# MihailMihov/simd-raytracer

Measured on AMD Instinct MI355X. Metric: Mrays/s (intersect invocations per second), hw09/scene5 dragon 1920x1080 1spp, higher is better.
Workload: dtype f32; 1 GPU; BASELINE configs[1]: scenes/hw09/scene5.crtscene 1920x1080 1spp max_ray_depth=5 (primary + shadow + reflection rays), kd_tree_simd_accel semantics; rays_per_frame=2726485, primary_rays=2073600, parallelism=bucket-tiles x1

## Files before the change

include/rtk.h:

```cpp
#ifndef RTK_H
#define RTK_H

#include <stddef.h>
#include <stdint.h>

#ifdef __cplusplus
extern "C" {
#endif

#define RTK_ABI_VERSION 4

enum {
    RTK_OK = 0,
    RTK_ERR_INVALID = 1,
    RTK_ERR_NO_DEVICE = 2,
    RTK_ERR_HIP = 3,
    RTK_ERR_IO = 4,
    RTK_ERR_PARSE = 5,
    RTK_ERR_UNSUPPORTED = 6
};

enum { RTK_MAT_DIFFUSE = 0, RTK_MAT_REFLECTIVE = 1, RTK_MAT_REFRACTIVE = 2, RTK_MAT_CONSTANT = 3, RTK_MAT_TEXTURE = 4 };

enum { RTK_TEX_ALBEDO = 0, RTK_TEX_EDGES = 1, RTK_TEX_CHECKER = 2, RTK_TEX_BITMAP = 3 };
// ... 28 lines not shown
    const int32_t *mat_texture;
    const float *uvs;
    const int32_t *mesh_has_uvs;
    int32_t n_textures;
    const int32_t *tex_kind;
    const float *tex_color_a;
    const float *tex_color_b;
    const float *tex_param;
    int32_t n_lights;
    const float *light_pos;
    const float *light_intensity;
    float cam_pos[3];
    float cam_mat[9];
    float background[3];
    int32_t width, height;
    int32_t bucket_size;
    const uint8_t *tex_pixels;
    const int32_t *tex_bitmap;
} rtk_scene_desc;

typedef struct {
    int32_t n_meshes, n_materials, n_lights;
    int32_t n_vertices, n_triangles;
    int32_t width, height, bucket_size;
    int32_t n_textures, n_uv_vertices;
    int32_t n_bitmap_bytes;
} rtk_scene_info;

typedef struct {
    int32_t max_depth;
    int32_t max_leaf_size;
    float eps;
    int32_t normalize_hit_normal;
    int32_t device;
    int32_t traversal;
} rtk_accel_params;

enum { RTK_TRAVERSAL_REFERENCE = 0, RTK_TRAVERSAL_FAST = 1 };

typedef struct {
    int32_t n_nodes, n_inner, n_leaves;
    int32_t n_leaf_refs;
    int32_t max_leaf_refs;
    int32_t n_triangles;
    int32_t tree_depth;
    int32_t reserved;
} rtk_tree_info;

typedef struct { float origin[3]; float direction[3]; } rtk_ray;

typedef struct {
    float t, u, v;
    uint32_t tri;
    uint32_t mesh;
    float normal[3];
} rtk_hit;

typedef struct {
    int32_t width, height;
    int32_t spp;
    int32_t max_ray_depth;
    int32_t diffuse_rays;
    uint32_t seed;
    double fov_degrees;
    float shadow_bias, reflection_bias, refraction_bias;
    int32_t trace_mode;
    int32_t rank, world_size;
    int32_t collect_stats;
    int32_t sample_begin, sample_count;
} rtk_render_params;

typedef struct {
    uint64_t rays;
    uint64_t primary;
    uint64_t hits;
    uint64_t nodes;
    uint64_t boxpass;
    uint64_t leaves;
    uint64_t tris;
    uint64_t packets16;
} rtk_counters;

int rtk_abi_version(void);
const char *rtk_last_error(void);
int rtk_device_count(int *count);

int rtk_scene_create(const rtk_scene_desc *desc, rtk_scene **out);
int rtk_scene_load_crtscene(const char *path, rtk_scene **out);
int rtk_scene_get_info(const rtk_scene *scene, rtk_scene_info *info);
int rtk_scene_get_arrays(const rtk_scene *scene, int32_t *mesh_material, int32_t *mesh_nverts, int32_t *mesh_ntris,
                         float *vertices, uint32_t *indices, int32_t *mat_kind, float *mat_albedo, float *mat_ior,
                         int32_t *mat_smooth, float *light_pos, float *light_intensity, float *cam_pos,
                         float *cam_mat, float *background);
int rtk_scene_get_textures(const rtk_scene *scene, int32_t *mat_texture, int32_t *mesh_has_uvs, float *uvs,
                           int32_t *tex_kind, float *tex_color_a, float *tex_color_b, float *tex_param);
int rtk_scene_get_bitmaps(const rtk_scene *scene, int32_t *tex_bitmap, uint8_t *tex_pixels);
int rtk_decode_jpeg(const uint8_t *data, size_t size, int32_t *width, int32_t *height, int32_t *channels,
                    uint8_t *pixels, size_t cap);
int rtk_scene_vertex_normals(const rtk_scene *scene, int32_t mesh, float *out);
void rtk_scene_destroy(rtk_scene *scene);

int rtk_accel_build(const rtk_scene *scene, const rtk_accel_params *params, rtk_accel **out);
int rtk_accel_tree_info(const rtk_accel *accel, rtk_tree_info *info);
int rtk_accel_tree_dump(const rtk_accel *accel, float *nodes_box, int32_t *nodes_link, int32_t *leaf_refs);
void rtk_accel_destroy(rtk_accel *accel);

int rtk_accel_intersect(rtk_accel *accel, const rtk_ray *rays, size_t n, int cull, int trace_mode,
                        rtk_hit *out);
int rtk_accel_intersect_device(rtk_accel *accel, const rtk_ray *d_rays, size_t n, int cull, int trace_mode,
                               rtk_hit *d_out, void *hip_stream);
int rtk_accel_intersect_stats(rtk_accel *accel, const rtk_ray *d_rays, size_t n, int cull, int trace_mode,
                              rtk_hit *d_out, rtk_counters *counters);

#define RTK_OCCLUDED_MAX_STEPS 1024
enum { RTK_OCC_CLEAR = 0, RTK_OCC_OCCLUDED = 1, RTK_OCC_STEP_LIMIT = 2 };

int rtk_accel_occluded(rtk_accel *accel, const rtk_ray *rays, const float *max_t, size_t n,
                       float shadow_bias, int trace_mode, uint8_t *out,
                       uint64_t *n_intersections );
int rtk_accel_occluded_device(rtk_accel *accel, const rtk_ray *d_rays, const float *d_max_t, size_t n,
                              float shadow_bias, int trace_mode, uint8_t *d_out,
                              void *hip_stream);

typedef struct {
    int32_t max_ray_depth;
    int32_t diffuse_rays;
    uint32_t seed;
    int32_t sample;
    float shadow_bias, reflection_bias, refraction_bias;
    int32_t cull;
    int32_t trace_mode;
} rtk_radiance_params;
int rtk_accel_radiance(rtk_accel *accel, const rtk_ray *rays, const uint32_t *ids , size_t n,
                       const rtk_radiance_params *p, float *rgb , rtk_counters *counters );
int rtk_accel_radiance_device(rtk_accel *accel, const rtk_ray *d_rays, const uint32_t *d_ids , size_t n,
                              const rtk_radiance_params *p, float *d_rgb , void *hip_stream);

int rtk_accel_update_vertices(rtk_accel *accel, const float *vertices );
int rtk_accel_update_vertices_device(rtk_accel *accel, const float *d_vertices , void *hip_stream);

int rtk_accel_update_geometry(rtk_accel *accel, const float *vertices ,
                              const uint32_t *indices ,
                              const int32_t *mesh_ntris );
int rtk_accel_update_geometry_device(rtk_accel *accel, const float *d_vertices, const uint32_t *d_indices,
                                     const int32_t *mesh_ntris , void *hip_stream);

int rtk_render_output_floats(const rtk_accel *accel, const rtk_render_params *p, size_t *n_floats);
int rtk_render_frame(rtk_accel *accel, const rtk_render_params *p, float *rgb ,
                     rtk_counters *counters );
int rtk_render_frame_device(rtk_accel *accel, const rtk_render_params *p, float *d_out, void *hip_stream);
int rtk_render_last_counters(rtk_accel *accel, rtk_counters *counters);
int rtk_render_last_critical_path(rtk_accel *accel, double *ms);
int rtk_debug_counter_fills(rtk_accel *accel, uint64_t *fills);
int rtk_tiles_assemble_device(const rtk_accel *accel, const rtk_render_params *p, const float *d_gathered,
                              float *d_rgb, void *hip_stream);

int rtk_camera_rays(rtk_accel *accel, const rtk_render_params *p, int32_t sample, rtk_ray *rays );
int rtk_camera_rays_device(rtk_accel *accel, const rtk_render_params *p, int32_t sample, rtk_ray *d_rays, void *hip_stream);

typedef struct { float position[3]; float matrix[9]; } rtk_view;

int rtk_accel_get_camera(const rtk_accel *accel, rtk_view *out);
int rtk_accel_set_camera(rtk_accel *accel, const rtk_view *view);

int rtk_render_views(rtk_accel *accel, const rtk_render_params *p, const rtk_view *views , int32_t n_views,
                     float *rgb , rtk_counters *counters );
int rtk_render_views_device(rtk_accel *accel, const rtk_render_params *p, const rtk_view *d_views ,
                            int32_t n_views, float *d_out , void *hip_stream);

typedef struct { int32_t x0, y0, x1, y1; } rtk_rect;
enum { RTK_REGIONS_IN_FRAME = 0, RTK_REGIONS_PACKED = 1 };

int rtk_render_regions(rtk_accel *accel, const rtk_render_params *p, const rtk_rect *rects , int32_t n_rects,
                       int layout, float *rgb , rtk_counters *counters );
int rtk_render_regions_device(rtk_accel *accel, const rtk_render_params *p, const rtk_rect *rects , int32_t n_rects,
                              int layout, float *d_out , void *hip_stream);

typedef struct {
    float    *depth;
    float    *position;
    float    *normal;
    float    *albedo;
    float    *bary;
    uint32_t *tri, *mesh, *material;
} rtk_gbuffer;

int rtk_render_gbuffer(rtk_accel *accel, const rtk_render_params *p, int32_t sample,
                       const rtk_view *views , int32_t n_views,
                       const rtk_gbuffer *out );
int rtk_render_gbuffer_device(rtk_accel *accel, const rtk_render_params *p, int32_t sample,
                              const rtk_view *d_views , int32_t n_views,
                              const rtk_gbuffer *out , void *hip_stream);

typedef struct {
    int32_t min_samples;
    int32_t step;
    float   threshold;
    float   floor;
} rtk_adaptive_params;

int rtk_render_adaptive(rtk_accel *accel, const rtk_render_params *p, const rtk_adaptive_params *ap,
                        float *rgb , uint32_t *samples ,
                        float *noise , rtk_counters *counters );
int rtk_render_adaptive_device(rtk_accel *accel, const rtk_render_params *p, const rtk_adaptive_params *ap,
                               float *d_rgb, uint32_t *d_samples, float *d_noise, void *hip_stream);

int rtk_render_frame_noise(rtk_accel *accel, const rtk_render_params *p, float *rgb ,
                           float *noise , rtk_counters *counters );
int rtk_render_frame_noise_device(rtk_accel *accel, const rtk_render_params *p, float *d_rgb, float *d_noise, void *hip_stream);
int rtk_debug_noise_fallbacks(rtk_accel *accel, uint64_t *count);

typedef struct {
    int32_t width, height;
    int32_t iterations;
    int32_t normal_power_log2;
    float   sigma_luminance;
    float   sigma_plane;
    float   albedo_floor;
    int32_t reserved;
} rtk_denoise_params;
typedef struct { const float *rgb, *noise, *albedo, *normal, *position, *depth; } rtk_denoise_inputs;

int rtk_denoise_workspace_bytes(const rtk_denoise_params *p, int32_t n_images, size_t *bytes);
int rtk_denoise_frame(const rtk_denoise_params *p, int32_t n_images, const rtk_denoise_inputs *in ,
                      float *rgb_out );
int rtk_denoise_frame_device(const rtk_denoise_params *p, int32_t n_images,
                             const rtk_denoise_inputs *in , float *d_rgb_out,
                             void *d_workspace, size_t workspace_bytes, void *hip_stream);

typedef struct { float position[3]; float intensity; } rtk_light;
typedef struct { int32_t kind, smooth; float albedo[3]; float ior; int32_t texture; int32_t reserved; } rtk_material;

int rtk_accel_get_lights(const rtk_accel *accel, rtk_light *out , int32_t cap, int32_t *n);
int rtk_accel_set_lights(rtk_accel *accel, const rtk_light *lights , int32_t n);
int rtk_accel_set_lights_device(rtk_accel *accel, const rtk_light *d_lights , int32_t n, void *hip_stream);

int rtk_accel_get_materials(const rtk_accel *accel, rtk_material *out );
int rtk_accel_set_materials(rtk_accel *accel, const rtk_material *materials , int32_t n);

int rtk_accel_get_background(const rtk_accel *accel, float rgb[3]);
int rtk_accel_set_background(rtk_accel *accel, const float rgb[3]);

typedef struct { int32_t kind; float color_a[3]; float color_b[3]; float param; int32_t width, height; } rtk_texture;

int rtk_accel_get_textures(const rtk_accel *accel, rtk_texture *out , int32_t cap, int32_t *n);
int rtk_accel_get_texture_pixels(const rtk_accel *accel, int32_t texture, uint8_t *out , size_t cap, size_t *n_bytes);
int rtk_accel_set_textures(rtk_accel *accel, const rtk_texture *textures, int32_t n,
                           const uint8_t *const *pixels );
int rtk_accel_set_texture_pixels(rtk_accel *accel, int32_t texture, int32_t width, int32_t height, const uint8_t *rgb );
int rtk_accel_set_texture_pixels_device(rtk_accel *accel, int32_t texture, int32_t width, int32_t height, const uint8_t *d_rgb, void *hip_stream);
int rtk_accel_set_texture_frame_device(rtk_accel *accel, int32_t texture, int32_t width, int32_t height,
                                       const float *d_rgb , void *hip_stream);
int rtk_accel_get_uvs(const rtk_accel *accel, float *uvs );
int rtk_accel_set_uvs(rtk_accel *accel, const float *uvs );
int rtk_accel_set_uvs_device(rtk_accel *accel, const float *d_uvs , void *hip_stream);

int rtk_frame_to_rgb8_device(const float *d_rgb, size_t n, uint8_t *d_out, void *hip_stream);
int rtk_format_ppm_rgb8(const uint8_t *rgb8, int32_t width, int32_t height, char *buf, size_t cap, size_t *n);
int rtk_write_ppm(const float *rgb, int32_t width, int32_t height, const char *path);
int rtk_format_ppm(const float *rgb, int32_t width, int32_t height, char *buf, size_t cap, size_t *n);

#ifdef __cplusplus
}
#endif
#endif
```

simd-raytracer_amd/__init__.py:

```python
from __future__ import annotations

import ctypes as C
import os
from dataclasses import dataclass

import numpy as np

_HERE = os.path.dirname(os.path.abspath(__file__))
_LIB_PATH = os.environ.get("RTK_LIB_OVERRIDE") or os.path.join(_HERE, "librtk_hip.so")

RTK_OK, RTK_ERR_INVALID, RTK_ERR_NO_DEVICE, RTK_ERR_HIP, RTK_ERR_IO, RTK_ERR_PARSE, RTK_ERR_UNSUPPORTED = range(7)
MAT_DIFFUSE, MAT_REFLECTIVE, MAT_REFRACTIVE, MAT_CONSTANT, MAT_TEXTURE = 0, 1, 2, 3, 4
TEX_ALBEDO, TEX_EDGES, TEX_CHECKER, TEX_BITMAP = 0, 1, 2, 3
TRACE_AUTO, TRACE_LANE, TRACE_WAVE, TRACE_GROUP4, TRACE_GROUP8, TRACE_GROUP16, TRACE_STREAM, TRACE_TWOPASS = 0, 1, 2, 3, 4, 5, 6, 7
TRAVERSAL_REFERENCE, TRAVERSAL_FAST = 0, 1
TRACE_REPACK = 8
OCC_CLEAR, OCC_OCCLUDED, OCC_STEP_LIMIT = 0, 1, 2
OCCLUDED_MAX_STEPS = 1024
REGIONS_IN_FRAME, REGIONS_PACKED = 0, 1
MAX_REGIONS = 65536

ABI_SYMBOLS = [
    "rtk_abi_version", "rtk_last_error", "rtk_device_count",
    "rtk_scene_create", "rtk_scene_load_crtscene", "rtk_scene_get_info", "rtk_scene_get_arrays", "rtk_scene_get_textures",
    "rtk_scene_get_bitmaps", "rtk_decode_jpeg",
    "rtk_scene_vertex_normals", "rtk_scene_destroy",
    "rtk_accel_build", "rtk_accel_tree_info", "rtk_accel_tree_dump", "rtk_accel_destroy",
    "rtk_accel_intersect", "rtk_accel_intersect_device", "rtk_accel_intersect_stats",
    "rtk_accel_occluded", "rtk_accel_occluded_device",
    "rtk_accel_radiance", "rtk_accel_radiance_device",
    "rtk_accel_update_vertices", "rtk_accel_update_vertices_device",
    "rtk_accel_update_geometry", "rtk_accel_update_geometry_device",
    "rtk_render_output_floats", "rtk_render_frame", "rtk_render_frame_device", "rtk_render_last_counters",
    "rtk_render_last_critical_path", "rtk_debug_counter_fills",
    "rtk_tiles_assemble_device", "rtk_camera_rays", "rtk_camera_rays_device",
    "rtk_accel_get_camera", "rtk_accel_set_camera", "rtk_render_views", "rtk_render_views_device",
    "rtk_render_regions", "rtk_render_regions_device",
    "rtk_render_gbuffer", "rtk_render_gbuffer_device",
    "rtk_render_adaptive", "rtk_render_adaptive_device",
    "rtk_render_frame_noise", "rtk_render_frame_noise_device", "rtk_debug_noise_fallbacks",
    "rtk_denoise_workspace_bytes", "rtk_denoise_frame", "rtk_denoise_frame_device",
    "rtk_accel_get_lights", "rtk_accel_set_lights", "rtk_accel_set_lights_device",
    "rtk_accel_get_materials", "rtk_accel_set_materials", "rtk_accel_get_background", "rtk_accel_set_background",
    "rtk_accel_get_textures", "rtk_accel_get_texture_pixels", "rtk_accel_set_textures", "rtk_accel_set_texture_pixels",
    "rtk_accel_set_texture_pixels_device", "rtk_accel_set_texture_frame_device",
    "rtk_accel_get_uvs", "rtk_accel_set_uvs", "rtk_accel_set_uvs_device",
    "rtk_frame_to_rgb8_device", "rtk_format_ppm_rgb8", "rtk_write_ppm", "rtk_format_ppm",
]


class RtkError(RuntimeError):
    def __init__(self, code: int, msg: str):
        super().__init__(f"rtk error {code}: {msg}")
        self.code = code


if not os.path.exists(_LIB_PATH):
    raise ImportError(
        f"{_LIB_PATH} is missing: build it with `python -c 'import __graft_entry__ as g; g.build()'` "
        "(hipcc --offload-arch=gfx950).  This package has no CPU fallback."
    )

try:
    import torch
except ImportError:
    torch = None

_L = C.CDLL(_LIB_PATH)


class SceneDesc(C.Structure):
    _fields_ = [
        ("n_meshes", C.c_int32), ("mesh_material", C.POINTER(C.c_int32)), ("mesh_nverts", C.POINTER(C.c_int32)),
        ("mesh_ntris", C.POINTER(C.c_int32)), ("vertices", C.POINTER(C.c_float)), ("indices", C.POINTER(C.c_uint32)),
        ("n_materials", C.c_int32), ("mat_kind", C.POINTER(C.c_int32)), ("mat_albedo", C.POINTER(C.c_float)),
        ("mat_ior", C.POINTER(C.c_float)), ("mat_smooth", C.POINTER(C.c_int32)),
        ("mat_texture", C.POINTER(C.c_int32)), ("uvs", C.POINTER(C.c_float)), ("mesh_has_uvs", C.POINTER(C.c_int32)),
        ("n_textures", C.c_int32), ("tex_kind", C.POINTER(C.c_int32)), ("tex_color_a", C.POINTER(C.c_float)),
        ("tex_color_b", C.POINTER(C.c_float)), ("tex_param", C.POINTER(C.c_float)),
        ("n_lights", C.c_int32), ("light_pos", C.POINTER(C.c_float)), ("light_intensity", C.POINTER(C.c_float)),
        ("cam_pos", C.c_float * 3), ("cam_mat", C.c_float * 9), ("background", C.c_float * 3),
        ("width", C.c_int32), ("height", C.c_int32), ("bucket_size", C.c_int32),
        ("tex_pixels", C.POINTER(C.c_uint8)), ("tex_bitmap", C.POINTER(C.c_int32)),
    ]


class SceneInfo(C.Structure):
    _fields_ = [(n, C.c_int32) for n in
                ("n_meshes", "n_materials", "n_lights", "n_vertices", "n_triangles", "width", "height", "bucket_size",
                 "n_textures", "n_uv_vertices", "n_bitmap_bytes")]


class AccelParams(C.Structure):
    _fields_ = [("max_depth", C.c_int32), ("max_leaf_size", C.c_int32), ("eps", C.c_float),
                ("normalize_hit_normal", C.c_int32), ("device", C.c_int32), ("traversal", C.c_int32)]


class TreeInfo(C.Structure):
    _fields_ = [(n, C.c_int32) for n in
                ("n_nodes", "n_inner", "n_leaves", "n_leaf_refs", "max_leaf_refs", "n_triangles", "tree_depth", "reserved")]


class RenderParams(C.Structure):
    _fields_ = [("width", C.c_int32), ("height", C.c_int32), ("spp", C.c_int32), ("max_ray_depth", C.c_int32),
                ("diffuse_rays", C.c_int32), ("seed", C.c_uint32), ("fov_degrees", C.c_double),
                ("shadow_bias", C.c_float), ("reflection_bias", C.c_float), ("refraction_bias", C.c_float),
                ("trace_mode", C.c_int32), ("rank", C.c_int32), ("world_size", C.c_int32), ("collect_stats", C.c_int32),
                ("sample_begin", C.c_int32), ("sample_count", C.c_int32)]


class RadianceParams(C.Structure):
    _fields_ = [("max_ray_depth", C.c_int32), ("diffuse_rays", C.c_int32), ("seed", C.c_uint32), ("sample", C.c_int32),
                ("shadow_bias", C.c_float), ("reflection_bias", C.c_float), ("refraction_bias", C.c_float),
                ("cull", C.c_int32), ("trace_mode", C.c_int32)]


class Counters(C.Structure):
    _fields_ = [(n, C.c_uint64) for n in ("rays", "primary", "hits", "nodes", "boxpass", "leaves", "tris", "packets16")]

    def as_dict(self):
        return {n: int(getattr(self, n)) for n, _ in self._fields_}


class GBuffer(C.Structure):
    _fields_ = [(n, C.c_void_p) for n in ("depth", "position", "normal", "albedo", "bary", "tri", "mesh", "material")]


class AdaptiveParams(C.Structure):
    _fields_ = [("min_samples", C.c_int32), ("step", C.c_int32), ("threshold", C.c_float), ("floor", C.c_float)]


class DenoiseParams(C.Structure):
    _fields_ = [("width", C.c_int32), ("height", C.c_int32), ("iterations", C.c_int32), ("normal_power_log2", C.c_int32),
                ("sigma_luminance", C.c_float), ("sigma_plane", C.c_float), ("albedo_floor", C.c_float), ("reserved", C.c_int32)]


class DenoiseInputs(C.Structure):
    _fields_ = [(n, C.c_void_p) for n in ("rgb", "noise", "albedo", "normal", "position", "depth")]


GBUFFER_PLANES = {"depth": ((), np.float32), "position": ((3,), np.float32), "normal": ((3,), np.float32),
                  "albedo": ((3,), np.float32), "bary": ((2,), np.float32), "tri": ((), np.uint32), "mesh": ((), np.uint32),
                  "material": ((), np.uint32)}

RAY_DTYPE = np.dtype([("origin", "<f4", (3,)), ("direction", "<f4", (3,))])
LIGHT_DTYPE = np.dtype([("position", "<f4", (3,)), ("intensity", "<f4")])
MATERIAL_DTYPE = np.dtype([("kind", "<i4"), ("smooth", "<i4"), ("albedo", "<f4", (3,)), ("ior", "<f4"), ("texture", "<i4"),
                           ("reserved", "<i4")])
TEXTURE_DTYPE = np.dtype([("kind", "<i4"), ("color_a", "<f4", (3,)), ("color_b", "<f4", (3,)), ("param", "<f4"), ("width", "<i4"),
                          ("height", "<i4")])
assert LIGHT_DTYPE.itemsize == 16 and MATERIAL_DTYPE.itemsize == 32 and TEXTURE_DTYPE.itemsize == 40
HIT_DTYPE = np.dtype([("t", "<f4"), ("u", "<f4"), ("v", "<f4"), ("tri", "<u4"), ("mesh", "<u4"), ("normal", "<f4", (3,))])
assert RAY_DTYPE.itemsize == 24 and HIT_DTYPE.itemsize == 32

_vp = C.c_void_p
_L.rtk_abi_version.restype = C.c_int
_L.rtk_last_error.restype = C.c_char_p
_L.rtk_device_count.argtypes = [C.POINTER(C.c_int)]
_L.rtk_scene_create.argtypes = [C.POINTER(SceneDesc), C.POINTER(_vp)]
_L.rtk_scene_load_crtscene.argtypes = [C.c_char_p, C.POINTER(_vp)]
_L.rtk_scene_get_info.argtypes = [_vp, C.POINTER(SceneInfo)]
_L.rtk_scene_get_arrays.argtypes = [_vp] * 15
_L.rtk_scene_get_textures.argtypes = [_vp] * 8
_L.rtk_scene_get_bitmaps.argtypes = [_vp] * 3
_L.rtk_decode_jpeg.argtypes = [_vp, C.c_size_t, C.POINTER(C.c_int32), C.POINTER(C.c_int32), C.POINTER(C.c_int32), _vp, C.c_size_t]
_L.rtk_scene_vertex_normals.argtypes = [_vp, C.c_int32, _vp]
_L.rtk_scene_destroy.argtypes = [_vp]
_L.rtk_scene_destroy.restype = None
_L.rtk_accel_build.argtypes = [_vp, C.POINTER(AccelParams), C.POINTER(_vp)]
_L.rtk_accel_tree_info.argtypes = [_vp, C.POINTER(TreeInfo)]
_L.rtk_accel_tree_dump.argtypes = [_vp, _vp, _vp, _vp]
_L.rtk_accel_destroy.argtypes = [_vp]
_L.rtk_accel_destroy.restype = None
_L.rtk_accel_intersect.argtypes = [_vp, _vp, C.c_size_t, C.c_int, C.c_int, _vp]
_L.rtk_accel_intersect_device.argtypes = [_vp, _vp, C.c_size_t, C.c_int, C.c_int, _vp, _vp]
_L.rtk_accel_intersect_stats.argtypes = [_vp, _vp, C.c_size_t, C.c_int, C.c_int, _vp, C.POINTER(Counters)]
_L.rtk_accel_occluded.argtypes = [_vp, _vp, _vp, C.c_size_t, C.c_float, C.c_int, _vp, C.POINTER(C.c_uint64)]
_L.rtk_accel_occluded_device.argtypes = [_vp, _vp, _vp, C.c_size_t, C.c_float, C.c_int, _vp, _vp]
_L.rtk_accel_radiance.argtypes = [_vp, _vp, _vp, C.c_size_t, C.POINTER(RadianceParams), _vp, C.POINTER(Counters)]
_L.rtk_accel_radiance_device.argtypes = [_vp, _vp, _vp, C.c_size_t, C.POINTER(RadianceParams), _vp, _vp]
_L.rtk_accel_update_vertices.argtypes = [_vp, _vp]
_L.rtk_accel_update_vertices_device.argtypes = [_vp, _vp, _vp]
_L.rtk_accel_update_geometry.argtypes = [_vp, _vp, _vp, _vp]
_L.rtk_accel_update_geometry_device.argtypes = [_vp, _vp, _vp, _vp, _vp]
_L.rtk_render_output_floats.argtypes = [_vp, C.POINTER(RenderParams), C.POINTER(C.c_size_t)]
_L.rtk_render_frame.argtypes = [_vp, C.POINTER(RenderParams), _vp, C.POINTER(Counters)]
_L.rtk_render_frame_device.argtypes = [_vp, C.POINTER(RenderParams), _vp, _vp]
_L.rtk_render_last_counters.argtypes = [_vp, C.POINTER(Counters)]
_L.rtk_render_last_critical_path.argtypes = [_vp, C.POINTER(C.c_double)]
if hasattr(_L, "rtk_debug_counter_fills"):
    _L.rtk_debug_counter_fills.argtypes = [_vp, C.POINTER(C.c_uint64)]
_L.rtk_tiles_assemble_device.argtypes = [_vp, C.POINTER(RenderParams), _vp, _vp, _vp]
_L.rtk_camera_rays.argtypes = [_vp, C.POINTER(RenderParams), C.c_int32, _vp]
_L.rtk_camera_rays_device.argtypes = [_vp, C.POINTER(RenderParams), C.c_int32, _vp, _vp]
_L.rtk_accel_get_camera.argtypes = [_vp, _vp]
_L.rtk_accel_set_camera.argtypes = [_vp, _vp]
_L.rtk_render_views.argtypes = [_vp, C.POINTER(RenderParams), _vp, C.c_int32, _vp, C.POINTER(Counters)]
_L.rtk_render_views_device.argtypes = [_vp, C.POINTER(RenderParams), _vp, C.c_int32, _vp, _vp]
_L.rtk_render_regions.argtypes = [_vp, C.POINTER(RenderParams), _vp, C.c_int32, C.c_int, _vp, C.POINTER(Counters)]
_L.rtk_render_regions_device.argtypes = [_vp, C.POINTER(RenderParams), _vp, C.c_int32, C.c_int, _vp, _vp]
_L.rtk_render_gbuffer.argtypes = [_vp, C.POINTER(RenderParams), C.c_int32, _vp, C.c_int32, C.POINTER(GBuffer)]
_L.rtk_render_gbuffer_device.argtypes = [_vp, C.POINTER(RenderParams), C.c_int32, _vp, C.c_int32, C.POINTER(GBuffer), _vp]
_L.rtk_render_adaptive.argtypes = [_vp, C.POINTER(RenderParams), C.POINTER(AdaptiveParams), _vp, _vp, _vp, C.POINTER(Counters)]
_L.rtk_render_adaptive_device.argtypes = [_vp, C.POINTER(RenderParams), C.POINTER(AdaptiveParams), _vp, _vp, _vp, _vp]
if hasattr(_L, "rtk_render_frame_noise"):
    _L.rtk_render_frame_noise.argtypes = [_vp, C.POINTER(RenderParams), _vp, _vp, C.POINTER(Counters)]
    _L.rtk_render_frame_noise_device.argtypes = [_vp, C.POINTER(RenderParams), _vp, _vp, _vp]
    _L.rtk_debug_noise_fallbacks.argtypes = [_vp, C.POINTER(C.c_uint64)]
_L.rtk_denoise_workspace_bytes.argtypes =[C.POINTER(DenoiseParams), C.c_int32, C.POINTER(C.c_size_t)]
_L.rtk_denoise_frame.argtypes = [C.POINTER(DenoiseParams), C.c_int32, C.POINTER(DenoiseInputs), _vp]
_L.rtk_denoise_frame_device.argtypes = [C.POINTER(DenoiseParams), C.c_int32, C.POINTER(DenoiseInputs), _vp, _vp, C.c_size_t, _vp]
_L.rtk_accel_get_lights.argtypes =[_vp, _vp, C.c_int32, C.POINTER(C.c_int32)]
_L.rtk_accel_set_lights.argtypes = [_vp, _vp, C.c_int32]
_L.rtk_accel_set_lights_device.argtypes = [_vp, _vp, C.c_int32, _vp]
_L.rtk_accel_get_materials.argtypes = [_vp, _vp]
_L.rtk_accel_set_materials.argtypes = [_vp, _vp, C.c_int32]
_L.rtk_accel_get_background.argtypes = [_vp, _vp]
_L.rtk_accel_set_background.argtypes = [_vp, _vp]
_L.rtk_accel_get_textures.argtypes = [_vp, _vp, C.c_int32, C.POINTER(C.c_int32)]
_L.rtk_accel_get_texture_pixels.argtypes = [_vp, C.c_int32, _vp, C.c_size_t, C.POINTER(C.c_size_t)]
_L.rtk_accel_set_textures.argtypes = [_vp, _vp, C.c_int32, _vp]
_L.rtk_accel_set_texture_pixels.argtypes = [_vp, C.c_int32, C.c_int32, C.c_int32, _vp]
_L.rtk_accel_set_texture_pixels_device.argtypes = [_vp, C.c_int32, C.c_int32, C.c_int32, _vp, _vp]
_L.rtk_accel_set_texture_frame_device.argtypes = [_vp, C.c_int32, C.c_int32, C.c_int32, _vp, _vp]
_L.rtk_accel_get_uvs.argtypes = [_vp, _vp]
_L.rtk_accel_set_uvs.argtypes = [_vp, _vp]
_L.rtk_accel_set_uvs_device.argtypes = [_vp, _vp, _vp]
_L.rtk_frame_to_rgb8_device.argtypes = [_vp, C.c_size_t, _vp, _vp]
_L.rtk_format_ppm_rgb8.argtypes = [_vp, C.c_int32, C.c_int32, _vp, C.c_size_t, C.POINTER(C.c_size_t)]
_L.rtk_write_ppm.argtypes = [_vp, C.c_int32, C.c_int32, C.c_char_p]
_L.rtk_format_ppm.argtypes = [_vp, C.c_int32, C.c_int32, _vp, C.c_size_t, C.POINTER(C.c_size_t)]


def _check(rc: int) -> None:
    if rc != RTK_OK:
        raise RtkError(rc, (_L.rtk_last_error() or b"").decode("utf-8", "replace"))


def lib() -> C.CDLL:
    return _L


def lib_path() -> str:
    return _LIB_PATH


def abi_version() -> int:
    return _L.rtk_abi_version()


def device_count() -> int:
    n = C.c_int(0)
    _check(_L.rtk_device_count(C.byref(n)))
    return n.value


def _fp(a, ty):
    return a.ctypes.data_as(C.POINTER(ty))


class Scene:

    def __init__(self, handle):
        self._h = handle
        info = SceneInfo()
        _check(_L.rtk_scene_get_info(self._h, C.byref(info)))
        self.info = info

    @classmethod
    def from_arrays(cls, mesh_material, mesh_nverts, mesh_ntris, vertices, indices, mat_kind, mat_albedo, mat_ior,
                    mat_smooth, light_pos, light_intensity, cam_pos, cam_mat, background, width, height, bucket_size=64,
                    mat_texture=None, uvs=None, mesh_has_uvs=None, tex_kind=None, tex_color_a=None, tex_color_b=None,
                    tex_param=None, tex_pixels=None, tex_bitmap=None):
        n_tex = 0 if tex_kind is None else len(tex_kind)
        keep = dict(
            mt=np.ascontiguousarray(mat_texture if mat_texture is not None else np.full(len(mat_kind), -1), np.int32),
            uv=np.ascontiguousarray(uvs if uvs is not None else np.zeros((0, 2)), np.float32),
            hu=np.ascontiguousarray(mesh_has_uvs if mesh_has_uvs is not None else np.zeros(len(mesh_material)), np.int32),
            tk=np.ascontiguousarray(tex_kind if tex_kind is not None else np.zeros(0), np.int32),
            ta=np.ascontiguousarray(tex_color_a if tex_color_a is not None else np.zeros((n_tex, 3)), np.float32),
            tb=np.ascontiguousarray(tex_color_b if tex_color_b is not None else np.zeros((n_tex, 3)), np.float32),
            tp=np.ascontiguousarray(tex_param if tex_param is not None else np.zeros(n_tex), np.float32),
            px=np.ascontiguousarray(tex_pixels if tex_pixels is not None else np.zeros(0), np.uint8),
            bm=np.ascontiguousarray(tex_bitmap if tex_bitmap is not None else np.zeros((n_tex, 3)), np.int32),
            mm=np.ascontiguousarray(mesh_material, np.int32), nv=np.ascontiguousarray(mesh_nverts, np.int32),
            nt=np.ascontiguousarray(mesh_ntris, np.int32), v=np.ascontiguousarray(vertices, np.float32),
            ix=np.ascontiguousarray(indices, np.uint32), mk=np.ascontiguousarray(mat_kind, np.int32),
            ma=np.ascontiguousarray(mat_albedo, np.float32), mi=np.ascontiguousarray(mat_ior, np.float32),
            ms=np.ascontiguousarray(mat_smooth, np.int32), lp=np.ascontiguousarray(light_pos, np.float32),
            li=np.ascontiguousarray(light_intensity, np.float32),
        )
        d = SceneDesc()
        d.n_meshes = len(keep["mm"])
        d.mesh_material, d.mesh_nverts, d.mesh_ntris = _fp(keep["mm"], C.c_int32), _fp(keep["nv"], C.c_int32), _fp(keep["nt"], C.c_int32)
        d.vertices, d.indices = _fp(keep["v"], C.c_float), _fp(keep["ix"], C.c_uint32)
        d.n_materials = len(keep["mk"])
        d.mat_kind, d.mat_albedo = _fp(keep["mk"], C.c_int32), _fp(keep["ma"], C.c_float)
        d.mat_ior, d.mat_smooth = _fp(keep["mi"], C.c_float), _fp(keep["ms"], C.c_int32)
        d.mat_texture, d.uvs, d.mesh_has_uvs = _fp(keep["mt"], C.c_int32), _fp(keep["uv"], C.c_float), _fp(keep["hu"], C.c_int32)
        d.n_textures = n_tex
        d.tex_kind, d.tex_color_a = _fp(keep["tk"], C.c_int32), _fp(keep["ta"], C.c_float)
        d.tex_color_b, d.tex_param = _fp(keep["tb"], C.c_float), _fp(keep["tp"], C.c_float)
        d.tex_pixels, d.tex_bitmap = _fp(keep["px"], C.c_uint8), _fp(keep["bm"], C.c_int32)
        d.n_lights = len(keep["li"])
        d.light_pos, d.light_intensity = _fp(keep["lp"], C.c_float), _fp(keep["li"], C.c_float)
        d.cam_pos[:] = [float(x) for x in np.asarray(cam_pos, np.float32)]
        d.cam_mat[:] = [float(x) for x in np.asarray(cam_mat, np.float32)]
        d.background[:] = [float(x) for x in np.asarray(background, np.float32)]
        d.width, d.height, d.bucket_size = int(width), int(height), int(bucket_size)
        h = _vp()
        _check(_L.rtk_scene_create(C.byref(d), C.byref(h)))
        return cls(h)

    def arrays(self) -> dict:
        i = self.info
        out = dict(
            mesh_material=np.zeros(i.n_meshes, np.int32), mesh_nverts=np.zeros(i.n_meshes, np.int32),
            mesh_ntris=np.zeros(i.n_meshes, np.int32), vertices=np.zeros((i.n_vertices, 3), np.float32),
            indices=np.zeros((i.n_triangles, 3), np.uint32), mat_kind=np.zeros(i.n_materials, np.int32),
            mat_albedo=np.zeros((i.n_materials, 3), np.float32), mat_ior=np.zeros(i.n_materials, np.float32),
            mat_smooth=np.zeros(i.n_materials, np.int32), light_pos=np.zeros((i.n_lights, 3), np.float32),
            light_intensity=np.zeros(i.n_lights, np.float32), cam_pos=np.zeros(3, np.float32),
            cam_mat=np.zeros(9, np.float32), background=np.zeros(3, np.float32),
        )
        _check(_L.rtk_scene_get_arrays(self._h, *[a.ctypes.data for a in out.values()]))
        tex = dict(
            mat_texture=np.zeros(i.n_materials, np.int32), mesh_has_uvs=np.zeros(i.n_meshes, np.int32),
            uvs=np.zeros((i.n_uv_vertices, 2), np.float32), tex_kind=np.zeros(i.n_textures, np.int32),
            tex_color_a=np.zeros((i.n_textures, 3), np.float32), tex_color_b=np.zeros((i.n_textures, 3), np.float32),
            tex_param=np.zeros(i.n_textures, np.float32),
        )
        _check(_L.rtk_scene_get_textures(self._h, *[a.ctypes.data for a in tex.values()]))
        out.update(tex)
        bmp = dict(tex_bitmap=np.zeros((i.n_textures, 3), np.int32), tex_pixels=np.zeros(i.n_bitmap_bytes, np.uint8))
        _check(_L.rtk_scene_get_bitmaps(self._h, bmp["tex_bitmap"].ctypes.data, bmp["tex_pixels"].ctypes.data))
        out.update(bmp)
        out.update(width=i.width, height=i.height, bucket_size=i.bucket_size)
        return out

    def vertex_normals(self, mesh: int) -> np.ndarray:
        nv = int(self.arrays()["mesh_nverts"][mesh])
        out = np.zeros((nv, 3), np.float32)
        _check(_L.rtk_scene_vertex_normals(self._h, mesh, out.ctypes.data))
        return out
# ... 395 lines not shown
        _check(_L.rtk_render_adaptive_device(self._h, C.byref(p), C.byref(ap), d_rgb_ptr or None, d_samples_ptr or None,
                                             d_noise_ptr or None, stream))

    def render_frame_noise(self, cfg: RenderConfig):
        w = cfg.width or self.scene.info.width
        h = cfg.height or self.scene.info.height
        rgb = np.zeros((h, w, 3), np.float32)
        noise = np.zeros((h, w), np.float32)
        p = cfg.to_c()
        c = Counters()
        _check(_L.rtk_render_frame_noise(self._h, C.byref(p), rgb.ctypes.data, noise.ctypes.data, C.byref(c)))
        return rgb, noise, c.as_dict()

    def render_frame_noise_device(self, cfg: RenderConfig, d_rgb_ptr: int, d_noise_ptr: int, stream: int = 0) -> None:
        p = cfg.to_c()
        _check(_L.rtk_render_frame_noise_device(self._h, C.byref(p), d_rgb_ptr or None, d_noise_ptr or None, stream))

    def noise_fallbacks(self) -> int:
        n = C.c_uint64(0)
        _check(_L.rtk_debug_noise_fallbacks(self._h, C.byref(n)))
        return n.value

    def lights(self):
        n = C.c_int32(0)
        _check(_L.rtk_accel_get_lights(self._h, None, 0, C.byref(n)))
        tab = np.zeros(n.value, LIGHT_DTYPE)
        _check(_L.rtk_accel_get_lights(self._h, tab.ctypes.data if n.value else None, n.value, C.byref(n)))
        return tab["position"].copy(), tab["intensity"].copy()

    def set_lights(self, positions, intensities) -> None:
        pos, inten = np.asarray(positions, np.float32), np.asarray(intensities, np.float32)
        if inten.ndim != 1 or pos.shape != (inten.shape[0], 3):
            raise ValueError("positions must have shape (n, 3) and intensities (n,)")
        tab = np.zeros(inten.shape[0], LIGHT_DTYPE)
        tab["position"], tab["intensity"] = pos, inten
        _check(_L.rtk_accel_set_lights(self._h, tab.ctypes.data if tab.size else None, tab.shape[0]))

    def set_lights_device(self, d_lights_ptr: int, n: int, stream: int = 0) -> None:
        _check(_L.rtk_accel_set_lights_device(self._h, d_lights_ptr or None, n, stream))

    def materials(self) -> dict:
        tab = np.zeros(self.scene.info.n_materials, MATERIAL_DTYPE)
        _check(_L.rtk_accel_get_materials(self._h, tab.ctypes.data))
        return {k: tab[k].copy() for k in ("kind", "albedo", "ior", "smooth", "texture")}

    def set_materials(self, kind, albedo, ior, smooth, texture=None) -> None:
        m = self.scene.info.n_materials
        kind, smooth = np.asarray(kind), np.asarray(smooth)
        albedo, ior = np.asarray(albedo, np.float32), np.asarray(ior, np.float32)
        texture = np.full(m, -1, np.int32) if texture is None else np.asarray(texture)
        for a in (kind, smooth, texture):
            if a.shape != (m,) or a.dtype.kind not in "iub":
                raise ValueError(f"kind, smooth and texture must be {m} integers, one per material")
        if albedo.shape != (m, 3) or ior.shape != (m,):
            raise ValueError(f"albedo must have shape ({m}, 3) and ior ({m},)")
        tab = np.zeros(m, MATERIAL_DTYPE)
        tab["kind"], tab["smooth"], tab["albedo"], tab["ior"], tab["texture"] = kind, smooth, albedo, ior, texture
        _check(_L.rtk_accel_set_materials(self._h, tab.ctypes.data, m))

    def background(self) -> np.ndarray:
        rgb = np.zeros(3, np.float32)
        _check(_L.rtk_accel_get_background(self._h, rgb.ctypes.data))
        return rgb

    def set_background(self, rgb) -> None:
        rgb = np.asarray(rgb, np.float32)
        if rgb.shape != (3,):
            raise ValueError("the background has 3 floats")
        rgb = np.ascontiguousarray(rgb)
        _check(_L.rtk_accel_set_background(self._h, rgb.ctypes.data))

    def textures(self) -> dict:
        n = C.c_int32(0)
        _check(_L.rtk_accel_get_textures(self._h, None, 0, C.byref(n)))
        tab = np.zeros(n.value, TEXTURE_DTYPE)
        _check(_L.rtk_accel_get_textures(self._h, tab.ctypes.data if n.value else None, n.value, C.byref(n)))
        return {k: tab[k].copy() for k in TEXTURE_DTYPE.names}

    def set_textures(self, kind, color_a=None, color_b=None, param=None, pixels=None) -> None:
        kind = np.asarray(kind)
        if kind.ndim != 1 or (kind.size and kind.dtype.kind not in "iub"):
            raise ValueError("kind must be a list of integers, one per texture")
        t = kind.shape[0]
        color_a = np.zeros((t, 3), np.float32) if color_a is None else np.asarray(color_a, np.float32)
        color_b = np.zeros((t, 3), np.float32) if color_b is None else np.asarray(color_b, np.float32)
        param = np.zeros(t, np.float32) if param is None else np.asarray(param, np.float32)
        if color_a.shape != (t, 3) or color_b.shape != (t, 3) or param.shape != (t,):
            raise ValueError(f"color_a and color_b must have shape ({t}, 3) and param ({t},)")
        pixels = [None] * t if pixels is None else list(pixels)
        if len(pixels) != t:
            raise ValueError("pixels must have one entry per texture")
        tab = np.zeros(t, TEXTURE_DTYPE)
        tab["kind"], tab["color_a"], tab["color_b"], tab["param"] = kind, color_a, color_b, param
        keep, ptrs = [], (_vp * max(1, t))()
        for i in range(t):
            if pixels[i] is None or kind[i] != TEX_BITMAP:
                continue
            px = np.ascontiguousarray(pixels[i], np.uint8)
            if px.ndim != 3 or px.shape[2] != 3:
                raise ValueError("the texels of a bitmap are uint8 [height, width, 3]")
            tab["height"][i], tab["width"][i] = px.shape[0], px.shape[1]
            keep.append(px)
            ptrs[i] = px.ctypes.data
        _check(_L.rtk_accel_set_textures(self._h, tab.ctypes.data if t else None, t, ptrs))

    def texture_pixels(self, texture: int) -> np.ndarray:
        n = C.c_size_t(0)
        _check(_L.rtk_accel_get_texture_pixels(self._h, texture, None, 0, C.byref(n)))
        tex = self.textures()
        out = np.zeros((int(tex["height"][texture]), int(tex["width"][texture]), 3), np.uint8)
        assert out.size == n.value
        if out.size:
            _check(_L.rtk_accel_get_texture_pixels(self._h, texture, out.ctypes.data, out.size, C.byref(n)))
        return out

    def set_texture_pixels(self, texture: int, rgb) -> None:
        px = np.asarray(rgb)
        if px.dtype != np.uint8 or px.ndim != 3 or px.shape[2] != 3:
            raise ValueError("the texels of a bitmap are uint8 [height, width, 3]")
        px = np.ascontiguousarray(px)
        _check(_L.rtk_accel_set_texture_pixels(self._h, texture, px.shape[1], px.shape[0], px.ctypes.data if px.size else None))

    def set_texture_pixels_device(self, texture: int, width: int, height: int, d_rgb_ptr: int, stream: int = 0) -> None:
        _check(_L.rtk_accel_set_texture_pixels_device(self._h, texture, width, height, d_rgb_ptr or None, stream))

    def set_texture_frame_device(self, texture: int, width: int, height: int, d_rgb_ptr: int, stream: int = 0) -> None:
        _check(_L.rtk_accel_set_texture_frame_device(self._h, texture, width, height, d_rgb_ptr or None, stream))

    def uvs(self) -> np.ndarray:
        out = np.zeros((self.scene.info.n_vertices, 2), np.float32)
        _check(_L.rtk_accel_get_uvs(self._h, out.ctypes.data))
        return out

    def set_uvs(self, uv) -> None:
        uv = np.asarray(uv, np.float32)
        if uv.shape != (self.scene.info.n_vertices, 2):
            raise ValueError(f"uvs must have shape ({self.scene.info.n_vertices}, 2)")
        uv = np.ascontiguousarray(uv)
        _check(_L.rtk_accel_set_uvs(self._h, uv.ctypes.data))

    def set_uvs_device(self, d_uvs_ptr: int, stream: int = 0) -> None:
        _check(_L.rtk_accel_set_uvs_device(self._h, d_uvs_ptr or None, stream))

    def last_critical_path_ms(self) -> float:
        ms = C.c_double(0.0)
        _check(_L.rtk_render_last_critical_path(self._h, C.byref(ms)))
        return ms.value

    def counter_fills(self) -> int:
        n = C.c_uint64(0)
        _check(_L.rtk_debug_counter_fills(self._h, C.byref(n)))
        return int(n.value)

    def assemble_device(self, cfg: RenderConfig, d_gathered_ptr: int, d_rgb_ptr: int, stream: int = 0) -> None:
        p = cfg.to_c()
        _check(_L.rtk_tiles_assemble_device(self._h, C.byref(p), d_gathered_ptr, d_rgb_ptr, stream))

    def __del__(self, _destroy=_L.rtk_accel_destroy):
        if getattr(self, "_h", None):
            _destroy(self._h)
            self._h = None


def render_frame(accel: KdTreeSimdAccel, cfg: RenderConfig | None = None):
    return accel.render_frame(cfg or RenderConfig())


def format_ppm(rgb: np.ndarray) -> bytes:
    rgb = np.ascontiguousarray(rgb, np.float32)
    h, w, _ = rgb.shape
    n = C.c_size_t(0)
    _check(_L.rtk_format_ppm(rgb.ctypes.data, w, h, None, 0, C.byref(n)))
    buf = C.create_string_buffer(n.value)
    _check(_L.rtk_format_ppm(rgb.ctypes.data, w, h, buf, n.value, C.byref(n)))
    return buf.raw[: n.value]


def frame_to_rgb8_device(d_rgb_ptr: int, n_floats: int, d_out_ptr: int, stream: int = 0) -> None:
    _check(_L.rtk_frame_to_rgb8_device(d_rgb_ptr, n_floats, d_out_ptr, stream))


def denoise_workspace_bytes(width: int, height: int, n_images: int = 1, cfg: DenoiseConfig | None = None) -> int:
    p = (cfg or DenoiseConfig()).to_c(width, height)
    n = C.c_size_t(0)
    _check(_L.rtk_denoise_workspace_bytes(C.byref(p), n_images, C.byref(n)))
    return n.value


def denoise(rgb: np.ndarray, normal: np.ndarray, position: np.ndarray, depth: np.ndarray, noise: np.ndarray | None = None,
            albedo: np.ndarray | None = None, cfg: DenoiseConfig | None = None) -> np.ndarray:
    rgb = np.ascontiguousarray(rgb, np.float32)
    if rgb.ndim not in (3, 4) or rgb.shape[-1] != 3:
        raise ValueError("rgb must be [h, w, 3] or [K, h, w, 3]")
    lead = rgb.shape[:-1]
    k = 1 if rgb.ndim == 3 else lead[0]
    h, w = lead[-2], lead[-1]

    def plane(a, shape, name):
        if a is None:
            return None
        a = np.ascontiguousarray(a, np.float32)
        if a.shape != shape:
            raise ValueError(f"{name} must have shape {shape}, not {a.shape}")
        return a

    normal, position = plane(normal, rgb.shape, "normal"), plane(position, rgb.shape, "position")
    albedo = plane(albedo, rgb.shape, "albedo")
    depth, noise = plane(depth, lead, "depth"), plane(noise, lead, "noise")
    if normal is None or position is None or depth is None:
        raise ValueError("normal, position and depth are required")
    out = np.zeros_like(rgb)
    if rgb.size == 0:
        return out
    ptr = lambda a: None if a is None else a.ctypes.data
    inputs = DenoiseInputs(ptr(rgb), ptr(noise), ptr(albedo), ptr(normal), ptr(position), ptr(depth))
    p = (cfg or DenoiseConfig()).to_c(w, h)
    _check(_L.rtk_denoise_frame(C.byref(p), k, C.byref(inputs), out.ctypes.data))
    return out


def denoise_device(width: int, height: int, d_rgb_ptr: int, d_normal_ptr: int, d_position_ptr: int, d_depth_ptr: int, d_out_ptr: int,
                   d_workspace_ptr: int, workspace_bytes: int, d_noise_ptr: int = 0, d_albedo_ptr: int = 0, n_images: int = 1,
                   cfg: DenoiseConfig | None = None, stream: int = 0) -> None:
    inputs = DenoiseInputs(d_rgb_ptr or None, d_noise_ptr or None, d_albedo_ptr or None, d_normal_ptr or None, d_position_ptr or None,
                           d_depth_ptr or None)
    p = (cfg or DenoiseConfig()).to_c(width, height)
    _check(_L.rtk_denoise_frame_device(C.byref(p), n_images, C.byref(inputs), d_out_ptr or None, d_workspace_ptr or None,
                                       workspace_bytes, stream or None))


def format_ppm_rgb8(rgb8: np.ndarray) -> bytes:
    rgb8 = np.ascontiguousarray(rgb8, np.uint8)
    h, w, _ = rgb8.shape
    n = C.c_size_t(0)
    _check(_L.rtk_format_ppm_rgb8(rgb8.ctypes.data, w, h, None, 0, C.byref(n)))
    buf = C.create_string_buffer(n.value)
    _check(_L.rtk_format_ppm_rgb8(rgb8.ctypes.data, w, h, buf, n.value, C.byref(n)))
    return buf.raw[: n.value]


def write_ppm(rgb: np.ndarray, path: str) -> None:
    rgb = np.ascontiguousarray(rgb, np.float32)
    h, w, _ = rgb.shape
    _check(_L.rtk_write_ppm(rgb.ctypes.data, w, h, os.fsencode(path)))
```

simd-raytracer_amd/csrc/accel.hpp:

```cpp
#pragma once

#include <hip/hip_runtime.h>

#include <cstdlib>
#include <mutex>
#include <string>
#include <vector>

#include "abi_guard.hpp"
#include "kernels.hpp"
#include "stream.hpp"
#include "build.hpp"
#include "dev_mem.hpp"
#include "frame_plan.hpp"
#include "update_plan.hpp"

struct rtk_knobs {
    uint32_t slice_min_tris = rtk::kSliceMinTrisDefault;
    bool shadow_exit = true;
    bool skip_unlit_shadow = true;
    bool bundle_cull = true;
    bool auto_trials = true;
    bool cost_feedback = true;
    unsigned resort_every = 16;
    uint32_t light_cycles = 140000u;
    uint32_t order_floor_cycles = 20000u;
    bool batch_scalar_surv = false;
    bool stream_scalar_surv = true;
    bool repack = true;
    bool raster_tiles = true;
    int repack_skip_bits = 6;
    bool repack_full_bounds = false;
    int repack_skip_bits2 = 14;
    bool repack_dirs3 = false;
    int repack_trace = -1;
    size_t group8_below = 9000;
    int stream_node_factor = 0;
    int stream_deep_level = 99, stream_deep_mode = RTK_TRACE_AUTO;
    uint32_t auto_min_lanes = 12;
    int stream_sort_from = -1;
    bool stream_debug = false;
    bool stream_side = true;
    int stream_lanes = 4;
    int stream_slices = 0;
    int stream_batch = 0;
    int stream_mem_gb = 96;
    int stream_side_below = 2;
    bool first_frame_prior = true;
    bool fast_occluders = true;
    bool camera_keeps_order = false;
    size_t views_launch_units = 131072;
    bool traversal_fast = false;
    size_t adaptive_chunk_pixels = size_t(1) << 20;

    static rtk_knobs from_env() {
        rtk_knobs k;
        auto geti = [](const char *name, long &out) { const char *e = std::getenv(name); if (!e || !*e) return false; out = std::atol(e); return true; };
        long v;
        if (geti("RTK_SLICE_MIN_TRIS", v) && v > 0) k.slice_min_tris = uint32_t(v);
        if (geti("RTK_SHADOW_EARLY_EXIT", v)) k.shadow_exit = v != 0;
        if (geti("RTK_SKIP_UNLIT_SHADOW", v)) k.skip_unlit_shadow = v != 0;
        if (geti("RTK_BUNDLE_CULL", v)) k.bundle_cull = v != 0;
        if (geti("RTK_AUTO_TRIALS", v)) k.auto_trials = v != 0;
        if (geti("RTK_COST_FEEDBACK", v)) k.cost_feedback = v != 0;
        if (geti("RTK_COST_RESORT_EVERY", v) && v > 0) k.resort_every = unsigned(v);
        if (geti("RTK_LIGHT_BELOW_CYCLES", v) && v >= 0) k.light_cycles = uint32_t(v);
        if (geti("RTK_ORDER_FLOOR_CYCLES", v) && v >= 0) k.order_floor_cycles = uint32_t(v);
        if (geti("RTK_REPACK", v)) k.repack = v != 0;
        if (geti("RTK_RASTER_TILES", v)) k.raster_tiles = v != 0;
        if (geti("RTK_REPACK_FULL_BOUNDS", v)) k.repack_full_bounds = v != 0;
        if (geti("RTK_REPACK_SKIP_BITS2", v) && v >= 0 && v <= 22) k.repack_skip_bits2 = int(v);
        if (geti("RTK_REPACK_DIRS3", v)) k.repack_dirs3 = v != 0;
        if (geti("RTK_REPACK_SKIP_BITS", v) && v >= 0 && v <= 14) k.repack_skip_bits = int(v);
        if (geti("RTK_STREAM_SCALAR_SURV", v)) k.stream_scalar_surv = v != 0;
        if (geti("RTK_BATCH_SCALAR_SURV", v)) k.batch_scalar_surv = v != 0;
        if (geti("RTK_REPACK_TRACE", v) && (v == RTK_TRACE_AUTO || v == RTK_TRACE_WAVE || v == RTK_TRACE_LANE)) k.repack_trace = int(v);
        if (geti("RTK_GROUP8_BELOW_BLOCKS", v) && v >= 0) k.group8_below = size_t(v);
        if (geti("RTK_STREAM_NODE_FACTOR", v) && v >= 1) k.stream_node_factor = int(v);
        if (geti("RTK_STREAM_DEEP_LEVEL", v)) k.stream_deep_level = int(v);
        if (geti("RTK_STREAM_DEEP_MODE", v)) k.stream_deep_mode = int(v);
        if (geti("RTK_AUTO_MIN_LANES", v) && v > 0 && v <= 64) k.auto_min_lanes = uint32_t(v);
        if (geti("RTK_STREAM_SORT_FROM", v)) k.stream_sort_from = int(v);
        if (geti("RTK_STREAM_DEBUG", v)) k.stream_debug = v != 0;
        if (geti("RTK_STREAM_SIDE", v)) k.stream_side = v != 0;
        if (geti("RTK_TRAVERSAL_FAST", v)) k.traversal_fast = v != 0;
        if (geti("RTK_FIRST_FRAME_PRIOR", v)) k.first_frame_prior = v != 0;
        if (geti("RTK_STREAM_SLICES", v) && (v == 0 || v == 1 || v == 2 || v == 4)) k.stream_slices = int(v);
        if (geti("RTK_STREAM_BATCH", v) && v >= 0 && v <= 4096) k.stream_batch = int(v);
        if (geti("RTK_STREAM_MEM_GB", v) && v >= 1 && v <= 256) k.stream_mem_gb = int(v);
        if (geti("RTK_FAST_OCCLUDERS", v)) k.fast_occluders = v != 0;
        if (geti("RTK_STREAM_SIDE_BELOW", v) && v >= 0) k.stream_side_below = int(v);
        if (geti("RTK_VIEWS_LAUNCH_UNITS", v) && v >= 1 && v <= (1l << 30)) k.views_launch_units = size_t(v);
        if (geti("RTK_CAMERA_KEEPS_ORDER", v)) k.camera_keeps_order = v != 0;
        if (geti("RTK_STREAM_LANES", v) && v >= 1 && v <= rtk::dev::kStreamLanes) k.stream_lanes = int(v);
        if (geti("RTK_ADAPTIVE_CHUNK_PIXELS", v) && v >= 1 && v <= (1l << 30)) k.adaptive_chunk_pixels = size_t(v);
        return k;
    }
};

namespace rtk {
struct DeviceMem {
    static int alloc(void **p, size_t bytes) { return int(hipMalloc(p, bytes)); }
    static void free(void *p) { (void)hipFree(p); }
};
struct PinnedMem {
    static int alloc(void **p, size_t bytes) { return int(hipHostMalloc(p, bytes, hipHostMallocDefault)); }
    static void free(void *p) { (void)hipHostFree(p); }
};
template <unsigned Flags> struct EventSrc {
    using handle = hipEvent_t;
    static int create(handle *h) { return int(Flags == hipEventDefault ? hipEventCreate(h) : hipEventCreateWithFlags(h, Flags)); }
    static void destroy(handle h) { (void)hipEventDestroy(h); }
};
template <typename T> using DevBuf = Buf<T, DeviceMem>;
template <typename T> using PinBuf = Buf<T, PinnedMem>;
using DevEvent = Event<EventSrc<hipEventDisableTiming>>;
using TimedEvent = Event<EventSrc<hipEventDefault>>;

struct LastUse {
    DevEvent done;
    bool in_use = false;
    hipError_t wait_previous(hipStream_t s) {
        const hipError_t e = static_cast<hipError_t>(done.ensure());
        return e == hipSuccess && in_use ? hipStreamWaitEvent(s, done.get(), 0) : e;
    }
    hipError_t record(hipStream_t s) {
        hipError_t e = static_cast<hipError_t>(done.ensure());
        if (e == hipSuccess) e = hipEventRecord(done.get(), s);
        if (e == hipSuccess) in_use = true;
        return e;
    }
};

class GeomFence {
    DevEvent ready_;
    bool pending_ = false;
public:
    hipError_t quiesce() {
        hipError_t e = static_cast<hipError_t>(ready_.ensure());
        if (e == hipSuccess) e = hipDeviceSynchronize();
        if (e == hipSuccess) pending_ = false;
        return e;
    }
    hipError_t publish(hipStream_t s) {
        const hipError_t e = hipEventRecord(ready_.get(), s);
        if (e == hipSuccess) pending_ = true;
        return e;
    }
    hipError_t wait(hipStream_t s) {
        if (!pending_) return hipSuccess;
        if (hipEventQuery(ready_.get()) == hipSuccess) { pending_ = false; return hipSuccess; }
        (void)hipGetLastError();
        return hipStreamWaitEvent(s, ready_.get(), 0);
    }
    hipError_t sync_host() const { return ready_.get() ? hipEventSynchronize(ready_.get()) : hipSuccess; }
};

struct GeomBufs {
    DevBuf<DevNode> nodes, leaves;
    DevBuf<DevNode> leaves_fast;
    DevBuf<DevTri> tris;
    DevBuf<uint32_t> tri_ids;
    DevBuf<DevShade> shade;
    DevBuf<int32_t> leaf_refs;
    DevBuf<DevNode> occl_nodes, occl_leaves;
    DevBuf<DevTri> occl_tris;
    DevBuf<uint32_t> occl_ids;
    void swap_occl(GeomBufs &o) { occl_nodes.swap(o.occl_nodes); occl_leaves.swap(o.occl_leaves); occl_tris.swap(o.occl_tris); occl_ids.swap(o.occl_ids); }
    void swap(GeomBufs &o, bool fast, bool occl) {
        nodes.swap(o.nodes); leaves.swap(o.leaves); tris.swap(o.tris); tri_ids.swap(o.tri_ids); shade.swap(o.shade); leaf_refs.swap(o.leaf_refs);
        if (fast) leaves_fast.swap(o.leaves_fast);
        if (occl) swap_occl(o);
    }
};
struct TopoBufs {
    DevBuf<uint32_t> index, inc_off, inc;
    DevBuf<uint8_t> opaque;
    DevBuf<DevTriUv> tri_uv;
    void swap(TopoBufs &o, bool uv) { index.swap(o.index); inc_off.swap(o.inc_off); inc.swap(o.inc); opaque.swap(o.opaque); if (uv) tri_uv.swap(o.tri_uv); }
};
struct StreamBufs {
    DevBuf<dev::RayRec> rays;
    DevBuf<dev::NodeRes> nodes;
    DevBuf<dev::HitRec> hits;
    DevBuf<float2> contrib;
    DevBuf<uint32_t> ctrl, node_bins, hit_bins, node_order, hit_order;
    void reset() { rays.reset(); nodes.reset(); hits.reset(); contrib.reset(); ctrl.reset(); node_bins.reset(); hit_bins.reset(); node_order.reset(); hit_order.reset(); }
};
}

struct rtk_cost_feedback {
    rtk::DevBuf<uint32_t> cost, order;
    rtk::DevBuf<uint8_t> bins;
    rtk::OrderState state;
    rtk::PinBuf<uint32_t> nwgs_host;
    rtk::DevEvent nwgs_ev;

    void forget() { state.forget(); }
};

struct rtk_accel {
    rtk_knobs knobs;
    bool coords_small = false;
    rtk_scene scene;
    rtk::HostTree tree;
    rtk_accel_params params;
    bool has_refractive = false;
    bool fast_traversal = false;
    int stream_slices_auto = 4;
    std::mutex mu;
    bool on_device = false;
    int device = -1;
    ~rtk_accel() { if (device >= 0) (void)hipSetDevice(device); }
    rtk::GeomBufs geom, geom_spare;
    rtk::DevBuf<rtk::DevMaterial> d_materials;
    rtk::DevBuf<rtk::DevLight> d_lights;
    rtk::DevBuf<rtk::DevTexture> d_textures;
    rtk::DevBuf<uint8_t> d_tex_pixels;
    rtk::DevBuf<unsigned long long> d_counters;
    rtk::CounterState cnt;
    uint64_t counter_fills = 0;
    uint32_t occl_n_leaves = 0;
    bool occl_on = false;
    rtk::StreamBufs ws_bufs[rtk::dev::kStreamLanes];
    rtk::DevBuf<float> ws_sumbuf;
    rtk::dev::StreamWs ws = {};
    rtk::dev::StreamWs ws_lane[rtk::dev::kStreamLanes] = {};
    rtk::StreamWsShape ws_shape;
    hipStream_t lane_stream[rtk::dev::kStreamLanes] = {};
    rtk::DevEvent lane_done[rtk::dev::kStreamLanes];
    rtk::DevEvent lane_fork;
    struct SideEvents { rtk::DevEvent ready[2], done[2]; } lane_side_ev[rtk::dev::kStreamLanes];
    rtk::StreamSide lane_side[rtk::dev::kStreamLanes] = {};
    rtk::LastUse ws_last;
    rtk_cost_feedback fb;
    std::vector<rtk_cost_feedback> fb_views;
    rtk::DevBuf<rtk_view> views_tab;
    rtk::DevBuf<float> views_out;
    rtk::DevBuf<unsigned long long> d_views_counters;
    std::vector<rtk_cost_feedback> fb_regions;
    std::vector<rtk_rect> rg_rects;
    rtk::RegionsPlan rg_plan;
    int rg_layout = -1;
    uint32_t rg_width = 0;
    size_t rg_limit = 0;
    rtk::DevBuf<rtk::RegionEntry> rg_table;
    bool rg_table_valid = false;
    rtk::LastUse rg_last;
    rtk::DevBuf<rtk_ray> rg_rays;
    rtk::DevBuf<uint32_t> rg_ids;
    rtk::DevBuf<float> rg_rgb;
    rtk::DevBuf<float> rg_out;
    rtk::DevBuf<rtk_view> gb_views;
    rtk::DevBuf<uint32_t> gb_out;
    rtk::DevBuf<double> ad_s1, ad_s2;
    rtk::DevBuf<uint32_t> ad_list;
    rtk::DevBuf<uint32_t> ad_blocks;
    rtk::DevBuf<unsigned long long> ad_count;
    rtk::PinBuf<unsigned long long> ad_count_host;
    rtk::DevBuf<rtk_ray> ad_rays;
    rtk::DevBuf<float> ad_rgb;
    rtk::DevBuf<uint32_t> ad_out;
    rtk::LastUse ad_last;
    rtk::PinBuf<uint32_t> fn_overflow_host;
    rtk::DevBuf<float> fn_out;
    uint64_t noise_fallbacks = 0;
    rtk::TimedEvent trial_ev[4];
    rtk::EngineTrial trial;
    rtk::DevBuf<uint32_t> rp_bounds, rp_keys, rp_idx;
    rtk::DevBuf<uint8_t> rp_temp;
    size_t rp_temp_bytes = 0;
    rtk::PinBuf<uint32_t> rp_host;
    rtk::DevEvent rp_probe_ev;
    rtk::LastUse rp_last;
    rtk::DevBuf<rtk_ray> oc_rays;
    rtk::DevBuf<float> oc_max_t;
    rtk::DevBuf<uint8_t> oc_out;
    rtk::DevBuf<unsigned long long> d_rad_counters;
    rtk::DevBuf<rtk_ray> rad_rays;
    rtk::DevBuf<uint32_t> rad_ids;
    rtk::DevBuf<float> rad_rgb;
    bool refs_on_device = false;
    int32_t n_leaf_refs_dev = 0;
    bool up_static = false;
    rtk::TopoBufs topo, topo_spare;
    rtk::DevBuf<float> up_verts;
    rtk::DevBuf<rtk::DevTri> up_tris;
    rtk::DevBuf<float> up_tbox;
    std::vector<int32_t> mesh_nverts, mesh_ntris;
    rtk::DevBuf<rtk::dev::TopoMesh> topo_meshes;
    rtk::DevBuf<float> topo_vert_uv;
    rtk::DevBuf<uint32_t> topo_keys;
    rtk::DevBuf<uint8_t> topo_temp;
    rtk::DevBuf<uint32_t> up_idx_stage;
    rtk::DevBuf<uint32_t> up_ref_id, up_ref_node;
    rtk::DevBuf<uint8_t> up_table;
    rtk::PinBuf<uint8_t> up_table_host;
    rtk::DevBuf<rtk::dev::GatherLeaf> up_gather;
    rtk::PinBuf<uint8_t> up_stage;
    rtk::GeomFence geom_fence;
    bool lights_on_device = false;
    rtk::DevBuf<rtk::DevMaterial> st_materials;
    rtk::DevBuf<rtk::dev::OcclLeaf> st_leaves;
    rtk::DevBuf<uint32_t> st_counts;
    struct TexSlot {
        int32_t off = 0;
        size_t cap = 0;
        bool on_device = false;
    };
    std::vector<TexSlot> tx_slots;
    size_t tx_used = 0;
    rtk::DevBuf<rtk::DevTexture> tx_textures;
    rtk::DevBuf<uint8_t> tx_pixels;
    std::vector<float> vert_uv;
    bool vert_uv_made = false;
    bool uvs_on_device = false;
    bool vert_uv_dev = false;
    hipStream_t last_stream = nullptr;
    uint64_t last_primary = 0;
    bool last_stats = false;
};

namespace rtk {

inline int fail(int code, const std::string &msg) { set_error(msg); return code; }

inline int hip_fail(hipError_t e, const char *what) {
    set_error(std::string(what) + ": " + hipGetErrorString(e));
    return RTK_ERR_HIP;
}

#define RTK_HIP_AS(call, what)                               \
    do {                                                     \
        const hipError_t e_ = (call);                        \
        if (e_ != hipSuccess) return hip_fail(e_, what);     \
    } while (0)
#define RTK_HIP(call) RTK_HIP_AS(call, #call)
#define RTK_TRY(call) do { const int rc_ = (call); if (rc_ != RTK_OK) return rc_; } while (0)

#define RTK_MEM(call) RTK_HIP_AS(static_cast<hipError_t>(call), #call)

template <typename T>
int upload(const std::vector<T> &src, DevBuf<T> &dst) {
    RTK_MEM(dst.reserve(src.empty() ? 1 : src.size()));
    if (src.empty()) return RTK_OK;
    const hipError_t e = hipMemcpy(dst.get(), src.data(), src.size() * sizeof(T), hipMemcpyHostToDevice);
    if (e != hipSuccess) { dst.reset(); return hip_fail(e, "upload"); }
    return RTK_OK;
}

inline bool valid_mode(int m) { return m == RTK_TRACE_AUTO || m == RTK_TRACE_LANE || m == RTK_TRACE_WAVE; }
inline bool valid_batch_mode(int m) { return valid_mode(m) || m == RTK_TRACE_REPACK; }
inline bool valid_frame_mode(int m) { return valid_mode(m) || m == RTK_TRACE_GROUP4 || m == RTK_TRACE_GROUP8 || m == RTK_TRACE_GROUP16 ||
           m == RTK_TRACE_STREAM || m == RTK_TRACE_TWOPASS; }

inline int stream_slices_for(const HostTree &t) {
    double refs = 0.0, sq = 0.0;
    for (const DevNode &l : t.dev_leaves) { refs += double(l.b); sq += double(l.b) * double(l.b); }
    return (refs > 0.0 && sq / refs < 150.0) ? 1 : 4;
}

inline bool scene_forks(const rtk_accel *a, int diffuse_rays) { return a->has_refractive || diffuse_rays > 0; }
inline bool scene_general(const rtk_accel *a, int diffuse_rays) { return scene_forks(a, diffuse_rays) || !a->scene.textures.empty(); }

inline unsigned long long *counters_now(const rtk_accel *a) { return a->d_counters.get() + size_t(a->cnt.current) * kCounterAllocWords; }
inline unsigned long long *counters_other(const rtk_accel *a) { return a->d_counters.get() + size_t(a->cnt.current ^ 1) * kCounterAllocWords; }

int ensure_device(rtk_accel *a, hipStream_t s = nullptr);
dev::TreeView tree_view(const rtk_accel *a);
enum : unsigned { kKeepViewOrders = 1u, kKeepTrial = 2u };
inline void forget_orders(rtk_accel *a, unsigned keep = 0u) {
    a->fb.forget();
    a->cnt.forget();
    if (!(keep & kKeepViewOrders)) for (rtk_cost_feedback &f : a->fb_views) f.forget();
    for (rtk_cost_feedback &f : a->fb_regions) f.forget();
    if (!(keep & kKeepTrial)) a->trial.abandon();
}

int remake_occluders(rtk_accel *a, const std::vector<DevMaterial> &materials, const DevMaterial *d_materials, hipStream_t s);
int ensure_update_static(rtk_accel *a);
void dense_texture_slots(rtk_accel *a);
const std::vector<float> &host_vert_uv(rtk_accel *a);
int ensure_vert_uv_dev(rtk_accel *a);
int frame_geom(const rtk_accel *a, const rtk_render_params *p, FrameGeom &g);
rtk_view accel_camera(const rtk_accel *a);
void camera_args(const rtk_view &cam, const rtk_render_params *p, const FrameGeom &g, dev::RenderArgs &A);
int ensure_stream_ws(rtk_accel *a, size_t pixels, size_t nodes, size_t lights, bool need_sum, int lanes);
hipError_t zero_counters(rtk_accel *a, hipStream_t s);
void record_last(rtk_accel *a, hipStream_t s, bool stats, uint64_t primary);
int radiance_device_impl(rtk_accel *a, const rtk_ray *d_rays, const uint32_t *d_ids, size_t n, const rtk_radiance_params *p,
                         float *d_rgb, hipStream_t s, uint32_t *n_chunks_out);
void free_stream_ws(rtk_accel *a);
struct StreamSetup {
    dev::StreamArgs S;
    int deep_level, deep_mode, sort_from, slices;
    size_t factor, node_bytes, budget;
};
StreamSetup stream_args(const rtk_accel *a, const dev::RenderArgs &A, int diffuse_rays, bool forks);
int claim_stream_ws(rtk_accel *a, hipStream_t s);
int release_stream_ws(rtk_accel *a, hipStream_t s);
int fork_lanes(rtk_accel *a, int lanes, hipStream_t s);
int join_lanes(rtk_accel *a, int lanes, hipStream_t s);
dev::RenderArgs frame_args(const rtk_accel *a, const rtk_render_params *p, const FrameGeom &g, const rtk_view &cam, float *d_out);
int adaptive_device_impl(rtk_accel *a, const rtk_render_params *p, const rtk_adaptive_params *ap, const FrameGeom &g, float *d_rgb,
                         uint32_t *d_samples, float *d_noise, hipStream_t s);

}
```

simd-raytracer_amd/csrc/api_frame.hip:

```cpp
#include <cmath>
#include <cstdio>
#include <cstring>
#include <mutex>

#include "accel.hpp"
#include "stream_plan.hpp"

namespace rtk {

int frame_geom(const rtk_accel *a, const rtk_render_params *p, FrameGeom &g) {
    if (!a || !p) return fail(RTK_ERR_INVALID, "null accel or params");
    const int64_t w = p->width > 0 ? p->width : a->scene.width;
    const int64_t h = p->height > 0 ? p->height : a->scene.height;
    if (w <= 0 || h <= 0 || w > 65536 || h > 65536) return fail(RTK_ERR_INVALID, "image size must be in [1, 65536]");
    if (p->spp < 1) return fail(RTK_ERR_INVALID, "spp must be >= 1");
    if (p->max_ray_depth < 0 || p->max_ray_depth > kMaxRayDepth)
        return fail(RTK_ERR_INVALID, "max_ray_depth must be in [0, 16]");
    if (p->diffuse_rays < 0 || p->diffuse_rays > 32767) return fail(RTK_ERR_INVALID, "diffuse_rays must be in [0, 32767]");
    if (!valid_frame_mode(p->trace_mode)) return fail(RTK_ERR_INVALID, "unknown trace_mode");
    if (p->sample_begin < 0 || p->sample_count < 0 || p->sample_begin >= p->spp ||
        int64_t(p->sample_begin) + p->sample_count > p->spp)
        return fail(RTK_ERR_INVALID, "sample_begin / sample_count must select samples inside [0, spp)");
    if (p->sample_count == 0 && p->sample_begin != 0) return fail(RTK_ERR_INVALID, "sample_count == 0 means all samples: sample_begin must be 0");
    g.sample_begin = p->sample_begin;
// ... 125 lines not shown
        A.occl.nodes = a->geom.occl_nodes.get(); A.occl.leaves = a->geom.occl_leaves.get(); A.occl.leaves_fast = nullptr; A.occl.n_leaves = a->occl_n_leaves;
        A.occl.tris = a->geom.occl_tris.get(); A.occl.tri_ids = a->geom.occl_ids.get();
    }
    return A;
}

hipError_t fill_counters(rtk_accel *a, hipStream_t s) {
    a->counter_fills += 1;
    return hipMemsetAsync(counters_now(a), 0, kCounterAllocWords * sizeof(unsigned long long), s);
}

}

hipError_t zero_counters(rtk_accel *a, hipStream_t s) {
    a->cnt.forget();
    return fill_counters(a, s);
}

void record_last(rtk_accel *a, hipStream_t s, bool stats, uint64_t primary) {
    a->last_stream = s;
    a->last_stats = stats;
    a->last_primary = primary;
}

rtk_view accel_camera(const rtk_accel *a) {
    rtk_view v;
    std::memcpy(v.position, a->scene.cam_pos, sizeof(v.position));
    std::memcpy(v.matrix, a->scene.cam_mat, sizeof(v.matrix));
    return v;
}

void camera_args(const rtk_view &cam, const rtk_render_params *p, const FrameGeom &g, dev::RenderArgs &A) {
    std::memcpy(A.cam_pos, cam.position, sizeof(A.cam_pos));
    std::memcpy(A.cam_mat, cam.matrix, sizeof(A.cam_mat));
    A.width = g.width; A.height = g.height;
    A.aspect = static_cast<float>(g.width) / static_cast<float>(g.height);
    const float fov_radians = static_cast<float>(p->fov_degrees * (3.14159265358979323846 / 180.0));
    A.tan_half_fov = std::tan(fov_radians / 2.0f);
    A.spp = p->spp; A.seed = p->seed;
    A.width_f = static_cast<float>(g.width); A.height_f = static_cast<float>(g.height); A.spp_f = static_cast<float>(p->spp);
}


StreamSetup stream_args(const rtk_accel *a, const dev::RenderArgs &A, int diffuse_rays, bool forks) {
    StreamSetup u = {};
    u.S.r = A; u.S.r.tree.scalar_surv = a->knobs.stream_scalar_surv ? 1 : 0;
    u.S.key_dirs = diffuse_rays > 0 ? 1u : 0u; u.S.n_batch = 1; u.S.auto_min_lanes = a->knobs.auto_min_lanes;
    const DevNode &root = a->tree.dev_nodes[0];
    for (int k = 0; k < 3; ++k) {
        const float ext = root.hi[k] - root.lo[k];
        u.S.grid_lo[k] = root.lo[k];
        u.S.grid_scale[k] = (ext > 0.f && ext < 3.0e38f) ? 16.0f / ext : 0.f;
    }
    u.deep_level = a->knobs.stream_deep_level; u.deep_mode = a->knobs.stream_deep_mode;
    u.sort_from = a->knobs.stream_sort_from >= 0 ? a->knobs.stream_sort_from : (forks ? 1 : 99);
    u.slices = a->knobs.stream_slices > 0 ? a->knobs.stream_slices : a->stream_slices_auto;
    u.factor = a->knobs.stream_node_factor > 0 ? size_t(a->knobs.stream_node_factor) : (forks ? 8 : 3);
    u.node_bytes = stream_bytes_per_node(sizeof(dev::RayRec), sizeof(dev::NodeRes), sizeof(dev::HitRec), sizeof(float2), a->scene.lights.size());
    u.budget = size_t(a->knobs.stream_mem_gb) << 30;
    return u;
}

int claim_stream_ws(rtk_accel *a, hipStream_t s) { RTK_HIP(a->ws_last.wait_previous(s)); return RTK_OK; }
int release_stream_ws(rtk_accel *a, hipStream_t s) { RTK_HIP(a->ws_last.record(s)); return RTK_OK; }

int fork_lanes(rtk_accel *a, int lanes, hipStream_t s) {
    if (lanes > 1) RTK_HIP(hipEventRecord(a->lane_fork.get(), s));
    for (int j = 1; j < lanes; ++j) RTK_HIP(hipStreamWaitEvent(a->lane_stream[j], a->lane_fork.get(), 0));
    return RTK_OK;
}
int join_lanes(rtk_accel *a, int lanes, hipStream_t s) {
    for (int j = 1; j < lanes; ++j) RTK_HIP(hipStreamWaitEvent(s, a->lane_done[j].get(), 0));
    return RTK_OK;
}

namespace {

void trial_abandon(rtk_accel *a, hipEvent_t trial[2]) { trial[0] = trial[1] = nullptr; a->trial.abandon(); }

int choose_engine(rtk_accel *a, const rtk_render_params *p, const FrameGeom &g, bool forks, bool &stream, hipEvent_t trial[2]) {
    stream = p->trace_mode == RTK_TRACE_STREAM || (p->trace_mode == RTK_TRACE_AUTO && forks);
    if (!EngineTrial::applies(p->trace_mode, forks, p->collect_stats != 0)) return RTK_OK;
    uint64_t tsig[3];
    shape_sig(g, p->spp, p->max_ray_depth, p->diffuse_rays, tsig);
    if (a->knobs.auto_trials) {
        for (TimedEvent &e : a->trial_ev) RTK_MEM(e.ensure());
        if (a->trial.waiting(tsig)) {
            float t_stream = 0.f, t_mega = 0.f;
            if (hipEventQuery(a->trial_ev[1].get()) == hipSuccess && hipEventQuery(a->trial_ev[3].get()) == hipSuccess &&
                hipEventElapsedTime(&t_stream, a->trial_ev[0].get(), a->trial_ev[1].get()) == hipSuccess &&
                hipEventElapsedTime(&t_mega, a->trial_ev[2].get(), a->trial_ev[3].get()) == hipSuccess)
                a->trial.verdict(t_stream, t_mega);
            else (void)hipGetLastError();
        }
    }
    const EngineTrial::Step step = a->trial.next(tsig, a->knobs.auto_trials);
    stream = step.stream;
    if (step.record != EngineTrial::kNoRecord) { trial[0] = a->trial_ev[step.record].get(); trial[1] = a->trial_ev[step.record + 1].get(); }
    return RTK_OK;
}

int render_stream(rtk_accel *a, const rtk_render_params *p, const FrameGeom &g, const dev::RenderArgs &A, bool forks, bool general,
                  hipEvent_t trial[2], hipStream_t s) {
    StreamSetup u = stream_args(a, A, p->diffuse_rays, forks);
    const size_t n_root = g.blocks() * 64;
    const size_t nodes_per_sample = n_root * u.factor + 4096;
    const FramePlan plan = plan_frame_batches(g.sample_end - g.sample_begin, nodes_per_sample, u.node_bytes, u.budget,
                                              a->knobs.stream_lanes, a->knobs.stream_batch);
    const int batch = plan.batch, lanes = plan.lanes;
    const StreamWsShape ws_before = a->ws_shape;
    RTK_TRY(ensure_stream_ws(a, out_pixels(g), nodes_per_sample * size_t(batch), a->scene.lights.size(), p->spp > 1, lanes));
    if (trial[0] && (a->ws_shape.nodes != ws_before.nodes || a->ws_shape.lanes != ws_before.lanes)) trial_abandon(a, trial);
    if (trial[0]) RTK_HIP(hipEventRecord(trial[0], s));
    dev::StreamArgs &S = u.S;
    S.ws = a->ws; S.n_root = uint32_t(n_root); S.n_level0 = uint32_t(n_root);
    S.n_lanes = uint32_t(lanes);
    for (int j = 0; j < dev::kStreamLanes; ++j) S.lane_overflow[j] = a->ws_lane[j < lanes ? j : 0].ctrl + dev::kCtrlOverflow;
    RTK_TRY(claim_stream_ws(a, s));
    for (int j = 0; j < lanes; ++j) RTK_HIP(hipMemsetAsync(a->ws_lane[j].ctrl, 0, dev::kCtrlWords * sizeof(uint32_t), s));
    RTK_TRY(fork_lanes(a, lanes, s));
    const bool side = a->knobs.stream_side && lanes <= 2 && batch * lanes <= a->knobs.stream_side_below;
    for (int i = 0; i < plan.n_launch; ++i) {
        const int j = i % lanes;
        S.sample = g.sample_begin + i * batch;
        S.n_batch = uint32_t(g.sample_end - S.sample < batch ? g.sample_end - S.sample : batch);
        S.n_level0 = uint32_t(n_root) * S.n_batch;
        S.ws = a->ws_lane[j];
        const hipStream_t ls = j == 0 ? s : a->lane_stream[j];
        const hipEvent_t wait = (lanes > 1 && i > 0) ? a->lane_done[(i - 1) % lanes].get() : nullptr;
        const hipEvent_t done = lanes > 1 ? a->lane_done[j].get() : nullptr;
        RTK_HIP_AS(launch_stream_sample(S, p->collect_stats != 0, u.deep_level, u.deep_mode, u.sort_from, ls, wait, done,
                                        side ? &a->lane_side[j] : nullptr, u.slices), "launch streaming pipeline");
    }
    RTK_TRY(join_lanes(a, lanes, s));
    S.ws = a->ws;
    RTK_HIP_AS(launch_stream_overflow_reset(S, s), "launch overflow reset");
    dev::RenderArgs F = A;
    F.only_if = a->ws.ctrl + dev::kCtrlOverflow;
    RTK_HIP_AS(launch_render(F, RTK_TRACE_GROUP4, p->collect_stats != 0, general, s), "launch fallback k_render");
    RTK_TRY(release_stream_ws(a, s));
    if (a->knobs.stream_debug) {
        uint32_t h[dev::kCtrlWords];
        (void)hipStreamSynchronize(s);
        (void)hipMemcpy(h, a->ws.ctrl, sizeof(h), hipMemcpyDeviceToHost);
        std::fprintf(stderr, "[rtk stream] node_cap %u hit_cap %u overflow %u; nodes per level:", a->ws.node_cap, a->ws.hit_cap, h[dev::kCtrlOverflow]);
        for (int l = 0; l <= p->max_ray_depth + 1; ++l) std::fprintf(stderr, " %u", l == 0 ? unsigned(n_root) : h[dev::kCtrlNodeCount + l]);
        std::fprintf(stderr, "; hits:");
        for (int l = 0; l <= p->max_ray_depth; ++l) std::fprintf(stderr, " %u", h[dev::kCtrlHitCount + l]);
        std::fprintf(stderr, "\n");
    }
    return RTK_OK;
}

int ensure_feedback_ws(rtk_accel *a, rtk_cost_feedback &fb, const FrameGeom &g, size_t units) {
    if (fb.state.units >= units) return RTK_OK;
    const uint32_t bk = g.bucket;
    const uint64_t tx = (uint64_t(a->scene.width > 0 ? a->scene.width : 0) + bk - 1) / bk, ty = (uint64_t(a->scene.height > 0 ? a->scene.height : 0) + bk - 1) / bk;
    const size_t cap = fb.state.capacity(units, &fb == &a->fb, g.blocks_of(tx * ty));
    RTK_MEM(fb.cost.reserve(cap));
    RTK_MEM(fb.order.reserve(2 * (2 * cap + 4) + 8));
    RTK_MEM(fb.bins.reserve(cap));
    fb.state.units = cap;
    return RTK_OK;
}

struct ListSet { uint32_t *order, *hdr, *wg_list; };
ListSet list_set(rtk_cost_feedback &fb, int k, size_t units) {
    uint32_t *const order = fb.order.get() + size_t(k) * (2 * fb.state.units + 4);
    return {order, order + units, order + units + 4};
}

int launch_sort(rtk_accel *a, rtk_cost_feedback &fb, int k, int frame_mode, size_t units, hipStream_t s) {
    const ListSet L = list_set(fb, k, units);
    RTK_HIP_AS(launch_order_by_cost(fb.cost.get(), fb.bins.get(), L.order, L.wg_list, L.hdr, uint32_t(units),
                                    frame_mode == RTK_TRACE_GROUP4 ? a->knobs.light_cycles >> 4 : 0u, a->knobs.order_floor_cycles >> 4, 4u, s),
               "launch k_order_by_cost");
    RTK_MEM(fb.nwgs_host.reserve(1));
    RTK_MEM(fb.nwgs_ev.ensure());
    RTK_HIP(hipMemcpyAsync(fb.nwgs_host.get(), L.hdr, sizeof(uint32_t), hipMemcpyDeviceToHost, s));
    RTK_HIP(hipEventRecord(fb.nwgs_ev.get(), s));
    return RTK_OK;
}

int order_launch(rtk_accel *a, rtk_cost_feedback &fb, const rtk_render_params *p, const FrameGeom &g, dev::RenderArgs &A, int frame_mode,
                 size_t units, hipStream_t s, OrderState::Step &step) {
    uint64_t sig[5];
    shape_sig(g, p->spp, p->max_ray_depth, p->diffuse_rays, sig);
    sig[3] = (uint64_t(uint32_t(g.bucket)) << 32) | (uint64_t(uint32_t(g.sample_end - g.sample_begin) & 0xFFFFu) << 16) | uint32_t(p->trace_mode);
    sig[4] = A.regions ? ((1ull << 63) | (uint64_t(A.n_regions) << 32) | uint64_t(A.n_units))
                       : (A.views ? uint64_t(A.n_views) : 0ull);
    RTK_TRY(ensure_feedback_ws(a, fb, g, units));
    step = fb.state.step(sig, frame_mode, p->collect_stats != 0, A.regions != nullptr, {a->knobs.first_frame_prior, a->knobs.resort_every});
    const ListSet L = list_set(fb, step.read_set, units);
    if (step.prior)
        RTK_HIP_AS(launch_block_prior(A, fb.bins.get(), L.order, L.wg_list, L.hdr,
                                      reinterpret_cast<uint32_t *>(A.counters + kPriorScratchWord), 4u, s), "launch k_block_prior");
    if (step.sort_front) RTK_TRY(launch_sort(a, fb, step.read_set, frame_mode, units, s));
    if (step.use_order) { A.order_in = L.order; A.order_hdr = L.hdr; A.wg_list = L.wg_list; }
    if (&fb == &a->fb) a->cnt.after_order(step);
    A.cost_out = fb.cost.get();
    return RTK_OK;
}

int render_megakernel(rtk_accel *a, rtk_cost_feedback &fb, const rtk_render_params *p, const FrameGeom &g, dev::RenderArgs &A, bool general,
                      hipStream_t s) {
    const size_t units = A.regions ? size_t(A.n_units) : (A.views ? g.blocks() * A.n_views : g.blocks());
    A.n_units = uint32_t(units);
    const int frame_mode = OrderState::frame_mode(p->trace_mode, units, a->knobs.group8_below);
    OrderState::Step step = {};
    if (a->knobs.cost_feedback && units > 0 && units <= 0x7FFFFFFFull) {
        const int rc = order_launch(a, fb, p, g, A, frame_mode, units, s, step);
        if (rc != RTK_OK) { fb.forget(); return rc; }
    }
    unsigned n_wgs = 0;
    if (A.wg_list != nullptr) {
        bool ready = false;
        if (fb.state.awaits_count() && !(ready = hipEventQuery(fb.nwgs_ev.get()) == hipSuccess)) (void)hipGetLastError();
        n_wgs = fb.state.workgroups(ready, fb.nwgs_host.get());
    }
    int rc = RTK_OK;
    const hipError_t e = launch_render(A, frame_mode, p->collect_stats != 0, general, s, n_wgs);
    if (e != hipSuccess) rc = hip_fail(e, "launch k_render");
    if (rc == RTK_OK && step.sort_behind) rc = launch_sort(a, fb, step.write_set, frame_mode, units, s);
    if (rc != RTK_OK) fb.forget();
    return rc;
}

}

dev::RenderArgs frame_args(const rtk_accel *a, const rtk_render_params *p, const FrameGeom &g, const rtk_view &cam, float *d_out) {
    dev::RenderArgs A = scene_args(a, p->collect_stats);
    camera_args(cam, p, g, A);
    A.max_depth = p->max_ray_depth; A.diffuse_rays = p->diffuse_rays;
    A.gi_div_f = static_cast<float>(p->diffuse_rays + 1);
    A.sample_begin = g.sample_begin; A.sample_end = g.sample_end;
    A.shadow_bias = p->shadow_bias; A.reflection_bias = p->reflection_bias; A.refraction_bias = p->refraction_bias;
    A.bucket = g.bucket; A.tiles_x = g.tiles_x; A.tiles_y = g.tiles_y; A.n_buckets = g.n_buckets;
    A.blocks_per_bucket_side = g.blocks_side; A.buckets_per_rank = g.buckets_per_rank;
    A.rank = g.rank; A.world = g.world; A.compact = g.world > 1 ? 1 : 0; A.skew_q = g.skew_q;
    A.out = d_out; A.counters = counters_now(a);
    return A;
}

namespace {

int render_frame_body(rtk_accel *a, const rtk_render_params *p, const FrameGeom &g, const rtk_view &cam, float *d_out, hipStream_t s, bool steady) {
    const bool forks = scene_forks(a, p->diffuse_rays), general = scene_general(a, p->diffuse_rays);
    bool stream = false;
    hipEvent_t trial[2] = {nullptr, nullptr};
    RTK_TRY(choose_engine(a, p, g, forks, stream, trial));
    const CounterState::Step cs = a->cnt.frame(s, steady && !stream && p->collect_stats == 0);
    if (cs.fill) RTK_HIP(fill_counters(a, s));
    dev::RenderArgs A = frame_args(a, p, g, cam, d_out);
    if (cs.carry) A.zero_next = counters_other(a);
    if (g.world > 1 && g.sample_begin == 0) RTK_HIP(hipMemsetAsync(d_out, 0, out_pixels(g) * 3 * sizeof(float), s));
    if (trial[0] && !stream) RTK_HIP(hipEventRecord(trial[0], s));
    if (p->trace_mode == RTK_TRACE_TWOPASS && p->spp != 1) return fail(RTK_ERR_UNSUPPORTED, "RTK_TRACE_TWOPASS needs spp == 1");
    if (stream) RTK_TRY(render_stream(a, p, g, A, forks, general, trial, s));
    else RTK_TRY(render_megakernel(a, a->fb, p, g, A, general, s));
    if (trial[1]) RTK_HIP(hipEventRecord(trial[1], s));
    record_last(a, s, p->collect_stats != 0, primary_rays_of_rank(g));
    return RTK_OK;
}

int render_frame_impl(rtk_accel *a, const rtk_render_params *p, const FrameGeom &g, const rtk_view &cam, float *d_out, hipStream_t s, bool steady) {
    const int rc = render_frame_body(a, p, g, cam, d_out, s, steady);
    if (rc != RTK_OK) a->cnt.forget();
    return rc;
}

int render_device_impl(rtk_accel *a, const rtk_render_params *p, float *d_out, hipStream_t s) {
    FrameGeom g;
    RTK_TRY(frame_geom(a, p, g));
    if (!d_out) return fail(RTK_ERR_INVALID, "null output buffer");
    return render_frame_impl(a, p, g, accel_camera(a), d_out, s, true);
}



bool views_one_launch(const rtk_accel *a, const rtk_render_params *p) {
    if (p->collect_stats != 0) return false;
    if (p->trace_mode == RTK_TRACE_GROUP4 || p->trace_mode == RTK_TRACE_GROUP8 || p->trace_mode == RTK_TRACE_GROUP16) return true;
    return p->trace_mode == RTK_TRACE_AUTO && !scene_forks(a, p->diffuse_rays);
}

int views_check(const rtk_accel *a, const rtk_render_params *p, const void *views, int32_t n_views, const void *out, FrameGeom &g) {
    RTK_TRY(frame_geom(a, p, g));
    if (n_views < 0) return fail(RTK_ERR_INVALID, "n_views must be >= 0");
    if (p->world_size > 1) return fail(RTK_ERR_INVALID, "views are not sharded: deal whole views to the ranks");
    if (n_views > 0 && (!views || !out)) return fail(RTK_ERR_INVALID, "null views or output buffer");
    return RTK_OK;
}

struct CallCounters {
    rtk_accel *a;
    bool many;
    hipStream_t s;
    int begin() {
        if (!many) return RTK_OK;
        RTK_MEM(a->d_views_counters.reserve(kCounterWords));
        RTK_HIP(hipMemsetAsync(a->d_views_counters.get(), 0, kCounterWords * sizeof(unsigned long long), s));
        return RTK_OK;
    }
    int zero_part() { RTK_HIP(zero_counters(a, s)); return RTK_OK; }
    int after_part() { if (many) RTK_HIP_AS(launch_counters_fold(counters_now(a), a->d_views_counters.get(), s), "launch k_counters_fold"); return RTK_OK; }
    int end() {
        if (many) RTK_HIP(hipMemcpyAsync(counters_now(a), a->d_views_counters.get(), kCounterWords * sizeof(unsigned long long), hipMemcpyDeviceToDevice, s));
        return RTK_OK;
    }
};

template <typename PartArgs>
int render_parts(rtk_accel *a, std::vector<rtk_cost_feedback> &tables, size_t n_parts, const rtk_render_params *p, const FrameGeom &g,
                 hipStream_t s, PartArgs part_args) {
    if (tables.size() < n_parts) tables.resize(n_parts);
    const bool general = scene_general(a, p->diffuse_rays);
    CallCounters cc{a, n_parts > 1, s};
    RTK_TRY(cc.begin());
    for (size_t c = 0; c < n_parts; ++c) {
        dev::RenderArgs A = part_args(c);
        RTK_TRY(cc.zero_part());
        RTK_TRY(render_megakernel(a, tables[c], p, g, A, general, s));
        RTK_TRY(cc.after_part());
    }
    return cc.end();
}

int render_views_impl(rtk_accel *a, const rtk_render_params *p, const FrameGeom &g, const rtk_view *h_views, const rtk_view *d_views,
                      int32_t n_views, float *d_out, hipStream_t s) {
    const size_t stride = size_t(g.width) * g.height * 3;
    const size_t n = size_t(n_views);
    if (views_one_launch(a, p)) {
        const size_t per_view = g.blocks();
        const ViewsLaunches cut = views_launches(n, per_view, a->knobs.views_launch_units);
        const size_t per_launch = cut.per_launch;
        RTK_TRY(render_parts(a, a->fb_views, cut.n_parts, p, g, s, [&](size_t c) {
            const size_t first = c * per_launch, cnt = n - first < per_launch ? n - first : per_launch;
            dev::RenderArgs A = frame_args(a, p, g, accel_camera(a), d_out + first * stride);
            A.views = reinterpret_cast<const float *>(d_views + first);
            A.n_views = uint32_t(cnt); A.units_per_view = uint32_t(per_view); A.view_stride = stride;
            return A;
        }));
    } else {
        std::vector<rtk_view> back;
        if (!h_views) {
            back.resize(n);
            RTK_HIP(hipMemcpyAsync(back.data(), d_views, n * sizeof(rtk_view), hipMemcpyDeviceToHost, s));
            RTK_HIP(hipStreamSynchronize(s));
            h_views = back.data();
        }
        CallCounters cc{a, n > 1, s};
        RTK_TRY(cc.begin());
        for (size_t v = 0; v < n; ++v) {
            RTK_TRY(render_frame_impl(a, p, g, h_views[v], d_out + v * stride, s, false));
            RTK_TRY(cc.after_part());
        }
        RTK_TRY(cc.end());
    }
    record_last(a, s, p->collect_stats != 0, primary_rays_of_rank(g) * uint64_t(n));
    return RTK_OK;
}

int radiance_check(const rtk_accel *a, const void *rays, const void *ids, size_t n, const rtk_radiance_params *p, const void *rgb) {
    if (!a || !p) return fail(RTK_ERR_INVALID, "null accel or params");
    if (p->trace_mode != RTK_TRACE_AUTO && p->trace_mode != RTK_TRACE_STREAM)
        return fail(RTK_ERR_INVALID, "trace_mode of a radiance batch must be RTK_TRACE_AUTO or RTK_TRACE_STREAM");
    if (p->max_ray_depth < 0 || p->max_ray_depth > kMaxRayDepth) return fail(RTK_ERR_INVALID, "max_ray_depth must be in [0, 16]");
    if (p->diffuse_rays < 0 || p->diffuse_rays > 32767) return fail(RTK_ERR_INVALID, "diffuse_rays must be in [0, 32767]");
    if (p->sample < 0) return fail(RTK_ERR_INVALID, "sample must be >= 0");
    if (!std::isfinite(p->shadow_bias) || !std::isfinite(p->reflection_bias) || !std::isfinite(p->refraction_bias))
        return fail(RTK_ERR_INVALID, "shadow_bias, reflection_bias and refraction_bias must be finite");
    if (n > (size_t(1) << 38)) return fail(RTK_ERR_INVALID, "too many rays for one call");
    if (n > 0 && (!rays || !rgb)) return fail(RTK_ERR_INVALID, "null ray or colour buffer");
    if (!ids && n > (size_t(1) << 32)) return fail(RTK_ERR_INVALID, "more than 2^32 rays need explicit ids");
    return RTK_OK;
}
// ... 61 lines not shown
    if (p->world_size > 1) return fail(RTK_ERR_INVALID, "regions are not sharded: deal rectangles to the ranks");
    if (n_rects < 0 || n_rects > kMaxRegions) return fail(RTK_ERR_INVALID, "n_rects must be in [0, 65536]");
    if (layout != RTK_REGIONS_IN_FRAME && layout != RTK_REGIONS_PACKED) return fail(RTK_ERR_INVALID, "unknown layout");
    if (n_rects > 0 && (!rects || !out)) return fail(RTK_ERR_INVALID, "null rectangles or output buffer");
    for (int32_t i = 0; i < n_rects; ++i)
        if (!region_valid(rects[i], g.width, g.height)) return fail(RTK_ERR_INVALID, "rectangle " + std::to_string(i) + " is not inside the frame");
    if (layout == RTK_REGIONS_IN_FRAME && regions_overlap(rects, size_t(n_rects)))
        return fail(RTK_ERR_INVALID, "rectangles overlap: RTK_REGIONS_IN_FRAME needs them pairwise disjoint");
    return RTK_OK;
}

uint64_t regions_pixels(const rtk_rect *rects, int32_t n_rects) {
    uint64_t px = 0;
    for (int32_t i = 0; i < n_rects; ++i) px += region_area(rects[i]);
    return px;
}

int regions_table(rtk_accel *a, const FrameGeom &g, const rtk_rect *rects, size_t n, int layout, hipStream_t s) {
    const size_t limit = a->knobs.views_launch_units;
    if (a->rg_table_valid && a->rg_layout == layout && a->rg_width == g.width && a->rg_limit == limit && a->rg_rects.size() == n &&
        std::memcmp(a->rg_rects.data(), rects, n * sizeof(rtk_rect)) == 0) return RTK_OK;
    a->rg_table_valid = false;
    for (rtk_cost_feedback &f : a->fb_regions) f.forget();
    a->rg_plan = plan_regions(rects, n, layout, g.width, limit);
    const size_t n_entries = a->rg_plan.entries.size();
    if (a->rg_table.capacity() < n_entries) {
        RTK_HIP(hipDeviceSynchronize());
        RTK_MEM(a->rg_table.reserve(n_entries, grow_table()));
    } else {
        RTK_HIP(a->rg_last.wait_previous(s));
    }
    RTK_HIP(hipMemcpyAsync(a->rg_table.get(), a->rg_plan.entries.data(), n_entries * sizeof(RegionEntry), hipMemcpyHostToDevice, s));
    a->rg_rects.assign(rects, rects + n);
    a->rg_layout = layout; a->rg_width = g.width; a->rg_limit = limit;
    a->rg_table_valid = true;
    return RTK_OK;
}

int render_regions_impl(rtk_accel *a, const rtk_render_params *p, const FrameGeom &g, const rtk_rect *rects, int32_t n_rects, int layout,
                        float *d_out, hipStream_t s) {
    RTK_TRY(regions_table(a, g, rects, size_t(n_rects), layout, s));
    const RegionsPlan &P = a->rg_plan;
    const bool forks = scene_forks(a, p->diffuse_rays);
    const bool stream = p->trace_mode == RTK_TRACE_STREAM || (p->trace_mode == RTK_TRACE_AUTO && forks);
    dev::RenderArgs A = frame_args(a, p, g, accel_camera(a), d_out);
    if (!stream) {
        RTK_TRY(render_parts(a, a->fb_regions, P.launches.size(), p, g, s, [&](size_t c) {
            const RegionLaunch &L = P.launches[c];
            dev::RenderArgs R = A;
            R.regions = a->rg_table.get() + L.first_entry; R.n_regions = L.n_entries; R.n_units = L.n_units;
            return R;
        }));
    } else {
        uint64_t largest = 0;
        for (const RegionLaunch &L : P.launches) largest = L.n_pixels > largest ? L.n_pixels : largest;
        const size_t chunk = size_t(largest < kRegionChunkPixels ? largest : kRegionChunkPixels);
        if (a->rg_rays.capacity() < chunk || a->rg_ids.capacity() < chunk || a->rg_rgb.capacity() < chunk * 3) {
            const grow_capped rule{size_t(kRegionChunkPixels)};
            RTK_HIP(hipDeviceSynchronize());
            RTK_MEM(a->rg_rays.reserve(chunk, rule));
            RTK_MEM(a->rg_ids.reserve(chunk, rule));
            RTK_MEM(a->rg_rgb.reserve(rule(chunk, 0) * 3));
        }
        rtk_radiance_params rp;
        rp.max_ray_depth = p->max_ray_depth; rp.diffuse_rays = p->diffuse_rays; rp.seed = p->seed; rp.sample = 0;
        rp.shadow_bias = p->shadow_bias; rp.reflection_bias = p->reflection_bias; rp.refraction_bias = p->refraction_bias;
        rp.cull = 1; rp.trace_mode = RTK_TRACE_STREAM;
        RTK_HIP(zero_counters(a, s));
        for (const RegionLaunch &L : P.launches) {
            A.regions = a->rg_table.get() + L.first_entry; A.n_regions = L.n_entries; A.n_units = L.n_units;
            for (uint64_t first = 0; first < L.n_pixels; first += chunk) {
                const uint32_t cn = uint32_t(L.n_pixels - first < chunk ? L.n_pixels - first : chunk);
                for (int smp = g.sample_begin; smp < g.sample_end; ++smp) {
                    RTK_HIP_AS(launch_region_rays(A, smp, first, cn, a->rg_rays.get(), a->rg_ids.get(), s), "launch k_region_rays");
                    rp.sample = smp;
                    RTK_TRY(radiance_device_impl(a, a->rg_rays.get(), a->rg_ids.get(), cn, &rp, a->rg_rgb.get(), s, nullptr));
                    RTK_HIP_AS(launch_add_word(counters_now(a), a->d_rad_counters.get() + radiance_total_word(dev::kStreamLanes) + kRadianceRays, s), "launch k_add_word");
                    RTK_HIP_AS(launch_region_accumulate(A, first, cn, a->rg_rgb.get(), smp == 0, p->spp != 1 && smp + 1 == p->spp, s), "launch k_region_accumulate");
                }
            }
        }
    }
    RTK_HIP(a->rg_last.record(s));
    record_last(a, s, false, P.total_pixels * uint64_t(g.sample_end - g.sample_begin));
    return RTK_OK;
}

}
}

using namespace rtk;

extern "C" {

int rtk_render_output_floats(const rtk_accel *a, const rtk_render_params *p, size_t *n_floats) {
    return abi_guard([&]() -> int {
        if (!n_floats) return fail(RTK_ERR_INVALID, "null n_floats");
        FrameGeom g;
        RTK_TRY(frame_geom(a, p, g));
        *n_floats = out_pixels(g) * 3;
        return RTK_OK;
    });
}

int rtk_render_frame_device(rtk_accel *a, const rtk_render_params *p, float *d_out, void *stream) {
    return abi_guard([&]() -> int {
        if (!a || !p) return fail(RTK_ERR_INVALID, "null accel or params");
        std::lock_guard<std::mutex> lock(a->mu);
        RTK_TRY(ensure_device(a, static_cast<hipStream_t>(stream)));
        return render_device_impl(a, p, d_out, static_cast<hipStream_t>(stream));
    });
}

int rtk_render_last_counters(rtk_accel *a, rtk_counters *c) {
    return abi_guard([&]() -> int {
        if (!a || !c) return fail(RTK_ERR_INVALID, "null accel or counters");
        std::lock_guard<std::mutex> lock(a->mu);
        if (!a->on_device) return fail(RTK_ERR_INVALID, "no frame has been rendered on this accel");
        RTK_HIP(hipSetDevice(a->device));
        RTK_HIP(hipStreamSynchronize(a->last_stream));
        unsigned long long h[kCounterWords];
        RTK_HIP(hipMemcpy(h, counters_now(a), sizeof(h), hipMemcpyDeviceToHost));
        counters_from_block(h, a->last_stats, c);
        for (int i = 0; i < kRayCounterShards; ++i) c->rays += h[kRayShardWord + i];
        c->primary = a->last_primary;
        return RTK_OK;
    });
}

int rtk_render_last_critical_path(rtk_accel *a, double *ms) {
    return abi_guard([&]() -> int {
        if (!a || !ms) return fail(RTK_ERR_INVALID, "null accel or ms");
        std::lock_guard<std::mutex> lock(a->mu);
        if (!a->on_device) return fail(RTK_ERR_INVALID, "no frame has been rendered on this accel");
        RTK_HIP(hipSetDevice(a->device));
        RTK_HIP(hipStreamSynchronize(a->last_stream));
        unsigned long long shard[kRayCounterShards], ticks = 0;
        RTK_HIP(hipMemcpy(shard, counters_now(a) + kCriticalWord, sizeof(shard), hipMemcpyDeviceToHost));
        for (unsigned long long t : shard) ticks = t > ticks ? t : ticks;
        *ms = double(ticks) * 1.0e-5;
        return RTK_OK;
    });
}

int rtk_debug_counter_fills(rtk_accel *a, uint64_t *fills) {
    return abi_guard([&]() -> int {
        if (!a || !fills) return fail(RTK_ERR_INVALID, "null accel or fills");
        std::lock_guard<std::mutex> lock(a->mu);
        *fills = a->counter_fills;
        return RTK_OK;
    });
}

int rtk_render_frame(rtk_accel *a, const rtk_render_params *p, float *rgb, rtk_counters *counters) {
    return abi_guard([&]() -> int {
        if (!a || !p || !rgb) return fail(RTK_ERR_INVALID, "null accel, params or rgb");
        if (p->world_size > 1) return fail(RTK_ERR_INVALID, "rtk_render_frame renders whole frames; use rtk_render_frame_device for sharded output");
        size_t nf = 0;
        RTK_TRY(rtk_render_output_floats(a, p, &nf));
        {
            std::lock_guard<std::mutex> lock(a->mu);
            RTK_TRY(ensure_device(a));
            DevBuf<float> d_out;
            RTK_MEM(d_out.reserve(nf));
            if (p->sample_begin > 0) RTK_HIP_AS(hipMemcpy(d_out.get(), rgb, nf * sizeof(float), hipMemcpyHostToDevice), "upload of the running sums");
            RTK_TRY(render_device_impl(a, p, d_out.get(), nullptr));
            RTK_HIP_AS(hipMemcpy(rgb, d_out.get(), nf * sizeof(float), hipMemcpyDeviceToHost), "frame copy");
        }
        if (counters) return rtk_render_last_counters(a, counters);
        return RTK_OK;
    });
}

int rtk_tiles_assemble_device(const rtk_accel *a, const rtk_render_params *p, const float *d_gathered, float *d_rgb, void *stream) {
    return abi_guard([&]() -> int {
        FrameGeom g;
        RTK_TRY(frame_geom(a, p, g));
        if (!d_gathered || !d_rgb) return fail(RTK_ERR_INVALID, "null buffer");
        dev::AssembleArgs A;
        A.gathered = d_gathered; A.rgb = d_rgb; A.width = g.width; A.height = g.height; A.bucket = g.bucket;
        A.tiles_x = g.tiles_x; A.world = uint32_t(g.world); A.buckets_per_rank = g.buckets_per_rank; A.skew_q = g.skew_q;
        RTK_HIP_AS(launch_assemble(A, static_cast<hipStream_t>(stream)), "launch k_assemble");
        return RTK_OK;
    });
}


int rtk_accel_radiance_device(rtk_accel *a, const rtk_ray *d_rays, const uint32_t *d_ids, size_t n, const rtk_radiance_params *p,
                              float *d_rgb, void *stream) {
    return abi_guard([&]() -> int {
        RTK_TRY(radiance_check(a, d_rays, d_ids, n, p, d_rgb));
        if (n == 0) return RTK_OK;
        std::lock_guard<std::mutex> lock(a->mu);
        RTK_TRY(ensure_device(a, static_cast<hipStream_t>(stream)));
        return radiance_device_impl(a, d_rays, d_ids, n, p, d_rgb, static_cast<hipStream_t>(stream), nullptr);
    });
}

int rtk_accel_radiance(rtk_accel *a, const rtk_ray *rays, const uint32_t *ids, size_t n, const rtk_radiance_params *p, float *rgb,
                       rtk_counters *counters) {
    return abi_guard([&]() -> int {
        RTK_TRY(radiance_check(a, rays, ids, n, p, rgb));
        if (n == 0) {
            if (counters) std::memset(counters, 0, sizeof(*counters));
            return RTK_OK;
        }
        std::lock_guard<std::mutex> lock(a->mu);
        RTK_TRY(ensure_device(a));
        RTK_MEM(a->rad_rays.reserve(n));
        RTK_MEM(a->rad_ids.reserve(n));
        RTK_MEM(a->rad_rgb.reserve(n * 3));
        RTK_HIP(hipMemcpy(a->rad_rays.get(), rays, n * sizeof(rtk_ray), hipMemcpyHostToDevice));
        if (ids) RTK_HIP(hipMemcpy(a->rad_ids.get(), ids, n * sizeof(uint32_t), hipMemcpyHostToDevice));
        uint32_t n_chunks = 0;
        RTK_TRY(radiance_device_impl(a, a->rad_rays.get(), ids ? a->rad_ids.get() : nullptr, n, p, a->rad_rgb.get(), nullptr, &n_chunks));
        RTK_HIP(hipMemcpy(rgb, a->rad_rgb.get(), n * 3 * sizeof(float), hipMemcpyDeviceToHost));
        unsigned long long h[kRadianceTotalWords] = {};
        RTK_HIP(hipMemcpy(h, a->d_rad_counters.get() + radiance_total_word(dev::kStreamLanes), sizeof(h), hipMemcpyDeviceToHost));
        if (counters) {
            std::memset(counters, 0, sizeof(*counters));
            counters->rays = h[kRadianceRays]; counters->primary = n;
        }
        if (a->knobs.stream_debug)
            std::fprintf(stderr, "[rtk radiance] rays %zu chunks %u redone %llu node_cap %u\n", n, n_chunks, h[kRadianceRedone], a->ws.node_cap);
        return RTK_OK;
    });
}


int rtk_accel_get_camera(const rtk_accel *a, rtk_view *out) {
    return abi_guard([&]() -> int {
        if (!a || !out) return fail(RTK_ERR_INVALID, "null accel or view");
        std::lock_guard<std::mutex> lock(const_cast<rtk_accel *>(a)->mu);
        *out = accel_camera(a);
        return RTK_OK;
    });
}

int rtk_accel_set_camera(rtk_accel *a, const rtk_view *view) {
    return abi_guard([&]() -> int {
        if (!a || !view) return fail(RTK_ERR_INVALID, "null accel or view");
        std::lock_guard<std::mutex> lock(a->mu);
        std::memcpy(a->scene.cam_pos, view->position, sizeof(a->scene.cam_pos));
        std::memcpy(a->scene.cam_mat, view->matrix, sizeof(a->scene.cam_mat));
        if (!a->knobs.camera_keeps_order) forget_orders(a, kKeepViewOrders | kKeepTrial);
        return RTK_OK;
    });
}

int rtk_render_views_device(rtk_accel *a, const rtk_render_params *p, const rtk_view *d_views, int32_t n_views, float *d_out, void *stream) {
    return abi_guard([&]() -> int {
        if (!a || !p) return fail(RTK_ERR_INVALID, "null accel or params");
        FrameGeom g;
        RTK_TRY(views_check(a, p, d_views, n_views, d_out, g));
        if (n_views == 0) return RTK_OK;
        std::lock_guard<std::mutex> lock(a->mu);
        RTK_TRY(ensure_device(a, static_cast<hipStream_t>(stream)));
        return render_views_impl(a, p, g, nullptr, d_views, n_views, d_out, static_cast<hipStream_t>(stream));
    });
}

int rtk_render_views(rtk_accel *a, const rtk_render_params *p, const rtk_view *views, int32_t n_views, float *rgb, rtk_counters *counters) {
    return abi_guard([&]() -> int {
        if (!a || !p) return fail(RTK_ERR_INVALID, "null accel or params");
        FrameGeom g;
        RTK_TRY(views_check(a, p, views, n_views, rgb, g));
        if (n_views == 0) return RTK_OK;
        {
            std::lock_guard<std::mutex> lock(a->mu);
            RTK_TRY(ensure_device(a));
            const size_t n = size_t(n_views), nf = n * g.width * g.height * 3;
            RTK_MEM(a->views_tab.reserve(n));
            RTK_MEM(a->views_out.reserve(nf));
            RTK_HIP(hipMemcpy(a->views_tab.get(), views, n * sizeof(rtk_view), hipMemcpyHostToDevice));
            if (p->sample_begin > 0) RTK_HIP(hipMemcpy(a->views_out.get(), rgb, nf * sizeof(float), hipMemcpyHostToDevice));
            RTK_TRY(render_views_impl(a, p, g, views, a->views_tab.get(), n_views, a->views_out.get(), nullptr));
            RTK_HIP(hipMemcpy(rgb, a->views_out.get(), nf * sizeof(float), hipMemcpyDeviceToHost));
        }
        if (counters) return rtk_render_last_counters(a, counters);
        return RTK_OK;
    });
}


int rtk_render_regions_device(rtk_accel *a, const rtk_render_params *p, const rtk_rect *rects, int32_t n_rects, int layout, float *d_out,
                              void *stream) {
    return abi_guard([&]() -> int {
        if (!a || !p) return fail(RTK_ERR_INVALID, "null accel or params");
        FrameGeom g;
        RTK_TRY(regions_check(a, p, rects, n_rects, layout, d_out, g));
        if (n_rects == 0 || regions_pixels(rects, n_rects) == 0) return RTK_OK;
        std::lock_guard<std::mutex> lock(a->mu);
        RTK_TRY(ensure_device(a, static_cast<hipStream_t>(stream)));
        return render_regions_impl(a, p, g, rects, n_rects, layout, d_out, static_cast<hipStream_t>(stream));
    });
}

int rtk_render_regions(rtk_accel *a, const rtk_render_params *p, const rtk_rect *rects, int32_t n_rects, int layout, float *rgb,
                       rtk_counters *counters) {
    return abi_guard([&]() -> int {
        if (!a || !p) return fail(RTK_ERR_INVALID, "null accel or params");
        FrameGeom g;
        RTK_TRY(regions_check(a, p, rects, n_rects, layout, rgb, g));
        const uint64_t pixels = n_rects > 0 ? regions_pixels(rects, n_rects) : 0;
        if (pixels == 0) return RTK_OK;
        {
// ... 51 lines not shown
```

simd-raytracer_amd/csrc/api_state.hip:

```cpp
#include <algorithm>
#include <cstring>
#include <mutex>

#include "accel.hpp"

using namespace rtk;

namespace {

int reserve_lights(rtk_accel *a, size_t n) {
    if (n <= a->d_lights.capacity()) return RTK_OK;
    DevBuf<DevLight> larger;
    RTK_MEM(larger.reserve(n, grow_lights()));
    a->d_lights.swap(larger);
    return RTK_OK;
}

void lights_changed(rtk_accel *a, size_t n_before) {
    if (a->scene.lights.size() == n_before) return;
    forget_orders(a, kKeepTrial);
}


constexpr size_t kTexelLimit = 0x7FFFFFFFull;
constexpr size_t kSlotAlign = 16;

inline size_t slot_round(size_t bytes) { return (bytes + kSlotAlign - 1) & ~(kSlotAlign - 1); }
inline bool is_bitmap(const DevTexture &t) { return t.kind == RTK_TEX_BITMAP; }
inline size_t texel_bytes(const DevTexture &t) { return is_bitmap(t) ? size_t(t.bmp[0]) * size_t(t.bmp[1]) * 3 : 0; }

inline bool bitmap_size_ok(int32_t w, int32_t h) { return w >= 1 && h >= 1 && int64_t(w) * int64_t(h) <= (int64_t{1} << 28); }

void host_tri_uv(const rtk_accel *a, const std::vector<float> &vert_uv, std::vector<DevTriUv> &out) {
    std::vector<size_t> first(a->mesh_nverts.size() + 1, 0);
    for (size_t mi = 0; mi < a->mesh_nverts.size(); ++mi) first[mi + 1] = first[mi] + size_t(a->mesh_nverts[mi]);
    out.resize(a->tree.triangles.size());
    for (size_t i = 0; i < out.size(); ++i) {
        const HostTriangle &tr = a->tree.triangles[i];
        for (int k = 0; k < 3; ++k) {
            const size_t g = first[tr.mesh] + tr.vi[k];
            out[i].uv[k * 2] = vert_uv[g * 2]; out[i].uv[k * 2 + 1] = vert_uv[g * 2 + 1];
        }
    }
}

int make_tri_uv(rtk_accel *a, hipStream_t s) {
    RTK_TRY(ensure_update_static(a));
    const size_t nt = size_t(a->scene.n_triangles);
    RTK_MEM(a->topo_spare.tri_uv.reserve(std::max<size_t>(1, nt), grow_bytes()));
    RTK_HIP_AS(launch_tri_uv(a->topo.index.get(), a->topo_vert_uv.get(), uint32_t(nt), uint32_t(a->scene.n_vertices), a->topo_spare.tri_uv.get(), s),
               "launch k_tri_uv");
    return RTK_OK;
}

DevTexture device_row(const DevTexture &host, const rtk_accel::TexSlot &slot) {
    DevTexture t = host;
    if (is_bitmap(t)) t.bmp[2] = slot.off;
    return t;
}

int send_rows(rtk_accel *a, const std::vector<DevTexture> &rows, DevTexture *table, size_t first, size_t n, hipStream_t s) {
    if (n == 0) return RTK_OK;
    RTK_MEM(a->up_stage.reserve(n * sizeof(DevTexture), grow_bytes()));
    std::memcpy(a->up_stage.get(), rows.data() + first, n * sizeof(DevTexture));
    RTK_HIP(hipMemcpyAsync(table + first, a->up_stage.get(), n * sizeof(DevTexture), hipMemcpyHostToDevice, s));
    return RTK_OK;
}

struct TexelPlan {
    uint8_t *dst = nullptr;
    std::vector<rtk_accel::TexSlot> slots;
    size_t used = 0;
    bool moved = false;
};

int place_texels(rtk_accel *a, size_t texture, const DevTexture &row, size_t need, hipStream_t s, TexelPlan &P) {
    const std::vector<DevTexture> &tex = a->scene.textures;
    P.slots = a->tx_slots; P.used = a->tx_used;
    rtk_accel::TexSlot &mine = P.slots[texture];
    const bool same_shape = tex[texture].bmp[0] == row.bmp[0] && tex[texture].bmp[1] == row.bmp[1];
    if (need <= mine.cap) {
        P.dst = a->d_tex_pixels.get() + mine.off;
        if (same_shape) return RTK_OK;
    } else {
        size_t room = slot_round(need + need / 2);
        size_t off = slot_round(P.used);
        if (off + room > kTexelLimit) room = slot_round(need);
        if (off + room <= a->d_tex_pixels.capacity() && off + room <= kTexelLimit && a->d_tex_pixels.get()) {
            mine.off = int32_t(off); mine.cap = room; P.used = off + room;
            P.dst = a->d_tex_pixels.get() + off;
        } else {
            size_t at = 0;
            std::vector<rtk_accel::TexSlot> packed = P.slots;
            for (size_t i = 0; i < tex.size(); ++i) {
                if (!is_bitmap(tex[i])) continue;
                const size_t live = i == texture ? need : texel_bytes(tex[i]);
                packed[i].off = int32_t(at); packed[i].cap = slot_round(i == texture ? need + need / 2 : live);
                if (at + packed[i].cap > kTexelLimit) packed[i].cap = slot_round(live);
                at += packed[i].cap;
                if (at > kTexelLimit) return fail(RTK_ERR_INVALID, "the texel bytes of all bitmaps must fit an int32 offset");
            }
            RTK_MEM(a->tx_pixels.reserve(at, grow_bytes()));
            for (size_t i = 0; i < tex.size(); ++i)
                if (is_bitmap(tex[i]) && i != texture)
                    RTK_HIP(hipMemcpyAsync(a->tx_pixels.get() + packed[i].off, a->d_tex_pixels.get() + P.slots[i].off, texel_bytes(tex[i]),
                                           hipMemcpyDeviceToDevice, s));
            P.slots.swap(packed); P.used = at; P.moved = true;
            P.dst = a->tx_pixels.get() + P.slots[texture].off;
            std::vector<DevTexture> rows(tex.size());
            for (size_t i = 0; i < tex.size(); ++i) rows[i] = device_row(i == texture ? row : tex[i], P.slots[i]);
            RTK_MEM(a->tx_textures.reserve(rows.size()));
            return send_rows(a, rows, a->tx_textures.get(), 0, rows.size(), s);
        }
    }
    std::vector<DevTexture> rows(tex.size());
    rows[texture] = device_row(row, P.slots[texture]);
    return send_rows(a, rows, a->d_textures.get(), texture, 1, s);
}

struct HostTexels {
    bool same = false;
    std::vector<DevTexture> table;
    std::vector<uint8_t> pixels;
};
int host_texels(const rtk_accel *a, size_t texture, int32_t w, int32_t h, const uint8_t *rgb, HostTexels &H) {
    const std::vector<DevTexture> &tex = a->scene.textures;
    const size_t was = texel_bytes(tex[texture]), need = size_t(w) * size_t(h) * 3, at = size_t(tex[texture].bmp[2]);
    const std::vector<uint8_t> &old = a->scene.tex_pixels;
    if (old.size() - was + need > kTexelLimit) return fail(RTK_ERR_INVALID, "the texel bytes of all bitmaps must fit an int32 offset");
    H.same = tex[texture].bmp[0] == w && tex[texture].bmp[1] == h;
    if (H.same) return RTK_OK;
    H.table = tex;
    H.table[texture].bmp[0] = w; H.table[texture].bmp[1] = h;
    for (size_t i = 0; i < tex.size(); ++i)
        if (is_bitmap(tex[i]) && size_t(tex[i].bmp[2]) > at) H.table[i].bmp[2] = int32_t(size_t(tex[i].bmp[2]) - was + need);
    H.pixels.resize(old.size() - was + need);
    std::memcpy(H.pixels.data(), old.data(), at);
    if (rgb) std::memcpy(H.pixels.data() + at, rgb, need);
    std::memcpy(H.pixels.data() + at + need, old.data() + at + was, old.size() - at - was);
    return RTK_OK;
}

int check_texel_call(const rtk_accel *a, int32_t texture, int32_t w, int32_t h) {
    if (texture < 0 || size_t(texture) >= a->scene.textures.size()) return fail(RTK_ERR_INVALID, "texture index out of range");
    if (!bitmap_size_ok(w, h)) return fail(RTK_ERR_INVALID, "bad bitmap texture size");
    if (!is_bitmap(a->scene.textures[size_t(texture)])) return fail(RTK_ERR_INVALID, "the texture is not a bitmap");
    return RTK_OK;
}

void adopt_texels(rtk_accel *a, size_t texture, HostTexels &H, const uint8_t *rgb, TexelPlan *P, bool on_device) {
    if (H.same) { if (rgb) std::memcpy(a->scene.tex_pixels.data() + a->scene.textures[texture].bmp[2], rgb, texel_bytes(a->scene.textures[texture])); }
    else { a->scene.textures.swap(H.table); a->scene.tex_pixels.swap(H.pixels); }
    if (!P) return;
    if (P->moved) { a->d_tex_pixels.swap(a->tx_pixels); a->d_textures.swap(a->tx_textures); }
    a->tx_slots.swap(P->slots); a->tx_used = P->used;
    a->tx_slots[texture].on_device = on_device;
}

template <typename Write>
int set_texels_device(rtk_accel *a, int32_t texture, int32_t w, int32_t h, const void *d_src, hipStream_t s, Write write) {
    if (!a || !d_src) return fail(RTK_ERR_INVALID, "null accel or texels");
    std::lock_guard<std::mutex> lock(a->mu);
    RTK_TRY(check_texel_call(a, texture, w, h));
    HostTexels H;
    RTK_TRY(host_texels(a, size_t(texture), w, h, nullptr, H));
    RTK_TRY(ensure_device(a));
    RTK_HIP(a->geom_fence.quiesce());
    DevTexture row = a->scene.textures[size_t(texture)];
    row.bmp[0] = w; row.bmp[1] = h;
    TexelPlan P;
    RTK_TRY(place_texels(a, size_t(texture), row, size_t(w) * size_t(h) * 3, s, P));
    RTK_TRY(write(P.dst, s));
// ... 369 lines not shown
```

simd-raytracer_amd/csrc/frame_plan.hpp:

```cpp
#pragma once

#include <cstddef>
#include <cstdint>
#include <cstring>

#include "../../include/rtk.h"

namespace rtk {

struct FrameGeom {
    uint32_t width, height, bucket, tiles_x, tiles_y, n_buckets, blocks_side, buckets_per_rank;
    uint32_t skew_q;
    int rank, world;
    int sample_begin, sample_end;
    uint64_t blocks_of(uint64_t buckets) const { return buckets * blocks_side * blocks_side; }
    size_t blocks() const { return size_t(blocks_of(buckets_per_rank)); }
};

inline void shape_sig(const FrameGeom &g, int spp, int max_ray_depth, int diffuse_rays, uint64_t out[3]) {
    out[0] = (uint64_t(uint32_t(g.width)) << 32) | uint32_t(g.height);
    out[1] = (uint64_t(uint32_t(g.rank)) << 32) | uint32_t(g.world);
    out[2] = (uint64_t(uint32_t(spp)) << 32) | (uint64_t(uint32_t(max_ray_depth)) << 16) | uint32_t(diffuse_rays);
}

struct EngineTrial {
    enum { kNoRecord = -1, kPipelinePair = 0, kMegakernelPair = 2 };
    struct Step { bool stream; int record; };
    uint64_t sig[3] = {0, 0, 0};
    int state = 0;

    static bool applies(int trace_mode, bool forks, bool stats) { return trace_mode == RTK_TRACE_AUTO && forks && !stats; }
    bool same(const uint64_t s[3]) const { return std::memcmp(s, sig, sizeof(sig)) == 0; }
    bool waiting(const uint64_t s[3]) const { return state == 3 && same(s); }
    void verdict(float t_stream, float t_mega) { state = t_mega < t_stream ? 5 : 4; }
    void abandon() { state = 0; }
    Step next(const uint64_t s[3], bool trials_on) {
        if (!same(s)) { std::memcpy(sig, s, sizeof(sig)); state = 0; }
        if (!trials_on) return {true, kNoRecord};
        switch (state) {
            case 0: state = 1; return {true, kPipelinePair};
            case 1: state = 2; return {false, kNoRecord};
            case 2: state = 3; return {false, kMegakernelPair};
            case 5: return {false, kNoRecord};
            default: return {true, kNoRecord};
        }
    }
};

struct OrderState {
    struct Knobs { bool first_frame_prior; unsigned resort_every; };
    struct Step { bool prior, resort, use_order, sort_front, sort_behind; int read_set, write_set; };
    size_t units = 0;
    uint64_t sig[5] = {0, 0, 0, 0, 0};
    bool valid = false;
    bool order_valid = false;
    unsigned age = 0;
    bool nwgs_pending = false, nwgs_known = false;
    int set = 0;
    bool presorted = false;

    void forget() { valid = false; order_valid = false; age = 0; nwgs_pending = false; nwgs_known = false; set = 0; presorted = false; }

    static int frame_mode(int trace_mode, size_t n_units, size_t group8_below) {
        if (trace_mode == RTK_TRACE_TWOPASS) return RTK_TRACE_GROUP4;
        return trace_mode != RTK_TRACE_AUTO ? trace_mode : (n_units < group8_below ? RTK_TRACE_GROUP8 : RTK_TRACE_GROUP4);
    }

    size_t capacity(size_t n_units, bool is_frame_table, uint64_t native) {
        if (units >= n_units) return units;
        size_t cap = n_units;
        if (is_frame_table && units == 0 && native > cap && native <= (1ull << 24)) cap = size_t(native);
        units = 0; valid = false; order_valid = false;
        return cap;
    }

    Step step(const uint64_t s[5], int mode, bool stats, bool regions, const Knobs &k) {
        const bool same_shape = valid && std::memcmp(s, sig, sizeof(sig)) == 0;
        if (!same_shape) { order_valid = false; set = 0; presorted = false; }
        Step r = {!same_shape && k.first_frame_prior && mode == RTK_TRACE_GROUP4 && !stats && !regions, false, false, false, false, 0, 0};
        if (same_shape) {
            r.resort = !order_valid || age >= k.resort_every;
            if (r.resort) {
                r.sort_front = !presorted;
                if (presorted) set ^= 1;
                presorted = false;
                order_valid = true; age = 0; nwgs_known = false; nwgs_pending = true;
            }
            age += 1;
            r.sort_behind = age >= k.resort_every;
            presorted = r.sort_behind;
        }
        r.use_order = r.prior || same_shape;
        r.read_set = set; r.write_set = set ^ 1;
        std::memcpy(sig, s, sizeof(sig));
        valid = true;
        return r;
    }

    bool awaits_count() const { return order_valid && nwgs_pending; }
    unsigned workgroups(bool ready, const uint32_t *host_word) {
        if (!order_valid) return 0;
        if (nwgs_pending && ready) { nwgs_pending = false; nwgs_known = true; }
        return nwgs_known && !nwgs_pending ? *host_word : 0;
    }
};

struct CounterState {
    struct Step { int current; bool fill, carry; };
    int current = 0;
    bool other_zero = false;
    const void *stream = nullptr;

    void forget() { other_zero = false; }
    void after_order(const OrderState::Step &st) { if (st.prior || !st.use_order) forget(); }
    Step frame(const void *s, bool carries) {
        const bool flip = carries && other_zero && stream == s;
        if (flip) current ^= 1;
        other_zero = carries; stream = s;
        return {current, !flip, carries};
    }
};

struct ViewsLaunches { size_t per_launch, n_parts; };
inline ViewsLaunches views_launches(size_t n, size_t per_view, size_t limit) {
    const size_t per_launch = per_view >= limit ? 1 : limit / per_view;
    return {per_launch, (n + per_launch - 1) / per_launch};
}

struct StreamWsShape {
    size_t pixels = 0, nodes = 0, lights = 0;
    int lanes = 0;
    bool sum = false;
    StreamWsShape asked() const { StreamWsShape r = *this; if (r.lights == 0) r.lights = 1; if (r.lanes < 1) r.lanes = 1; return r; }
    bool covers(const StreamWsShape &request) const {
        const StreamWsShape r = request.asked();
        return r.pixels <= pixels && r.nodes <= nodes && r.lights <= lights && (!r.sum || sum) && r.lanes <= lanes;
    }
    StreamWsShape grown(const StreamWsShape &request) const {
        const StreamWsShape r = request.asked();
        StreamWsShape n;
        n.pixels = r.pixels > pixels ? r.pixels : pixels; n.nodes = r.nodes > nodes ? r.nodes : nodes;
        n.lights = r.lights > lights ? r.lights : lights; n.lanes = r.lanes > lanes ? r.lanes : lanes;
        n.sum = r.sum || sum;
        return n;
    }
    bool refused() const { return nodes > 0xFFFFFFF0ull; }
    static size_t hit_cap(size_t nodes) { return nodes / 2 + 64; }
};

}
```

simd-raytracer_amd/csrc/kernels.hip:

```cpp
#include <hip/hip_runtime.h>

#include "kernels.hpp"
#include "trace.hip.hpp"
#include "shade.hip.hpp"

namespace rtk {
namespace dev {

template <int MODE, bool STATS, bool LDS_NODES>
__global__ __launch_bounds__(256) void k_intersect(IntersectArgs A) {
    extern __shared__ __attribute__((aligned(16))) unsigned char smem[];
    DevNode *lds_nodes = reinterpret_cast<DevNode *>(smem);
    if (LDS_NODES) stage_nodes(A.tree.nodes, A.tree.n_nodes, lds_nodes);

    const size_t slot = (size_t)blockIdx.x * blockDim.x + threadIdx.x;
    const bool active = slot < A.n;
    size_t i = (active && A.perm != nullptr) ? (size_t)A.perm[slot] : slot;
    uint32_t raster_w = A.raster_w;
    if (A.verdict != nullptr) {
        if (A.verdict[16] != 0u) return;
        raster_w = A.verdict[15];
        if (raster_w < 64u || (raster_w & 7u) != 0u || (size_t)raster_w * 16u > A.n) raster_w = 0u;
    }
    if (raster_w != 0u) {
        const size_t band = (size_t)raster_w * 8u;
        const size_t tiled = (A.n / band) * band;
        if (slot < tiled) {
            const size_t b = slot / band;
            const uint32_t within = (uint32_t)(slot % band), tile = within >> 6, l = within & 63u;
            i = (b * 8u + (l >> 3)) * (size_t)raster_w + (size_t)tile * 8u + (l & 7u);
        }
    }
    Ray r;
    if (active) {
        const float *p = reinterpret_cast<const float *>(A.rays + i);
        r = make_ray(mk(p[0], p[1], p[2]), mk(p[3], p[4], p[5]));
    } else {
        r = make_ray(mk(0.f, 0.f, 0.f), mk(1.f, 1.f, 1.f));
    }
    Stats st = {0, 0, 0, 0, 0, 0};
    __shared__ __attribute__((aligned(16))) float wave_bundles[4][kMaxBundles * kBundleFloats];
    SliceCtx sx = {nullptr, 0u, 0u, true, 0u, wave_bundles[(threadIdx.x >> 6) & 3u]};
    const Cand c = trace<MODE, STATS, LDS_NODES>(A.tree, lds_nodes, r, A.cull != 0, active, st, sx);
    if (active) {
        float4 o0, o1;
        if (c.k != kMiss) {
            const Surface s = reconstruct(A.tree, c);
            o0 = make_float4(c.t, c.u, c.v, __uint_as_float(s.tri));
            o1 = make_float4(__uint_as_float(s.mesh), s.hit_normal.x, s.hit_normal.y, s.hit_normal.z);
        } else {
            o0 = make_float4(-1.0f, 0.0f, 0.0f, __uint_as_float(kMiss));
            o1 = make_float4(__uint_as_float(kMiss), 0.0f, 0.0f, 0.0f);
        }
        float4 *out = reinterpret_cast<float4 *>(A.out + i);
        out[0] = o0;
        out[1] = o1;
    }
    if (STATS) flush_stats(st, active ? 1u : 0u, A.counters);
}


__device__ __forceinline__ bool upper_half(const V3 d, const bool sel) {
    Ray q;
    q.o = d; q.d = d; q.inv = d;
    const DirSpread S = dir_spread(q, sel);
    const float dv = S.axis == 0u ? d.x : (S.axis == 1u ? d.y : d.z);
    return sel & !(dv <= S.mid);
}
__device__ __forceinline__ uint32_t burst_part(const V3 d, const bool in, const uint32_t plog) {
    uint32_t part = 0u;
    if (plog == 0u) return part;
    if (upper_half(d, in)) part = 1u;
    if (plog >= 2u) {
#pragma unroll
        for (uint32_t h = 0u; h < 2u; ++h)
            if (upper_half(d, in & (part == h))) part |= 2u;
    }
    return part;
}

template <int SLICES>
struct ShadowBurstService {
    const RenderArgs &A;
    float4 *res;
    __device__ __forceinline__ void operator()(GroupShared *sh, const uint32_t slice) const {
        const uint32_t lane = __lane_id();
        const uint32_t hdr = (uint32_t)__builtin_amdgcn_readfirstlane((int)sh->count);
        const uint32_t plog = hdr & 0xFFu, n_jobs = hdr >> 8;
        const uint32_t first = (uint32_t)__builtin_amdgcn_readfirstlane((int)sh->first);
        const unsigned long long mask = sh->pass_mask;
        const float4 a = sh->ray_o[lane], b = sh->ray_d[lane];
        const V3 P = mk(a.x, a.y, a.z), ncos = mk(a.w, b.x, b.y);
        const bool in_burst = ((mask >> lane) & 1ull) != 0ull;
        for (;;) {
            uint32_t job = 0u;
            if (lane == 0u) job = atomicAdd(&sh->pad[0], 1u);
            job = (uint32_t)__builtin_amdgcn_readfirstlane((int)job);
            if (job >= n_jobs) break;
            const uint32_t k = first + (job >> plog);
            const uint32_t part = job & ((1u << plog) - 1u);
            const DevLight *L = A.lights + k;
            const V3 lp = mk(L->pos[0], L->pos[1], L->pos[2]);
            const LightTerm lt = light_term(L, P, ncos);
            const V3 ld = lt.dir;
            const float radius = lt.radius, contrib = lt.contrib;
            const bool mine = in_burst & (burst_part(ld, in_burst, plog) == part);
            const bool asked = mine & (0.0f < radius);
            const bool q = asked & !(A.skip_unlit != 0 && unlit_query(contrib, b.z));
            const Ray ray = make_ray(P + (A.shadow_bias * ld), ld);
            Stats st = {0, 0, 0, 0, 0, 0};
            SliceCtx sx = {nullptr, 0xFFFFFFFFu, 0u, true, 0u, group_private_bundles<SLICES>(sh, slice)};
            const float exit_t = A.shadow_exit ? radius : -1.0f;
            const Cand c = trace<RTK_TRACE_WAVE, false, false, 1>(A.tree, nullptr, ray, false, q, st, sx, kAutoMinLanes, exit_t,
                                                                  kClsHasApex | (0x100u + k), lp);
            bool clear = true;
            uint32_t fl = mine ? 2u : 0u;
            if (asked) fl |= 1u;
            if (q) clear = (c.k == kMiss) | (radius < c.t);
            res[job * 64u + lane] = make_float4(contrib, clear ? 1.0f : 0.0f, __uint_as_float(fl), 0.0f);
        }
    }
};

__device__ __forceinline__ uint32_t fresh_lane() {
    uint32_t l;
    asm volatile("v_mbcnt_lo_u32_b32 %0, -1, 0\n\tv_mbcnt_hi_u32_b32 %0, -1, %0" : "=v"(l));
    return l;
}

__device__ __forceinline__ Ray spawn_ray(const V3 o, const V3 d) {
    Ray r;
    r.o = o; r.d = d; r.inv = d;
    return r;
}

typedef const RegionEntry __attribute__((address_space(4))) *cptr_region;
__device__ __forceinline__ cptr_region region_entry(const RegionEntry *table, const uint32_t r) {
    return (cptr_region)(const void __attribute__((address_space(4))) *)(table + r);
}

enum : int { ST_NEW_SAMPLE = 0, ST_TRACE, ST_SHADE, ST_LIGHT, ST_RETURN, ST_DONE };
enum : int { PEND_CHILD_BG = 0, PEND_CHILD_BLACK = 1, PEND_SHADOW = 2 };
enum : uint32_t { FR_REFR_A = 0, FR_REFR_B = 1, FR_DIFFUSE = 2 };

struct Frame {
    float a[12];
    uint32_t meta;
    uint32_t tri;
    uint32_t key;
};

template <int MODE, bool STATS, bool FORKS, bool LDS_NODES, int SLICES, bool VIEWS = false, bool REGIONS = false>
__global__ __launch_bounds__(SLICES > 1 ? 64 * SLICES : 256, SLICES == 16 ? 1 : SLICES == 8 ? 2 : (SLICES == 4 && !STATS ? RTK_G4_WAVES : 4)) void k_render(RenderArgs A) {
    FrameProbe phases = FrameProbe::enter();
    if (A.only_if != nullptr && *A.only_if == 0u) return;
// ... 600 lines not shown
    if constexpr (VIEWS || REGIONS) return hipErrorInvalidValue;
    else {
        const unsigned packed = (units + 3u) / 4u;
        switch (mode) {
            case RTK_TRACE_LANE: return launch_render_mode<RTK_TRACE_LANE, 1, false, false>(A, packed, stats, forks, lds, lds_bytes, s);
            case RTK_TRACE_WAVE: return launch_render_mode<RTK_TRACE_WAVE, 1, false, false>(A, packed, stats, forks, lds, lds_bytes, s);
            default: return launch_render_mode<RTK_TRACE_AUTO, 1, false, false>(A, packed, stats, forks, lds, lds_bytes, s);
        }
    }
}

}

hipError_t launch_intersect(const dev::IntersectArgs &A, int mode, bool stats, hipStream_t s) {
    const size_t lds_bytes = (size_t)A.tree.n_nodes * sizeof(DevNode);
    const bool lds = lds_bytes <= kMaxNodeLdsBytes;
    switch (mode) {
        case RTK_TRACE_LANE:
            return stats ? launch_intersect_m<RTK_TRACE_LANE, true>(A, lds, lds_bytes, s)
                         : launch_intersect_m<RTK_TRACE_LANE, false>(A, lds, lds_bytes, s);
        case RTK_TRACE_WAVE:
            return stats ? launch_intersect_m<RTK_TRACE_WAVE, true>(A, lds, lds_bytes, s)
                         : launch_intersect_m<RTK_TRACE_WAVE, false>(A, lds, lds_bytes, s);
        default:
            return stats ? launch_intersect_m<RTK_TRACE_AUTO, true>(A, lds, lds_bytes, s)
                         : launch_intersect_m<RTK_TRACE_AUTO, false>(A, lds, lds_bytes, s);
    }
}

hipError_t launch_render(const dev::RenderArgs &A, int mode, bool stats, bool forks, hipStream_t s, unsigned n_workgroups) {
#ifdef RTK_ONLY_LEAN_G4
    hipLaunchKernelGGL((dev::k_render<RTK_TRACE_WAVE, false, false, false, 4>), dim3(A.n_units), dim3(256), 0, s, A);
    return hipGetLastError();
#else
    if (A.regions != nullptr) {
        if (stats || A.views != nullptr || A.n_regions == 0u || A.n_units == 0u || A.n_units > 0x7FFFFFFFu || A.world > 1) return hipErrorInvalidValue;
        const unsigned listed = (n_workgroups != 0u && n_workgroups < A.n_units) ? n_workgroups : A.n_units;
        return launch_render_units<false, true>(A, mode, A.n_units, listed, false, forks, s);
    }
    const uint32_t bpb = A.blocks_per_bucket_side * A.blocks_per_bucket_side;
    const uint64_t waves = (uint64_t)A.buckets_per_rank * bpb * (A.views != nullptr ? A.n_views : 1u);
    if (waves == 0) return hipSuccess;
    if (waves > 0x7FFFFFFFull) return hipErrorInvalidValue;
    const unsigned listed = (n_workgroups != 0u && n_workgroups < waves) ? n_workgroups : (unsigned)waves;
    if (A.views != nullptr) {
        if (stats || (uint64_t)A.units_per_view * A.n_views != waves || A.n_units != waves) return hipErrorInvalidValue;
        return launch_render_units<true, false>(A, mode, (unsigned)waves, listed, false, forks, s);
    }
    return launch_render_units<false, false>(A, mode, (unsigned)waves, listed, stats, forks, s);
#endif
}

namespace dev {
template <bool VIEWS>
__global__ __launch_bounds__(256) void k_block_prior(RenderArgs A, uint8_t *cls, uint32_t *count ) {
    const uint32_t unit = blockIdx.x * blockDim.x + threadIdx.x;
    const bool have = unit < A.n_units;
    const uint32_t view = (VIEWS && have) ? unit / A.units_per_view : 0u;
    const BlockMap blk = block_map(A, have ? unit - view * (VIEWS ? A.units_per_view : 0u) : 0u);
    const uint32_t x0 = blk.bx + blk.sub_x0, y0 = blk.by + blk.sub_y0;
    const bool in_frame = have && blk.bucket < A.n_buckets && x0 < A.width && y0 < A.height;
    const uint32_t x1 = x0 + 7u < A.width ? x0 + 7u : A.width - 1u, y1 = y0 + 7u < A.height ? y0 + 7u : A.height - 1u;
    RenderArgs P = A;
    P.spp = 1;
    if constexpr (VIEWS) {
        const float *cam = A.views + (size_t)(view < A.n_views ? view : 0u) * 12u;
        for (int i = 0; i < 3; ++i) P.cam_pos[i] = cam[i];
        for (int i = 0; i < 9; ++i) P.cam_mat[i] = cam[3 + i];
    }
    const float4 *root = reinterpret_cast<const float4 *>(A.tree.nodes);
    const float4 r0 = root[0], r1 = root[1];
    float t_min;
    const Ray centre = camera_ray(P, in_frame ? (x0 + x1) >> 1 : 0u, in_frame ? (y0 + y1) >> 1 : 0u, 0u);
    const bool centre_in = in_frame && slab(r0.x, r0.y, r0.z, r0.w, r1.x, r1.y, centre, t_min);
    bool enters = centre_in;
    if (in_frame) {
        const uint32_t px[4] = {x0, x1, x0, x1}, py[4] = {y0, y0, y1, y1};
#pragma unroll
        for (int i = 0; i < 4; ++i) {
            const Ray r = camera_ray(P, px[i], py[i], 0u);
            enters = enters | slab(r0.x, r0.y, r0.z, r0.w, r1.x, r1.y, r, t_min);
        }
    }
    const uint32_t c = enters ? 1u : 0u;
    if (have) cls[unit] = (uint8_t)c;
#pragma unroll
    for (uint32_t q = 0; q < 3u; ++q) {
        const unsigned long long m = __builtin_amdgcn_ballot_w64(have && c == q);
        if (m != 0ull && (int)__lane_id() == __builtin_ctzll(m)) atomicAdd(count + q, (uint32_t)__popcll(m));
    }
}

__global__ __launch_bounds__(256) void k_prior_layout(const uint8_t *cls, const uint32_t *count, uint32_t *cursor ,
                                                      uint32_t *order, uint32_t *wg_list, uint32_t *hdr, uint32_t n, uint32_t pack) {
    const uint32_t unit = blockIdx.x * blockDim.x + threadIdx.x;
    const bool have = unit < n;
    const uint32_t c = have ? (uint32_t)cls[unit] : 3u;
    const uint32_t n2 = count[2], n1 = count[1], n0 = count[0];
    uint32_t pos = 0u;
#pragma unroll
    for (uint32_t q = 0; q < 3u; ++q) {
        const unsigned long long m = __builtin_amdgcn_ballot_w64(have && c == q);
        if (m == 0ull) continue;
        const int leader = __builtin_ctzll(m);
        uint32_t first = 0u;
        if ((int)__lane_id() == leader) first = atomicAdd(cursor + q, (uint32_t)__popcll(m));
        first = (uint32_t)__builtin_amdgcn_readlane((int)first, leader);
        if (c == q) pos = first + (uint32_t)__popcll(m & ((1ull << __lane_id()) - 1ull));
    }
    if (have) {
        const uint32_t at = c == 2u ? pos : (c == 1u ? n2 + pos : n2 + n1 + pos);
        order[at] = unit;
        if (c != 0u) wg_list[at] = unit;
        else if (pos % pack == 0u) wg_list[n2 + n1 + pos / pack] = 0x80000000u | at;
    }
    if (unit == 0u) { hdr[0] = n2 + n1 + (n0 + pack - 1u) / pack; hdr[1] = n; }
}
}

hipError_t launch_block_prior(const dev::RenderArgs &A, uint8_t *cls, uint32_t *order, uint32_t *wg_list, uint32_t *hdr,
                              uint32_t *scratch , uint32_t pack, hipStream_t s) {
    if (A.n_units == 0u) return hipSuccess;
    const unsigned blocks = (A.n_units + 255u) / 256u;
    if (A.views != nullptr) hipLaunchKernelGGL(dev::k_block_prior<true>, dim3(blocks), dim3(256), 0, s, A, cls, scratch);
    else hipLaunchKernelGGL(dev::k_block_prior<false>, dim3(blocks), dim3(256), 0, s, A, cls, scratch);
    hipLaunchKernelGGL(dev::k_prior_layout, dim3(blocks), dim3(256), 0, s, cls, scratch, scratch + 3, order, wg_list, hdr, A.n_units, pack);
    return hipGetLastError();
}

namespace dev {
__global__ __launch_bounds__(256) void k_counters_fold(const unsigned long long *cur, unsigned long long *acc) {
    const uint32_t i = threadIdx.x;
    if (i >= (uint32_t)kCounterWords) return;
    const bool longest = i >= (uint32_t)kCriticalWord;
    const unsigned long long a = acc[i], c = cur[i];
    acc[i] = longest ? (a < c ? c : a) : a + c;
}
}

hipError_t launch_counters_fold(const unsigned long long *cur, unsigned long long *acc, hipStream_t s) {
    hipLaunchKernelGGL(dev::k_counters_fold, dim3(1), dim3(256), 0, s, cur, acc);
    return hipGetLastError();
}

namespace dev {
__device__ __forceinline__ uint32_t cost_bin(uint32_t c) {
    c |= 1u;
    const uint32_t e = 31u - (uint32_t)__clz((int)c);
    const uint32_t m = e >= 3u ? (c >> (e - 3u)) & 7u : (c << (3u - e)) & 7u;
    return e * 8u + m;
}
__global__ __launch_bounds__(1024) void k_order_by_cost(const uint32_t *cost, uint8_t *bins, uint32_t *order, uint32_t *wg_list,
                                                        uint32_t *hdr, uint32_t n, uint32_t light_below, uint32_t floor_below,
                                                        uint32_t pack) {
    __shared__ uint32_t hist[256];
    __shared__ uint32_t start[256];
    __shared__ uint32_t wg_hist[2][256], wg_base[2][256];
    __shared__ uint32_t n_single_sh;
    const uint32_t light_bin = light_below > 0u ? cost_bin(light_below) : 0u;
    const uint32_t floor_raw = floor_below > 0u ? cost_bin(floor_below) : 0u;
    const uint32_t floor_bin = floor_raw < light_bin ? floor_raw : light_bin;
    constexpr uint32_t kBatch = 8;
    for (uint32_t i = threadIdx.x; i < 256u; i += blockDim.x) { hist[i] = 0u; wg_hist[0][i] = 0u; wg_hist[1][i] = 0u; }
    __syncthreads();
    for (uint32_t base = 0; base < n; base += blockDim.x * kBatch) {
        uint32_t c[kBatch];
#pragma unroll
        for (uint32_t k = 0; k < kBatch; ++k) {
            const uint32_t i = base + k * blockDim.x + threadIdx.x;
            c[k] = i < n ? cost[i] : 0u;
        }
#pragma unroll
        for (uint32_t k = 0; k < kBatch; ++k) {
            const uint32_t i = base + k * blockDim.x + threadIdx.x;
            uint32_t b = i < n ? cost_bin(c[k]) : 0u;
            if (b < floor_bin) b = 0u;
            if (i < n) bins[i] = (uint8_t)b;
            const unsigned long long cheap = __builtin_amdgcn_ballot_w64(i < n && b == 0u);
            if (i < n && b != 0u) atomicAdd(&hist[b], 1u);
            if (cheap != 0ull && (int)__lane_id() == __builtin_ctzll(cheap)) atomicAdd(&hist[0], (uint32_t)__popcll(cheap));
        }
    }
    __syncthreads();
    if (threadIdx.x == 0u) {
        uint32_t acc = 0u;
        uint32_t singles = 0u;
        for (int b = 255; b >= 0; --b) {
            start[b] = acc; acc += hist[b];
            if (light_bin == 0u || (uint32_t)b >= light_bin) singles = acc;
        }
        n_single_sh = light_bin > 0u ? singles : n;
        hdr[1] = n;
    }
    __syncthreads();
    for (uint32_t base = 0; base < n; base += blockDim.x * kBatch) {
        uint32_t b[kBatch], pos[kBatch];
#pragma unroll
        for (uint32_t k = 0; k < kBatch; ++k) {
            const uint32_t i = base + k * blockDim.x + threadIdx.x;
            b[k] = i < n ? (uint32_t)bins[i] : 0u;
        }
#pragma unroll
        for (uint32_t k = 0; k < kBatch; ++k) {
            const uint32_t i = base + k * blockDim.x + threadIdx.x;
            const unsigned long long cheap = __builtin_amdgcn_ballot_w64(i < n && b[k] == 0u);
            pos[k] = 0u;
            if (i < n && b[k] != 0u) pos[k] = atomicAdd(&start[b[k]], 1u);
            if (cheap != 0ull) {
                const int leader = __builtin_ctzll(cheap);
                uint32_t first = 0u;
                if ((int)__lane_id() == leader) first = atomicAdd(&start[0], (uint32_t)__popcll(cheap));
                first = (uint32_t)__builtin_amdgcn_readlane((int)first, leader);
                if (i < n && b[k] == 0u) pos[k] = first + (uint32_t)__popcll(cheap & ((1ull << __lane_id()) - 1ull));
            }
        }
#pragma unroll
        for (uint32_t k = 0; k < kBatch; ++k) {
            const uint32_t i = base + k * blockDim.x + threadIdx.x;
            if (i < n) order[pos[k]] = i;
        }
    }
    __threadfence_block();
    __syncthreads();
    const uint32_t n_single = n_single_sh;
    const uint32_t n_packed = (n - n_single + pack - 1u) / pack;
    const uint32_t n_wgs = n_single + n_packed;
    for (uint32_t w = threadIdx.x; w < n_wgs; w += blockDim.x) {
        const bool packed = w >= n_single;
        const uint32_t at = packed ? n_single + (w - n_single) * pack : w;
        uint32_t key = (uint32_t)bins[order[at]];
        if (packed && key != 0u) key = key + 8u < 255u ? key + 8u : 255u;
        atomicAdd(&wg_hist[packed ? 1 : 0][key], 1u);
    }
    __syncthreads();
    if (threadIdx.x == 0u) {
        uint32_t acc = 0u;
        for (int b = 255; b >= 0; --b) {
            wg_base[0][b] = acc; acc += wg_hist[0][b];
            wg_base[1][b] = acc; acc += wg_hist[1][b];
        }
        hdr[0] = n_wgs;
    }
    __syncthreads();
    for (uint32_t w = threadIdx.x; w < n_wgs; w += blockDim.x) {
        const bool packed = w >= n_single;
        const uint32_t at = packed ? n_single + (w - n_single) * pack : w;
        const uint32_t blk = order[at];
        uint32_t key = (uint32_t)bins[blk];
        if (packed && key != 0u) key = key + 8u < 255u ? key + 8u : 255u;
        const uint32_t pos = atomicAdd(&wg_base[packed ? 1 : 0][key], 1u);
        wg_list[pos] = packed ? (0x80000000u | at) : blk;
    }
}
}

hipError_t launch_order_by_cost(const uint32_t *cost, uint8_t *bins, uint32_t *order, uint32_t *wg_list, uint32_t *hdr, uint32_t n,
                                uint32_t light_below, uint32_t floor_below, uint32_t pack, hipStream_t s) {
    if (n == 0u) return hipSuccess;
    if (pack == 0u) return hipErrorInvalidValue;
    hipLaunchKernelGGL(dev::k_order_by_cost, dim3(1), dim3(1024), 0, s, cost, bins, order, wg_list, hdr, n, light_below, floor_below, pack);
    return hipGetLastError();
}

hipError_t launch_camera_rays(const dev::RenderArgs &A, int sample, rtk_ray *d_rays, hipStream_t s) {
    const size_t n = (size_t)A.width * A.height;
    if (n == 0) return hipSuccess;
    hipLaunchKernelGGL(dev::k_camera_rays, dim3((unsigned)((n + 255) / 256)), dim3(256), 0, s, A, sample, d_rays);
    return hipGetLastError();
}

hipError_t launch_region_rays(const dev::RenderArgs &A, int sample, uint64_t first, uint32_t n, rtk_ray *d_rays, uint32_t *d_ids, hipStream_t s) {
    if (n == 0u) return hipSuccess;
    if (A.regions == nullptr || A.n_regions == 0u) return hipErrorInvalidValue;
    hipLaunchKernelGGL(dev::k_region_rays, dim3((n + 255u) / 256u), dim3(256), 0, s, A, sample, first, n, d_rays, d_ids);
    return hipGetLastError();
}

hipError_t launch_region_accumulate(const dev::RenderArgs &A, uint64_t first, uint32_t n, const float *d_rgb, bool start, bool divide, hipStream_t s) {
    if (n == 0u) return hipSuccess;
    if (A.regions == nullptr || A.n_regions == 0u) return hipErrorInvalidValue;
    hipLaunchKernelGGL(dev::k_region_accumulate, dim3((n + 255u) / 256u), dim3(256), 0, s, A, first, n, d_rgb, start ? 1 : 0, divide ? 1 : 0);
    return hipGetLastError();
}

hipError_t launch_add_word(unsigned long long *dst, const unsigned long long *src, hipStream_t s) {
    hipLaunchKernelGGL(dev::k_add_word, dim3(1), dim3(64), 0, s, dst, src);
    return hipGetLastError();
}

hipError_t launch_frame_to_texels(const float *d_rgb, size_t n, uint8_t *d_out, hipStream_t s) {
    if (n == 0) return hipSuccess;
    const size_t threads = n / 12u + 1u;
    hipLaunchKernelGGL(dev::k_frame_to_texels, dim3((unsigned)((threads + 255) / 256)), dim3(256), 0, s, d_rgb, n, d_out);
    return hipGetLastError();
}

hipError_t launch_to_rgb8(const float *d_rgb, size_t n, uint8_t *d_out, hipStream_t s) {
    if (n == 0) return hipSuccess;
    hipLaunchKernelGGL(dev::k_to_rgb8, dim3((unsigned)((n + 255) / 256)), dim3(256), 0, s, d_rgb, n, d_out);
    return hipGetLastError();
}

hipError_t launch_assemble(const dev::AssembleArgs &A, hipStream_t s) {
    const size_t n = (size_t)A.width * A.height;
    const unsigned blocks = (unsigned)((n + 255) / 256);
    if (blocks == 0) return hipSuccess;
    hipLaunchKernelGGL(dev::k_assemble, dim3(blocks), dim3(256), 0, s, A);
    return hipGetLastError();
}

}
```

simd-raytracer_amd/csrc/kernels.hpp:

```cpp
#pragma once

#include <hip/hip_runtime.h>

#include "rtk_internal.hpp"
#include "counters.hpp"

namespace rtk {

constexpr int kMaxRayDepth = 16;
constexpr unsigned long long kCriticalMinTicks = 1000;
constexpr uint32_t kSliceMinTrisDefault = 33;
constexpr size_t kMaxNodeLdsBytes = 48 * 1024;

}

#include "trace.hip.hpp"
#include "regions_plan.hpp"

namespace rtk {
namespace dev {

__host__ __device__ inline uint32_t rank_bucket(uint32_t rank, uint32_t local, uint32_t world, uint32_t skew_q) {
    if (skew_q == 0u) return rank + local * world;
    const uint32_t by = local / skew_q, m = local % skew_q;
    const uint32_t c0 = (rank + world - by % world) % world;
    return by * (skew_q * world) + c0 + m * world;
}
__host__ __device__ inline void bucket_owner(uint32_t bucket, uint32_t tiles_x, uint32_t world, uint32_t skew_q, uint32_t &rank, uint32_t &local) {
    if (skew_q == 0u) { rank = bucket % world; local = bucket / world; return; }
    const uint32_t bx = bucket % tiles_x, by = bucket / tiles_x;
    rank = (bx + by) % world; local = by * skew_q + bx / world;
}

struct IntersectArgs {
    TreeView tree;
    const rtk_ray *rays;
    rtk_hit *out;
    size_t n;
    const uint32_t *perm;
    uint32_t raster_w;
    const uint32_t *verdict;
    int cull;
    unsigned long long *counters;
};

struct RenderArgs {
    TreeView tree;
    const DevMaterial *materials;
    const DevTexture *textures;
    const DevTriUv *tri_uv;
    const uint8_t *tex_pixels;
    const DevLight *lights;
    int n_lights;
    int has_refractive;
    float cam_pos[3];
    float cam_mat[9];
    float background[3];
    uint32_t width, height;
    float aspect;
    float tan_half_fov;
    int spp, max_depth, diffuse_rays;
    int sample_begin, sample_end;
    uint32_t seed;
    float shadow_bias, reflection_bias, refraction_bias;
    uint32_t bucket, tiles_x, tiles_y, n_buckets, blocks_per_bucket_side;
    uint32_t buckets_per_rank;
    uint32_t skew_q;
    int rank, world;
    uint32_t slice_min_tris;
    int compact;
    float *out;
    unsigned long long *counters;
    unsigned long long *zero_next;
    unsigned long long keep_offsets_[5];
    const uint32_t *only_if;
    uint32_t n_units;
    uint32_t *cost_out;
    float width_f, height_f, spp_f, gi_div_f;
    const uint32_t *order_in;
    const uint32_t *order_hdr;
    const uint32_t *wg_list;
    int shadow_exit;
    int skip_unlit;
    int occl_on;
    TreeView occl;
    const float *views;
    uint32_t n_views, units_per_view;
    size_t view_stride;
    const RegionEntry *regions;
    uint32_t n_regions;

    __device__ __forceinline__ size_t out_index(uint32_t local_bucket, uint32_t lx, uint32_t ly, uint32_t px,
                                                uint32_t py) const {
        return compact ? (((size_t)local_bucket * bucket + ly) * bucket + lx) : ((size_t)py * width + px);
    }
};

struct AssembleArgs {
    const float *gathered;
    float *rgb;
    uint32_t width, height, bucket, tiles_x, world, buckets_per_rank, skew_q;
};

}

hipError_t launch_intersect(const dev::IntersectArgs &A, int mode, bool stats, hipStream_t s);
hipError_t launch_render(const dev::RenderArgs &A, int mode, bool stats, bool forks, hipStream_t s, unsigned n_workgroups = 0);
hipError_t launch_order_by_cost(const uint32_t *cost, uint8_t *bins , uint32_t *order, uint32_t *wg_list ,
                                uint32_t *hdr , uint32_t n, uint32_t light_below, uint32_t floor_below, uint32_t pack,
                                hipStream_t s);
hipError_t launch_block_prior(const dev::RenderArgs &A, uint8_t *cls, uint32_t *order, uint32_t *wg_list, uint32_t *hdr,
                              uint32_t *scratch, uint32_t pack, hipStream_t s);
hipError_t launch_counters_fold(const unsigned long long *cur, unsigned long long *acc, hipStream_t s);
hipError_t launch_assemble(const dev::AssembleArgs &A, hipStream_t s);
hipError_t launch_camera_rays(const dev::RenderArgs &A, int sample, rtk_ray *d_rays, hipStream_t s);
hipError_t launch_to_rgb8(const float *d_rgb, size_t n, uint8_t *d_out, hipStream_t s);
hipError_t launch_frame_to_texels(const float *d_rgb, size_t n, uint8_t *d_out, hipStream_t s);
hipError_t launch_region_rays(const dev::RenderArgs &A, int sample, uint64_t first, uint32_t n, rtk_ray *d_rays, uint32_t *d_ids, hipStream_t s);
hipError_t launch_region_accumulate(const dev::RenderArgs &A, uint64_t first, uint32_t n, const float *d_rgb, bool start, bool divide, hipStream_t s);
hipError_t launch_add_word(unsigned long long *dst, const unsigned long long *src, hipStream_t s);

}
```

Baseline: 14380 Mrays/s.

## Judge resorted tile orders by GPU frame time and back off resort interval

Adds an on-device judge that timestamps each render frame and compares the render time under a freshly sorted tile order against the previous champion. If the new order is slower, the old order list is copied back. The resort interval also doubles after a few sorts, up to a cap of 128 frames, so sort and readback kernels run less often. In exchange it adds small stamp and judge kernels per judged frame. It also forces n_wgs to zero on those frames, which may cost the persistent-workgroup count optimisation.

```diff
diff --git a/include/rtk.h b/include/rtk.h
--- a/include/rtk.h
+++ b/include/rtk.h
@@ -204,6 +204,16 @@
 int rtk_render_last_counters(rtk_accel *accel, rtk_counters *counters);
 int rtk_render_last_critical_path(rtk_accel *accel, double *ms);
 int rtk_debug_counter_fills(rtk_accel *accel, uint64_t *fills);
+typedef struct rtk_order_judge_stats {
+    uint64_t sorts, judges;
+    uint64_t taken, rejected;
+    uint32_t champion_ticks, challenger_ticks;
+    uint32_t units;
+    int32_t read_set;
+} rtk_order_judge_stats;
+enum { RTK_ORDER_TABLE_FRAMES = 0, RTK_ORDER_TABLE_VIEWS = 1, RTK_ORDER_TABLE_REGIONS = 2 };
+int rtk_debug_order_judge(rtk_accel *accel, int32_t table, int32_t index, rtk_order_judge_stats *stats);
+int rtk_debug_order_lists(rtk_accel *accel, int32_t set, uint32_t *words, size_t capacity, size_t *n_words);
 int rtk_tiles_assemble_device(const rtk_accel *accel, const rtk_render_params *p, const float *d_gathered,
                               float *d_rgb, void *hip_stream);
 
diff --git a/simd-raytracer_amd/__init__.py b/simd-raytracer_amd/__init__.py
--- a/simd-raytracer_amd/__init__.py
+++ b/simd-raytracer_amd/__init__.py
@@ -18,6 +18,7 @@
 OCC_CLEAR, OCC_OCCLUDED, OCC_STEP_LIMIT = 0, 1, 2
 OCCLUDED_MAX_STEPS = 1024
 REGIONS_IN_FRAME, REGIONS_PACKED = 0, 1
+ORDER_TABLE_FRAMES, ORDER_TABLE_VIEWS, ORDER_TABLE_REGIONS = 0, 1, 2
 MAX_REGIONS = 65536
 
 ABI_SYMBOLS = [
@@ -32,7 +33,7 @@
     "rtk_accel_update_vertices", "rtk_accel_update_vertices_device",
     "rtk_accel_update_geometry", "rtk_accel_update_geometry_device",
     "rtk_render_output_floats", "rtk_render_frame", "rtk_render_frame_device", "rtk_render_last_counters",
-    "rtk_render_last_critical_path", "rtk_debug_counter_fills",
+    "rtk_render_last_critical_path", "rtk_debug_counter_fills", "rtk_debug_order_judge", "rtk_debug_order_lists",
     "rtk_tiles_assemble_device", "rtk_camera_rays", "rtk_camera_rays_device",
     "rtk_accel_get_camera", "rtk_accel_set_camera", "rtk_render_views", "rtk_render_views_device",
     "rtk_render_regions", "rtk_render_regions_device",
@@ -117,6 +118,14 @@
 
 class Counters(C.Structure):
     _fields_ = [(n, C.c_uint64) for n in ("rays", "primary", "hits", "nodes", "boxpass", "leaves", "tris", "packets16")]
+
+    def as_dict(self):
+        return {n: int(getattr(self, n)) for n, _ in self._fields_}
+
+
+class OrderJudgeStats(C.Structure):
+    _fields_ = [("sorts", C.c_uint64), ("judges", C.c_uint64), ("taken", C.c_uint64), ("rejected", C.c_uint64),
+                ("champion_ticks", C.c_uint32), ("challenger_ticks", C.c_uint32), ("units", C.c_uint32), ("read_set", C.c_int32)]
 
     def as_dict(self):
         return {n: int(getattr(self, n)) for n, _ in self._fields_}
@@ -190,6 +199,9 @@
 _L.rtk_render_last_critical_path.argtypes = [_vp, C.POINTER(C.c_double)]
 if hasattr(_L, "rtk_debug_counter_fills"):
     _L.rtk_debug_counter_fills.argtypes = [_vp, C.POINTER(C.c_uint64)]
+if hasattr(_L, "rtk_debug_order_judge"):
+    _L.rtk_debug_order_judge.argtypes = [_vp, C.c_int32, C.c_int32, C.POINTER(OrderJudgeStats)]
+    _L.rtk_debug_order_lists.argtypes = [_vp, C.c_int32, _vp, C.c_size_t, C.POINTER(C.c_size_t)]
 _L.rtk_tiles_assemble_device.argtypes = [_vp, C.POINTER(RenderParams), _vp, _vp, _vp]
 _L.rtk_camera_rays.argtypes = [_vp, C.POINTER(RenderParams), C.c_int32, _vp]
 _L.rtk_camera_rays_device.argtypes = [_vp, C.POINTER(RenderParams), C.c_int32, _vp, _vp]
@@ -891,6 +903,21 @@
         _check(_L.rtk_debug_counter_fills(self._h, C.byref(n)))
         return int(n.value)
 
+    def order_judge(self, table: int = ORDER_TABLE_FRAMES, index: int = 0) -> dict:
+        st = OrderJudgeStats()
+        _check(_L.rtk_debug_order_judge(self._h, table, index, C.byref(st)))
+        return st.as_dict()
+
+    def order_lists(self, which: int):
+        n = C.c_size_t(0)
+        _check(_L.rtk_debug_order_lists(self._h, which, None, 0, C.byref(n)))
+        if n.value == 0:
+            return None
+        words = np.empty(n.value, np.uint32)
+        _check(_L.rtk_debug_order_lists(self._h, which, words.ctypes.data, words.size, C.byref(n)))
+        units = (n.value - 4) // 2
+        return words[:units], words[units:units + 4], words[units + 4:]
+
     def assemble_device(self, cfg: RenderConfig, d_gathered_ptr: int, d_rgb_ptr: int, stream: int = 0) -> None:
         p = cfg.to_c()
         _check(_L.rtk_tiles_assemble_device(self._h, C.byref(p), d_gathered_ptr, d_rgb_ptr, stream))
diff --git a/simd-raytracer_amd/csrc/accel.hpp b/simd-raytracer_amd/csrc/accel.hpp
--- a/simd-raytracer_amd/csrc/accel.hpp
+++ b/simd-raytracer_amd/csrc/accel.hpp
@@ -13,6 +13,7 @@
 #include "build.hpp"
 #include "dev_mem.hpp"
 #include "frame_plan.hpp"
+#include "order_judge.hpp"
 #include "update_plan.hpp"
 
 struct rtk_knobs {
@@ -23,6 +24,9 @@
     bool auto_trials = true;
     bool cost_feedback = true;
     unsigned resort_every = 16;
+    unsigned resort_max = 128;
+    bool judge = true;
+    int judge_force = rtk::kJudgeByScore;
     uint32_t light_cycles = 140000u;
     uint32_t order_floor_cycles = 20000u;
     bool batch_scalar_surv = false;
@@ -63,7 +67,10 @@
         if (geti("RTK_BUNDLE_CULL", v)) k.bundle_cull = v != 0;
         if (geti("RTK_AUTO_TRIALS", v)) k.auto_trials = v != 0;
         if (geti("RTK_COST_FEEDBACK", v)) k.cost_feedback = v != 0;
-        if (geti("RTK_COST_RESORT_EVERY", v) && v > 0) k.resort_every = unsigned(v);
+        if (geti("RTK_COST_RESORT_EVERY", v) && v > 0) { k.resort_every = unsigned(v); k.resort_max = 0; }
+        if (geti("RTK_COST_RESORT_MAX", v) && v >= 0 && v <= (1l << 30)) k.resort_max = unsigned(v);
+        if (geti("RTK_COST_JUDGE", v)) k.judge = v != 0;
+        if (geti("RTK_COST_JUDGE_FORCE", v) && v >= rtk::kJudgeByScore && v <= rtk::kJudgeAlwaysKeep) k.judge_force = int(v);
         if (geti("RTK_LIGHT_BELOW_CYCLES", v) && v >= 0) k.light_cycles = uint32_t(v);
         if (geti("RTK_ORDER_FLOOR_CYCLES", v) && v >= 0) k.order_floor_cycles = uint32_t(v);
         if (geti("RTK_REPACK", v)) k.repack = v != 0;
@@ -195,6 +202,9 @@
     rtk::OrderState state;
     rtk::PinBuf<uint32_t> nwgs_host;
     rtk::DevEvent nwgs_ev;
+    rtk::DevBuf<uint32_t> judge;
+    size_t list_units = 0;
+    uint64_t sorts = 0, judges = 0;
 
     void forget() { state.forget(); }
 };
@@ -377,6 +387,13 @@
     if (!(keep & kKeepTrial)) a->trial.abandon();
 }
 
+inline void restart_order_schedules(rtk_accel *a) {
+    const unsigned every = a->knobs.resort_every;
+    a->fb.state.restart_schedule(every);
+    for (rtk_cost_feedback &f : a->fb_views) f.state.restart_schedule(every);
+    for (rtk_cost_feedback &f : a->fb_regions) f.state.restart_schedule(every);
+}
+
 int remake_occluders(rtk_accel *a, const std::vector<DevMaterial> &materials, const DevMaterial *d_materials, hipStream_t s);
 int ensure_update_static(rtk_accel *a);
 void dense_texture_slots(rtk_accel *a);
diff --git a/simd-raytracer_amd/csrc/api_frame.hip b/simd-raytracer_amd/csrc/api_frame.hip
--- a/simd-raytracer_amd/csrc/api_frame.hip
+++ b/simd-raytracer_amd/csrc/api_frame.hip
@@ -301,7 +301,11 @@
     return RTK_OK;
 }
 
-int ensure_feedback_ws(rtk_accel *a, rtk_cost_feedback &fb, const FrameGeom &g, size_t units) {
+int ensure_feedback_ws(rtk_accel *a, rtk_cost_feedback &fb, const FrameGeom &g, size_t units, hipStream_t s) {
+    if (fb.judge.get() == nullptr) {
+        RTK_MEM(fb.judge.reserve(kJudgeWords));
+        RTK_HIP(hipMemsetAsync(fb.judge.get(), 0, kJudgeWords * sizeof(uint32_t), s));
+    }
     if (fb.state.units >= units) return RTK_OK;
     const uint32_t bk = g.bucket;
     const uint64_t tx = (uint64_t(a->scene.width > 0 ? a->scene.width : 0) + bk - 1) / bk, ty = (uint64_t(a->scene.height > 0 ? a->scene.height : 0) + bk - 1) / bk;
@@ -319,16 +323,30 @@
     return {order, order + units, order + units + 4};
 }
 
-int launch_sort(rtk_accel *a, rtk_cost_feedback &fb, int k, int frame_mode, size_t units, hipStream_t s) {
-    const ListSet L = list_set(fb, k, units);
-    RTK_HIP_AS(launch_order_by_cost(fb.cost.get(), fb.bins.get(), L.order, L.wg_list, L.hdr, uint32_t(units),
-                                    frame_mode == RTK_TRACE_GROUP4 ? a->knobs.light_cycles >> 4 : 0u, a->knobs.order_floor_cycles >> 4, 4u, s),
-               "launch k_order_by_cost");
+int read_back_count(rtk_cost_feedback &fb, const ListSet &L, hipStream_t s) {
     RTK_MEM(fb.nwgs_host.reserve(1));
     RTK_MEM(fb.nwgs_ev.ensure());
     RTK_HIP(hipMemcpyAsync(fb.nwgs_host.get(), L.hdr, sizeof(uint32_t), hipMemcpyDeviceToHost, s));
     RTK_HIP(hipEventRecord(fb.nwgs_ev.get(), s));
     return RTK_OK;
+}
+
+int launch_sort(rtk_accel *a, rtk_cost_feedback &fb, int k, int frame_mode, size_t units, hipStream_t s, int champion) {
+    const ListSet L = list_set(fb, k, units);
+    RTK_HIP_AS(launch_order_by_cost(fb.cost.get(), fb.bins.get(), L.order, L.wg_list, L.hdr, uint32_t(units),
+                                    frame_mode == RTK_TRACE_GROUP4 ? a->knobs.light_cycles >> 4 : 0u, a->knobs.order_floor_cycles >> 4, 4u, s,
+                                    a->knobs.judge ? fb.judge.get() : nullptr, champion),
+               "launch k_order_by_cost");
+    fb.sorts += 1;
+    return read_back_count(fb, L, s);
+}
+
+int launch_judge(rtk_accel *a, rtk_cost_feedback &fb, int read_set, size_t units, hipStream_t s) {
+    const ListSet R = list_set(fb, read_set, units), O = list_set(fb, read_set ^ 1, units);
+    RTK_HIP_AS(launch_judge_order(fb.judge.get(), R.order, O.order, uint32_t(2 * units + 4), a->knobs.judge_force, s), "launch k_judge_order");
+    fb.judges += 1;
+    fb.state.rearm_count();
+    return read_back_count(fb, R, s);
 }
 
 int order_launch(rtk_accel *a, rtk_cost_feedback &fb, const rtk_render_params *p, const FrameGeom &g, dev::RenderArgs &A, int frame_mode,
@@ -338,13 +356,15 @@
     sig[3] = (uint64_t(uint32_t(g.bucket)) << 32) | (uint64_t(uint32_t(g.sample_end - g.sample_begin) & 0xFFFFu) << 16) | uint32_t(p->trace_mode);
     sig[4] = A.regions ? ((1ull << 63) | (uint64_t(A.n_regions) << 32) | uint64_t(A.n_units))
                        : (A.views ? uint64_t(A.n_views) : 0ull);
-    RTK_TRY(ensure_feedback_ws(a, fb, g, units));
-    step = fb.state.step(sig, frame_mode, p->collect_stats != 0, A.regions != nullptr, {a->knobs.first_frame_prior, a->knobs.resort_every});
+    RTK_TRY(ensure_feedback_ws(a, fb, g, units, s));
+    step = fb.state.step(sig, frame_mode, p->collect_stats != 0, A.regions != nullptr,
+                         {a->knobs.first_frame_prior, a->knobs.resort_every, a->knobs.resort_max});
+    fb.list_units = units;
     const ListSet L = list_set(fb, step.read_set, units);
     if (step.prior)
         RTK_HIP_AS(launch_block_prior(A, fb.bins.get(), L.order, L.wg_list, L.hdr,
                                       reinterpret_cast<uint32_t *>(A.counters + kPriorScratchWord), 4u, s), "launch k_block_prior");
-    if (step.sort_front) RTK_TRY(launch_sort(a, fb, step.read_set, frame_mode, units, s));
+    if (step.sort_front) RTK_TRY(launch_sort(a, fb, step.read_set, frame_mode, units, s, kChampionNone));
     if (step.use_order) { A.order_in = L.order; A.order_hdr = L.hdr; A.wg_list = L.wg_list; }
     if (&fb == &a->fb) a->cnt.after_order(step);
     A.cost_out = fb.cost.get();
@@ -368,9 +388,17 @@
         n_wgs = fb.state.workgroups(ready, fb.nwgs_host.get());
     }
     int rc = RTK_OK;
-    const hipError_t e = launch_render(A, frame_mode, p->collect_stats != 0, general, s, n_wgs);
+    const bool judged = step.judge && a->knobs.judge && units <= 0x7FFFFFF0ull / 2;
+    if (a->knobs.judge && (judged || step.sort_behind)) {
+        n_wgs = 0;
+        const hipError_t es = launch_stamp(fb.judge.get(), s);
+        if (es != hipSuccess) rc = hip_fail(es, "launch k_stamp");
+    }
+    const hipError_t e = rc == RTK_OK ? launch_render(A, frame_mode, p->collect_stats != 0, general, s, n_wgs) : hipSuccess;
     if (e != hipSuccess) rc = hip_fail(e, "launch k_render");
-    if (rc == RTK_OK && step.sort_behind) rc = launch_sort(a, fb, step.write_set, frame_mode, units, s);
+    if (rc == RTK_OK && judged) rc = launch_judge(a, fb, step.read_set, units, s);
+    if (rc == RTK_OK && step.sort_behind)
+        rc = launch_sort(a, fb, step.write_set, frame_mode, units, s, judged ? kChampionLeave : kChampionScore);
     if (rc != RTK_OK) fb.forget();
     return rc;
 }
@@ -738,6 +766,46 @@
     });
 }
 
+int rtk_debug_order_judge(rtk_accel *a, int32_t table, int32_t index, rtk_order_judge_stats *st) {
+    return abi_guard([&]() -> int {
+        if (!a || !st) return fail(RTK_ERR_INVALID, "null accel or stats");
+        if (table < RTK_ORDER_TABLE_FRAMES || table > RTK_ORDER_TABLE_REGIONS || index < 0) return fail(RTK_ERR_INVALID, "unknown table or negative index");
+        std::lock_guard<std::mutex> lock(a->mu);
+        std::memset(st, 0, sizeof(*st));
+        const std::vector<rtk_cost_feedback> *many = table == RTK_ORDER_TABLE_VIEWS ? &a->fb_views : table == RTK_ORDER_TABLE_REGIONS ? &a->fb_regions : nullptr;
+        if (many ? size_t(index) >= many->size() : index != 0) return RTK_OK;
+        const rtk_cost_feedback &fb = many ? (*many)[size_t(index)] : a->fb;
+        st->sorts = fb.sorts; st->judges = fb.judges;
+        st->units = uint32_t(fb.list_units); st->read_set = fb.state.set;
+        if (!a->on_device || fb.judge.get() == nullptr) return RTK_OK;
+        RTK_HIP(hipSetDevice(a->device));
+        RTK_HIP(hipStreamSynchronize(a->last_stream));
+        uint32_t h[kJudgeWords];
+        RTK_HIP(hipMemcpy(h, fb.judge.get(), sizeof(h), hipMemcpyDeviceToHost));
+        st->taken = h[kJudgeTaken]; st->rejected = h[kJudgeRejected];
+        st->champion_ticks = h[kJudgeChampion]; st->challenger_ticks = h[kJudgeChallenger];
+        return RTK_OK;
+    });
+}
+
+int rtk_debug_order_lists(rtk_accel *a, int32_t set, uint32_t *words, size_t capacity, size_t *n_words) {
+    return abi_guard([&]() -> int {
+        if (!a || !n_words) return fail(RTK_ERR_INVALID, "null accel or n_words");
+        if (set != 0 && set != 1) return fail(RTK_ERR_INVALID, "set must be 0 or 1");
+        std::lock_guard<std::mutex> lock(a->mu);
+        rtk_cost_feedback &fb = a->fb;
+        const size_t units = fb.list_units;
+        if (!a->on_device || units == 0 || fb.state.units < units || fb.order.get() == nullptr) { *n_words = 0; return RTK_OK; }
+        *n_words = 2 * units + 4;
+        if (!words) return RTK_OK;
+        if (capacity < *n_words) return fail(RTK_ERR_INVALID, "capacity is below 2 * units + 4 words");
+        RTK_HIP(hipSetDevice(a->device));
+        RTK_HIP(hipStreamSynchronize(a->last_stream));
+        RTK_HIP(hipMemcpy(words, list_set(fb, set, units).order, *n_words * sizeof(uint32_t), hipMemcpyDeviceToHost));
+        return RTK_OK;
+    });
+}
+
 int rtk_render_frame(rtk_accel *a, const rtk_render_params *p, float *rgb, rtk_counters *counters) {
     return abi_guard([&]() -> int {
         if (!a || !p || !rgb) return fail(RTK_ERR_INVALID, "null accel, params or rgb");
diff --git a/simd-raytracer_amd/csrc/api_state.hip b/simd-raytracer_amd/csrc/api_state.hip
--- a/simd-raytracer_amd/csrc/api_state.hip
+++ b/simd-raytracer_amd/csrc/api_state.hip
@@ -17,7 +17,7 @@
 }
 
 void lights_changed(rtk_accel *a, size_t n_before) {
-    if (a->scene.lights.size() == n_before) return;
+    if (a->scene.lights.size() == n_before) { restart_order_schedules(a); return; }
     forget_orders(a, kKeepTrial);
 }
 
diff --git a/simd-raytracer_amd/csrc/frame_plan.hpp b/simd-raytracer_amd/csrc/frame_plan.hpp
--- a/simd-raytracer_amd/csrc/frame_plan.hpp
+++ b/simd-raytracer_amd/csrc/frame_plan.hpp
@@ -48,8 +48,8 @@
 };
 
 struct OrderState {
-    struct Knobs { bool first_frame_prior; unsigned resort_every; };
-    struct Step { bool prior, resort, use_order, sort_front, sort_behind; int read_set, write_set; };
+    struct Knobs { bool first_frame_prior; unsigned resort_every; unsigned resort_max = 0; };
+    struct Step { bool prior, resort, use_order, sort_front, sort_behind; int read_set, write_set; bool judge = false; };
     size_t units = 0;
     uint64_t sig[5] = {0, 0, 0, 0, 0};
     bool valid = false;
@@ -58,8 +58,20 @@
     bool nwgs_pending = false, nwgs_known = false;
     int set = 0;
     bool presorted = false;
+    unsigned sorts = 0;
 
-    void forget() { valid = false; order_valid = false; age = 0; nwgs_pending = false; nwgs_known = false; set = 0; presorted = false; }
+    void forget() { valid = false; order_valid = false; age = 0; nwgs_pending = false; nwgs_known = false; set = 0; presorted = false; sorts = 0; }
+
+    void restart_schedule(unsigned resort_every) {
+        sorts = 0;
+        if (!presorted && resort_every > 0 && age >= resort_every) age = resort_every - 1;
+    }
+
+    unsigned interval(const Knobs &k) const {
+        uint64_t iv = k.resort_every;
+        for (unsigned i = 3; i <= sorts && iv < k.resort_max; ++i) iv *= 2;
+        return (k.resort_max > k.resort_every && iv > k.resort_max) ? k.resort_max : unsigned(iv);
+    }
 
     static int frame_mode(int trace_mode, size_t n_units, size_t group8_below) {
         if (trace_mode == RTK_TRACE_TWOPASS) return RTK_TRACE_GROUP4;
@@ -76,18 +88,20 @@
 
     Step step(const uint64_t s[5], int mode, bool stats, bool regions, const Knobs &k) {
         const bool same_shape = valid && std::memcmp(s, sig, sizeof(sig)) == 0;
-        if (!same_shape) { order_valid = false; set = 0; presorted = false; }
-        Step r = {!same_shape && k.first_frame_prior && mode == RTK_TRACE_GROUP4 && !stats && !regions, false, false, false, false, 0, 0};
+        if (!same_shape) { order_valid = false; set = 0; presorted = false; sorts = 0; }
+        Step r = {!same_shape && k.first_frame_prior && mode == RTK_TRACE_GROUP4 && !stats && !regions, false, false, false, false, 0, 0, false};
         if (same_shape) {
-            r.resort = !order_valid || age >= k.resort_every;
+            r.resort = !order_valid || age >= interval(k);
             if (r.resort) {
                 r.sort_front = !presorted;
+                r.judge = presorted;
                 if (presorted) set ^= 1;
                 presorted = false;
                 order_valid = true; age = 0; nwgs_known = false; nwgs_pending = true;
+                sorts += 1;
             }
             age += 1;
-            r.sort_behind = age >= k.resort_every;
+            r.sort_behind = age >= interval(k);
             presorted = r.sort_behind;
         }
         r.use_order = r.prior || same_shape;
@@ -96,6 +110,8 @@
         valid = true;
         return r;
     }
+
+    void rearm_count() { if (order_valid) { nwgs_pending = true; nwgs_known = false; } }
 
     bool awaits_count() const { return order_valid && nwgs_pending; }
     unsigned workgroups(bool ready, const uint32_t *host_word) {
diff --git a/simd-raytracer_amd/csrc/kernels.hip b/simd-raytracer_amd/csrc/kernels.hip
--- a/simd-raytracer_amd/csrc/kernels.hip
+++ b/simd-raytracer_amd/csrc/kernels.hip
@@ -1,6 +1,7 @@
 #include <hip/hip_runtime.h>
 
 #include "kernels.hpp"
+#include "order_judge.hpp"
 #include "trace.hip.hpp"
 #include "shade.hip.hpp"
 
@@ -907,7 +908,12 @@
 }
 __global__ __launch_bounds__(1024) void k_order_by_cost(const uint32_t *cost, uint8_t *bins, uint32_t *order, uint32_t *wg_list,
                                                         uint32_t *hdr, uint32_t n, uint32_t light_below, uint32_t floor_below,
-                                                        uint32_t pack) {
+                                                        uint32_t pack, uint32_t *judge, int champion) {
+    if (judge != nullptr && threadIdx.x == 0u) {
+        const unsigned long long now = __builtin_amdgcn_s_memrealtime();
+        const unsigned long long t0 = *reinterpret_cast<const unsigned long long *>(judge + kJudgeStampLo);
+        if (champion != kChampionLeave) judge[kJudgeChampion] = champion == kChampionScore ? judge_score(t0, now) : 0u;
+    }
     __shared__ uint32_t hist[256];
     __shared__ uint32_t start[256];
     __shared__ uint32_t wg_hist[2][256], wg_base[2][256];
@@ -1010,10 +1016,69 @@
 }
 
 hipError_t launch_order_by_cost(const uint32_t *cost, uint8_t *bins, uint32_t *order, uint32_t *wg_list, uint32_t *hdr, uint32_t n,
-                                uint32_t light_below, uint32_t floor_below, uint32_t pack, hipStream_t s) {
+                                uint32_t light_below, uint32_t floor_below, uint32_t pack, hipStream_t s, uint32_t *judge, int champion) {
     if (n == 0u) return hipSuccess;
     if (pack == 0u) return hipErrorInvalidValue;
-    hipLaunchKernelGGL(dev::k_order_by_cost, dim3(1), dim3(1024), 0, s, cost, bins, order, wg_list, hdr, n, light_below, floor_below, pack);
+    hipLaunchKernelGGL(dev::k_order_by_cost, dim3(1), dim3(1024), 0, s, cost, bins, order, wg_list, hdr, n, light_below, floor_below, pack,
+                       judge, champion);
+    return hipGetLastError();
+}
+
+namespace dev {
+__global__ __launch_bounds__(64) void k_stamp(unsigned long long *stamp) {
+    if (threadIdx.x == 0u) *stamp = __builtin_amdgcn_s_memrealtime();
+}
+}
+
+hipError_t launch_stamp(uint32_t *judge, hipStream_t s) {
+    if (judge == nullptr) return hipErrorInvalidValue;
+    hipLaunchKernelGGL(dev::k_stamp, dim3(1), dim3(64), 0, s, reinterpret_cast<unsigned long long *>(judge + kJudgeStampLo));
+    return hipGetLastError();
+}
+
+namespace dev {
+__global__ __launch_bounds__(1024) void k_judge_order(uint32_t *judge, uint32_t *read_set, const uint32_t *other_set, uint32_t words, int force) {
+    __shared__ uint32_t take_sh;
+    if (threadIdx.x == 0u) {
+        const unsigned long long now = __builtin_amdgcn_s_memrealtime();
+        const unsigned long long t0 = *reinterpret_cast<const unsigned long long *>(judge + kJudgeStampLo);
+        const Verdict v = judge_order({judge[kJudgeChampion], judge_score(t0, now)}, force);
+        judge[kJudgeChampion] = v.after.champion;
+        judge[kJudgeChallenger] = v.after.challenger;
+        judge[v.take ? kJudgeTaken : kJudgeRejected] += 1u;
+        take_sh = v.take ? 1u : 0u;
+    }
+    __syncthreads();
+    if (take_sh != 0u) return;
+    uint32_t done = 0u;
+    if (((reinterpret_cast<uintptr_t>(read_set) | reinterpret_cast<uintptr_t>(other_set)) & 15u) == 0u) {
+        const uint32_t quads = words >> 2;
+        const uint4 *src = reinterpret_cast<const uint4 *>(other_set);
+        uint4 *dst = reinterpret_cast<uint4 *>(read_set);
+        constexpr uint32_t kBatch = 4;
+        for (uint32_t base = 0; base < quads; base += blockDim.x * kBatch) {
+            uint4 v[kBatch];
+#pragma unroll
+            for (uint32_t k = 0; k < kBatch; ++k) {
+                const uint32_t i = base + k * blockDim.x + threadIdx.x;
+                if (i < quads) v[k] = src[i];
+            }
+#pragma unroll
+            for (uint32_t k = 0; k < kBatch; ++k) {
+                const uint32_t i = base + k * blockDim.x + threadIdx.x;
+                if (i < quads) dst[i] = v[k];
+            }
+        }
+        done = quads << 2;
+    }
+    for (uint32_t i = done + threadIdx.x; i < words; i += blockDim.x) read_set[i] = other_set[i];
+}
+}
+
+hipError_t launch_judge_order(uint32_t *judge, uint32_t *read_set, const uint32_t *other_set, uint32_t words, int force, hipStream_t s) {
+    if (judge == nullptr || read_set == nullptr || other_set == nullptr || read_set == other_set) return hipErrorInvalidValue;
+    if (words == 0u) return hipSuccess;
+    hipLaunchKernelGGL(dev::k_judge_order, dim3(1), dim3(1024), 0, s, judge, read_set, other_set, words, force);
     return hipGetLastError();
 }
 
diff --git a/simd-raytracer_amd/csrc/kernels.hpp b/simd-raytracer_amd/csrc/kernels.hpp
--- a/simd-raytracer_amd/csrc/kernels.hpp
+++ b/simd-raytracer_amd/csrc/kernels.hpp
@@ -106,9 +106,12 @@
 
 hipError_t launch_intersect(const dev::IntersectArgs &A, int mode, bool stats, hipStream_t s);
 hipError_t launch_render(const dev::RenderArgs &A, int mode, bool stats, bool forks, hipStream_t s, unsigned n_workgroups = 0);
+enum : int { kChampionNone = 0, kChampionScore = 1, kChampionLeave = 2 };
 hipError_t launch_order_by_cost(const uint32_t *cost, uint8_t *bins , uint32_t *order, uint32_t *wg_list ,
                                 uint32_t *hdr , uint32_t n, uint32_t light_below, uint32_t floor_below, uint32_t pack,
-                                hipStream_t s);
+                                hipStream_t s, uint32_t *judge = nullptr, int champion = kChampionNone);
+hipError_t launch_stamp(uint32_t *judge, hipStream_t s);
+hipError_t launch_judge_order(uint32_t *judge, uint32_t *read_set, const uint32_t *other_set, uint32_t words, int force, hipStream_t s);
 hipError_t launch_block_prior(const dev::RenderArgs &A, uint8_t *cls, uint32_t *order, uint32_t *wg_list, uint32_t *hdr,
                               uint32_t *scratch, uint32_t pack, hipStream_t s);
 hipError_t launch_counters_fold(const unsigned long long *cur, unsigned long long *acc, hipStream_t s);
diff --git a/simd-raytracer_amd/csrc/order_judge.hpp b/simd-raytracer_amd/csrc/order_judge.hpp
--- /dev/null
+++ b/simd-raytracer_amd/csrc/order_judge.hpp
@@ -0,0 +1,42 @@
+#pragma once
+
+#include <cstdint>
+
+#if defined(__HIPCC__) || defined(__CUDACC__)
+#define RTK_JUDGE_FN __host__ __device__ inline
+#else
+#define RTK_JUDGE_FN inline
+#endif
+
+namespace rtk {
+
+enum : int { kJudgeByScore = 0, kJudgeAlwaysTake = 1, kJudgeAlwaysKeep = 2 };
+
+enum : uint32_t {
+    kJudgeStampLo = 0, kJudgeStampHi = 1,
+    kJudgeChampion = 2,
+    kJudgeChallenger = 3,
+    kJudgeTaken = 4, kJudgeRejected = 5,
+    kJudgeWords = 6
+};
+
+RTK_JUDGE_FN uint32_t judge_score(uint64_t frame_start, uint64_t behind_start) {
+    if (frame_start == 0 || behind_start <= frame_start) return 0u;
+    const uint64_t d = behind_start - frame_start;
+    return d > 0xFFFFFFFFull ? 0xFFFFFFFFu : uint32_t(d);
+}
+
+struct JudgeScores { uint32_t champion, challenger; };
+struct Verdict {
+    bool take;
+    JudgeScores after;
+};
+
+RTK_JUDGE_FN Verdict judge_order(JudgeScores s, int force) {
+    bool take = s.champion == 0u || s.challenger == 0u || s.challenger <= s.champion;
+    if (force == kJudgeAlwaysTake) take = true;
+    if (force == kJudgeAlwaysKeep) take = false;
+    return {take, {take ? s.challenger : s.champion, s.challenger}};
+}
+
+}
```

Measured after the change: 15110 Mrays/s (median of 6 runs). +5.1%, better.
